# azuxmioy/Render-In-Between

Measured on AMD Instinct MI355X. Metric: rendered frames/sec at 512x512 (generator forward + blend, device-resident), higher is better.
Workload: dtype f32

## Files before the change

### render-in-between_amd/csrc/kernels.hip.h

```cpp
#pragma once
#include "igemm.hip.h"

namespace rib {

struct GemmDmaParams {
  const float* A; const float* B; float* C;
  int M, N, K, lda, ldc;
  size_t sA, sB, sC;
  int modB;
};

typedef uint32_t u32x4 __attribute__((ext_vector_type(4)));
__device__ __forceinline__ void split3_bf16(const float4 p, const float4 q, bf16x8& hi, bf16x8& mid, bf16x8& lo) {
  const float x[8] = {p.x, p.y, p.z, p.w, q.x, q.y, q.z, q.w};
  u32x4 h, m, l;
#pragma unroll
  for (int i = 0; i < 4; ++i) {
    const uint32_t u0 = __float_as_uint(x[2 * i]), u1 = __float_as_uint(x[2 * i + 1]);
    h[i] = __builtin_amdgcn_perm(u1, u0, 0x07060302u);
    const float r0 = x[2 * i] - __uint_as_float(u0 & 0xffff0000u), r1 = x[2 * i + 1] - __uint_as_float(u1 & 0xffff0000u);
    const uint32_t v0 = __float_as_uint(r0), v1 = __float_as_uint(r1);
    m[i] = __builtin_amdgcn_perm(v1, v0, 0x07060302u);
    const float s0 = r0 - __uint_as_float(v0 & 0xffff0000u), s1 = r1 - __uint_as_float(v1 & 0xffff0000u);
    l[i] = __builtin_amdgcn_perm(__float_as_uint(s1), __float_as_uint(s0), 0x07060302u);
  }
  hi = __builtin_bit_cast(bf16x8, h); mid = __builtin_bit_cast(bf16x8, m); lo = __builtin_bit_cast(bf16x8, l);
}

template <int WM, int WN, int NF, int ST = ST_F32, int X3 = 0>
__global__ __launch_bounds__(256) void k_gemm_dma(const GemmDmaParams p) {
  static_assert(WM * WN == 4, "4 waves per workgroup");
  static_assert(X3 == 0 || ST == ST_F32, "split products: fp32 storage");
  constexpr int BM = 32 * WM, BN = 32 * NF * WN, BK = 32;
  constexpr int EPW = ST == ST_F32 ? 1 : 2;
  constexpr int STAGE = (BM + BN) * BK;
  constexpr int NFILL = (BM + BN) / 32;
  __shared__ __attribute__((aligned(16))) float smem[2 * STAGE];
  const int tid = threadIdx.x, lane = tid & 63, li = lane & 31, lh = lane >> 5;
  const int wave = __builtin_amdgcn_readfirstlane(tid >> 6);
  const int wm = wave / WN, wn = wave % WN;
  const int m0 = blockIdx.x * BM, n0 = blockIdx.y * BN;
  const int z = blockIdx.z;
  const float* A = p.A + (size_t)z * p.sA / EPW;
  const float* B = p.B + (size_t)(p.modB ? z % p.modB : 0) * p.sB / EPW;
  f32x16 acc[NF];
  f32x16 acc_s[X3 == 2 ? NF : 1];
#pragma unroll
  for (int nf = 0; nf < NF; ++nf)
#pragma unroll
    for (int r = 0; r < 16; ++r) { acc[nf][r] = 0.f; if constexpr (X3 == 2) acc_s[nf][r] = 0.f; }
  const int nch = p.K / (BK * EPW);
  typedef __attribute__((address_space(3))) void lds_void;
  const uint32_t lds0 = (uint32_t)(size_t)(lds_void*)smem;
  const float* src[NFILL];
#pragma unroll
  for (int j = 0; j < NFILL; ++j) {
    const int trow = wave * 8 + 32 * j + (lane >> 3);
    const bool isA = 32 * j < BM;
    const int row = isA ? trow : trow - BM;
    const int ls = (lane & 7) ^ ((row >> 1) & 7);
    src[j] = isA ? A + (size_t)min(m0 + row, p.M - 1) * (p.lda / EPW) + ls * 4 : B + (size_t)min(n0 + row, p.N - 1) * (p.K / EPW) + ls * 4;
  }
  auto fill = [&](int st, int kc) {
#pragma unroll
    for (int j = 0; j < NFILL; ++j) {
      const uint32_t dst = lds0 + (uint32_t)(st * STAGE + (wave * 8 + 32 * j) * BK) * 4u;
      asm volatile("s_mov_b32 m0, %0\n\ts_nop 0\n\tglobal_load_lds_dwordx4 %1, off" ::"s"(dst), "v"(src[j] + kc) : "memory");
    }
  };
  fill(0, 0);
  for (int c = 0; c < nch; ++c) {
    const int st = c & 1;
    asm volatile("s_waitcnt vmcnt(0)\n\ts_waitcnt lgkmcnt(0)\n\ts_barrier" ::: "memory");
    if (c + 1 < nch) fill(st ^ 1, (c + 1) * BK);
    const float* sA = smem + st * STAGE;
    const float* sB = sA + BM * BK;
    if constexpr (X3 != 0) {
#pragma unroll
      for (int ks = 0; ks < BK / 16; ++ks) {
        const int s0 = ks * 4 + lh, s1 = s0 + 2;
        const int ra = wm * 32 + li;
        bf16x8 ah, am, al;
        split3_bf16(*reinterpret_cast<const float4*>(sA + ra * BK + (s0 ^ ((ra >> 1) & 7)) * 4),
                    *reinterpret_cast<const float4*>(sA + ra * BK + (s1 ^ ((ra >> 1) & 7)) * 4), ah, am, al);
#pragma unroll
        for (int nf = 0; nf < NF; ++nf) {
          const int rb = (wn * NF + nf) * 32 + li;
          bf16x8 bh, bm, bl;
          split3_bf16(*reinterpret_cast<const float4*>(sB + rb * BK + (s0 ^ ((rb >> 1) & 7)) * 4),
                      *reinterpret_cast<const float4*>(sB + rb * BK + (s1 ^ ((rb >> 1) & 7)) * 4), bh, bm, bl);
          f32x16& sm = X3 == 2 ? acc_s[nf] : acc[nf];
          sm = __builtin_amdgcn_mfma_f32_32x32x16_bf16(am, bm, sm, 0, 0, 0);
          sm = __builtin_amdgcn_mfma_f32_32x32x16_bf16(ah, bl, sm, 0, 0, 0);
          sm = __builtin_amdgcn_mfma_f32_32x32x16_bf16(al, bh, sm, 0, 0, 0);
          sm = __builtin_amdgcn_mfma_f32_32x32x16_bf16(ah, bm, sm, 0, 0, 0);
          sm = __builtin_amdgcn_mfma_f32_32x32x16_bf16(am, bh, sm, 0, 0, 0);
          acc[nf] = __builtin_amdgcn_mfma_f32_32x32x16_bf16(ah, bh, acc[nf], 0, 0, 0);
        }
      }
      continue;
    }
#pragma unroll
    for (int kb = 0; kb < BK / 8; ++kb) {
      const int slot = kb * 2 + lh;
      const int ra = wm * 32 + li;
      const float4 a = *reinterpret_cast<const float4*>(sA + ra * BK + (slot ^ ((ra >> 1) & 7)) * 4);
      float4 b[NF];
#pragma unroll
      for (int nf = 0; nf < NF; ++nf) {
        const int rb = (wn * NF + nf) * 32 + li;
        b[nf] = *reinterpret_cast<const float4*>(sB + rb * BK + (slot ^ ((rb >> 1) & 7)) * 4);
      }
#pragma unroll
      for (int nf = 0; nf < NF; ++nf) {
        if constexpr (ST == ST_F32) {
          acc[nf] = __builtin_amdgcn_mfma_f32_32x32x2f32(a.x, b[nf].x, acc[nf], 0, 0, 0);
          acc[nf] = __builtin_amdgcn_mfma_f32_32x32x2f32(a.y, b[nf].y, acc[nf], 0, 0, 0);
          acc[nf] = __builtin_amdgcn_mfma_f32_32x32x2f32(a.z, b[nf].z, acc[nf], 0, 0, 0);
          acc[nf] = __builtin_amdgcn_mfma_f32_32x32x2f32(a.w, b[nf].w, acc[nf], 0, 0, 0);
        } else if constexpr (ST == ST_F16) {
          acc[nf] = __builtin_amdgcn_mfma_f32_32x32x16_f16(*reinterpret_cast<const f16x8*>(&a), *reinterpret_cast<const f16x8*>(&b[nf]), acc[nf], 0, 0, 0);
        } else {
          acc[nf] = __builtin_amdgcn_mfma_f32_32x32x16_bf16(*reinterpret_cast<const bf16x8*>(&a), *reinterpret_cast<const bf16x8*>(&b[nf]), acc[nf], 0, 0, 0);
        }
      }
    }
  }
  float* C = p.C + (size_t)z * p.sC;
#pragma unroll
  for (int nf = 0; nf < NF; ++nf) {
    const int col = n0 + (wn * NF + nf) * 32 + li;
#pragma unroll
    for (int r = 0; r < 16; ++r) {
      const int row = m0 + wm * 32 + (r & 3) + 8 * (r >> 2) + 4 * lh;
      float v = acc[nf][r];
      if constexpr (X3 == 2) v += acc_s[nf][r];
      if (row < p.M && col < p.N) C[(size_t)row * p.ldc + col] = v;
    }
  }
}

struct FinalizeParams {
  const double* part;
  int tiles, Cs, C;
// ... 106 lines not shown
      const int oy = pix / p.Wout, ox = pix % p.Wout;
      const size_t rpix = p.res_ups ? ((size_t)n * (p.Hout >> 1) + (oy >> 1)) * (p.Wout >> 1) + (ox >> 1) : (size_t)n * npix + pix;
#pragma unroll
      for (int e = 0; e < 4; ++e) rres[k][e] = ld_act<ST>(p.res, rpix * p.resC + min(c4 * 4 + e, p.resC - 1));
    }
  }
  float vals[4][4];
#pragma unroll
  for (int k = 0; k < 4; ++k) {
    const int pix = blockIdx.x * ppb + k * slots + slot;
    const float4 a = acc4[k];
    const float v[4] = {a.x + bv.x, a.y + bv.y, a.z + bv.z, a.w + bv.w};
#pragma unroll
    for (int e = 0; e < 4; ++e) {
      float t = v[e];
      if (p.res) t += rres[k][e];
      t = apply_act(t, p.act);
      if constexpr (ST != ST_F32) t = round16<ST>(t);
      vals[k][e] = (pix < npix && c4 * 4 + e < p.Cout) ? t : 0.f;
    }
#pragma unroll
    for (int e = 0; e < 4; ++e) { s1[e] += (double)vals[k][e]; s2[e] += (double)vals[k][e] * (double)vals[k][e]; }
  }
#pragma unroll
  for (int k = 0; k < 4; ++k) {
    const int pix = blockIdx.x * ppb + k * slots + slot;
    if (pix < npix) {
      const size_t opix = (size_t)n * npix + pix;
#pragma unroll
      for (int e = 0; e < 4; ++e)
        if (c4 * 4 + e < p.Cout) st_act<ST>(p.y, opix * p.yC + p.yoff + c4 * 4 + e, vals[k][e]);
    }
  }
  if (p.stat_part) {
#pragma unroll
    for (int e = 0; e < 4; ++e) { red[0][threadIdx.x][e] = s1[e]; red[1][threadIdx.x][e] = s2[e]; }
    __syncthreads();
    for (int c = threadIdx.x; c < p.CoutPad; c += 256) {
      const int g = c / 4, e = c % 4;
      double a1 = 0.0, a2 = 0.0;
      for (int s = 0; s < slots; ++s) { a1 += red[0][s * c4n + g][e]; a2 += red[1][s * c4n + g][e]; }
      double* dst = p.stat_part + (((size_t)n * p.blocks + blockIdx.x) * 2) * p.CoutPad;
      dst[c] = a1;
      dst[p.CoutPad + c] = a2;
    }
  }
}

struct StatSrc {
  const double* part;
  int tiles, Cs;
  float inv_count;
  const float* gamma;
  const float* beta;
};

__device__ __forceinline__ void block_stats_64(const StatSrc& s, int n, int c0, int nch, double* red ,
                                               float* s_sc, float* s_sh) {
  const int j = threadIdx.x & 63, q = threadIdx.x >> 6;
  double a1 = 0.0, a2 = 0.0;
  if (j < nch) stats_from_partials(s.part + (size_t)n * s.tiles * 2 * s.Cs, s.tiles, s.Cs, c0 + j, q, 4, a1, a2);
  red[(q * 64 + j) * 2] = a1; red[(q * 64 + j) * 2 + 1] = a2;
  __syncthreads();
  if (q == 0 && j < nch) {
    double t1 = 0.0, t2 = 0.0;
#pragma unroll
    for (int k = 0; k < 4; ++k) { t1 += red[(k * 64 + j) * 2]; t2 += red[(k * 64 + j) * 2 + 1]; }
    float sc, sh;
    scale_shift_of(t1, t2, s.inv_count, s.gamma ? s.gamma[c0 + j] : 1.f, s.beta ? s.beta[c0 + j] : 0.f, sc, sh);
    s_sc[j] = sc; s_sh[j] = sh;
  }
  __syncthreads();
}

enum { WSRC_PLAIN = 0, WSRC_SPADE = 1, WSRC_JOIN = 2 };
struct WinoInParams {
  const float* x; int H, W, xC, Cin;
  const float* pro_scale; const float* pro_shift; int pro_ld, pro_lrelu;
  StatSrc st;
  float* v; int tilesY, tilesX;
  int nslices, ublocks;
  int x_ups; const float* slab; int slab_ld, col0; const float* sbias;
  const float* x2; const float* xres; float* o; const float* pro2_scale; const float* pro2_shift; StatSrc st2;
};

__device__ __forceinline__ float spade_mod1(float x, float sc, float sh, float g, float bg, float b, float bb) {
  return fmaf(fmaf(x, sc, sh), 1.f + (g + bg), b + bb);
}

template <int MODE> struct WinoConsts { float4 sc, sh, bg, bb, sc2, sh2; bool aff; };
template <int MODE> struct WinoRaw { float4 a, b, c; };

template <int MODE>
__device__ __forceinline__ void wino_in_consts(const WinoInParams& p, int n, int slice, int c4, bool cok, double* red, float* s_sc,
                                               float* s_sh, WinoConsts<MODE>& k) {
  k.sc = make_float4(1.f, 1.f, 1.f, 1.f); k.sh = make_float4(0.f, 0.f, 0.f, 0.f);
  k.aff = false;
  const int l = (threadIdx.x & 15) * 4;
  if (p.st.part) {
    block_stats_64(p.st, n, slice * 64, min(64, p.Cin - slice * 64), red, s_sc, s_sh);
    k.sc = make_float4(s_sc[l], s_sc[l + 1], s_sc[l + 2], s_sc[l + 3]);
    k.sh = make_float4(s_sh[l], s_sh[l + 1], s_sh[l + 2], s_sh[l + 3]);
    k.aff = true;
  } else if (p.pro_scale && cok) {
    k.sc = *reinterpret_cast<const float4*>(p.pro_scale + (size_t)n * p.pro_ld + c4 * 4);
    k.sh = *reinterpret_cast<const float4*>(p.pro_shift + (size_t)n * p.pro_ld + c4 * 4);
    k.aff = true;
  }
  if constexpr (MODE == WSRC_SPADE) {
    const int v = c4 * 4, colg = (v / 32) * 64 + (v % 32);
    k.bg = cok ? *reinterpret_cast<const float4*>(p.sbias + colg) : k.sh;
    k.bb = cok ? *reinterpret_cast<const float4*>(p.sbias + colg + 32) : k.sh;
  }
  if constexpr (MODE == WSRC_JOIN) {
    k.sc2 = make_float4(1.f, 1.f, 1.f, 1.f); k.sh2 = make_float4(0.f, 0.f, 0.f, 0.f);
    if (p.x2) {
      if (p.st2.part) {
        __syncthreads();
        block_stats_64(p.st2, n, slice * 64, min(64, p.Cin - slice * 64), red, s_sc, s_sh);
        k.sc2 = make_float4(s_sc[l], s_sc[l + 1], s_sc[l + 2], s_sc[l + 3]);
        k.sh2 = make_float4(s_sh[l], s_sh[l + 1], s_sh[l + 2], s_sh[l + 3]);
      } else if (cok) {
        k.sc2 = *reinterpret_cast<const float4*>(p.pro2_scale + (size_t)n * p.pro_ld + c4 * 4);
        k.sh2 = *reinterpret_cast<const float4*>(p.pro2_shift + (size_t)n * p.pro_ld + c4 * 4);
      }
    }
  }
}

template <int MODE>
__device__ __forceinline__ void wino_fetch(const WinoInParams& p, int n, int cy, int cx, int c4, WinoRaw<MODE>& r) {
  if constexpr (MODE == WSRC_SPADE) {
    const int Hs = p.x_ups ? p.H >> 1 : p.H, Ws = p.x_ups ? p.W >> 1 : p.W;
    const int sy = p.x_ups ? cy >> 1 : cy, sx = p.x_ups ? cx >> 1 : cx;
    r.a = *reinterpret_cast<const float4*>(p.x + (((size_t)n * Hs + sy) * Ws + sx) * p.xC + c4 * 4);
    const int v = c4 * 4, colg = (v / 32) * 64 + (v % 32);
    const float* sl = p.slab + (((size_t)n * p.H + cy) * p.W + cx) * p.slab_ld + p.col0 + colg;
    r.b = *reinterpret_cast<const float4*>(sl);
    r.c = *reinterpret_cast<const float4*>(sl + 32);
  } else {
    const size_t e = (((size_t)n * p.H + cy) * p.W + cx) * p.xC + c4 * 4;
    r.a = *reinterpret_cast<const float4*>(p.x + e);
    if constexpr (MODE == WSRC_JOIN) r.b = *reinterpret_cast<const float4*>((p.x2 ? p.x2 : p.xres) + e);
  }
}

template <int MODE>
__device__ __forceinline__ float4 wino_value(const WinoInParams& p, const WinoConsts<MODE>& k, const WinoRaw<MODE>& r) {
  float4 w = r.a;
  if constexpr (MODE == WSRC_SPADE) {
    w = make_float4(spade_mod1(r.a.x, k.sc.x, k.sh.x, r.b.x, k.bg.x, r.c.x, k.bb.x), spade_mod1(r.a.y, k.sc.y, k.sh.y, r.b.y, k.bg.y, r.c.y, k.bb.y),
                    spade_mod1(r.a.z, k.sc.z, k.sh.z, r.b.z, k.bg.z, r.c.z, k.bb.z), spade_mod1(r.a.w, k.sc.w, k.sh.w, r.b.w, k.bg.w, r.c.w, k.bb.w));
    if (p.pro_lrelu) w = lrelu4(w);
  } else if constexpr (MODE == WSRC_JOIN) {
    w = make_float4(w.x * k.sc.x + k.sh.x, w.y * k.sc.y + k.sh.y, w.z * k.sc.z + k.sh.z, w.w * k.sc.w + k.sh.w);
    if (p.x2) { w.x += r.b.x * k.sc2.x + k.sh2.x; w.y += r.b.y * k.sc2.y + k.sh2.y; w.z += r.b.z * k.sc2.z + k.sh2.z; w.w += r.b.w * k.sc2.w + k.sh2.w; }
    else { w.x += r.b.x; w.y += r.b.y; w.z += r.b.z; w.w += r.b.w; }
  } else {
    if (k.aff) w = make_float4(w.x * k.sc.x + k.sh.x, w.y * k.sc.y + k.sh.y, w.z * k.sc.z + k.sh.z, w.w * k.sc.w + k.sh.w);
    if (p.pro_lrelu) w = lrelu4(w);
  }
  return w;
}

#define RIB_F4_SUB(a, b) make_float4((a).x - (b).x, (a).y - (b).y, (a).z - (b).z, (a).w - (b).w)
#define RIB_F4_ADD(a, b) make_float4((a).x + (b).x, (a).y + (b).y, (a).z + (b).z, (a).w + (b).w)

template <int MODE>
__global__ __launch_bounds__(256) void k_wino_in(const WinoInParams p) {
  __shared__ double red[4 * 64 * 2];
  __shared__ float s_sc[64], s_sh[64];
  const int c4n = p.Cin / 4;
  const int n = blockIdx.y;
  const int slice = blockIdx.x % p.nslices, ub = blockIdx.x / p.nslices;
  const int c4 = slice * 16 + (threadIdx.x & 15);
  const bool cok = c4 < c4n;
  const int ntiles = p.tilesY * p.tilesX;
  WinoConsts<MODE> kc;
  wino_in_consts<MODE>(p, n, slice, c4, cok, red, s_sc, s_sh, kc);
  if (!cok) return;
  for (int u = ub * 16 + (threadIdx.x >> 4); u < ntiles * 4; u += p.ublocks * 16) {
    const int r = u & 3, tile = u >> 2;
    const int ty = tile / p.tilesX, tx = tile % p.tilesX;
    const int ia = r == 0 ? 0 : (r == 2 ? 2 : 1), ib = r == 0 ? 2 : (r == 1 ? 2 : (r == 2 ? 1 : 3));
    const float sg = r == 1 ? 1.f : -1.f;
    WinoRaw<MODE> d[2][4];
#pragma unroll
    for (int a = 0; a < 2; ++a)
#pragma unroll
      for (int q = 0; q < 4; ++q) {
        const int iy = 2 * ty - 1 + (a ? ib : ia), ix = 2 * tx - 1 + q;
        wino_fetch<MODE>(p, n, min(max(iy, 0), p.H - 1), min(max(ix, 0), p.W - 1), c4, d[a][q]);
      }
    float4 t[4];
#pragma unroll
    for (int q = 0; q < 4; ++q) {
      float4 v[2];
#pragma unroll
      for (int a = 0; a < 2; ++a) {
        const int iy = 2 * ty - 1 + (a ? ib : ia), ix = 2 * tx - 1 + q;
        const bool inb = iy >= 0 && iy < p.H && ix >= 0 && ix < p.W;
        float4 w = wino_value<MODE>(p, kc, d[a][q]);
        if constexpr (MODE == WSRC_JOIN) {
          if (r == 1 && (q == 1 || q == 2) && inb) *reinterpret_cast<float4*>(p.o + (((size_t)n * p.H + iy) * p.W + ix) * p.xC + c4 * 4) = w;
        }
        if (!inb) w = make_float4(0.f, 0.f, 0.f, 0.f);
        v[a] = w;
      }
      t[q] = make_float4(v[0].x + sg * v[1].x, v[0].y + sg * v[1].y, v[0].z + sg * v[1].z, v[0].w + sg * v[1].w);
    }
    const size_t plane = (size_t)ntiles * p.Cin;
    float* vb = p.v + (size_t)n * 16 * plane + (size_t)tile * p.Cin + c4 * 4;
    *reinterpret_cast<float4*>(vb + (size_t)(r * 4 + 0) * plane) = RIB_F4_SUB(t[0], t[2]);
    *reinterpret_cast<float4*>(vb + (size_t)(r * 4 + 1) * plane) = RIB_F4_ADD(t[1], t[2]);
    *reinterpret_cast<float4*>(vb + (size_t)(r * 4 + 2) * plane) = RIB_F4_SUB(t[2], t[1]);
    *reinterpret_cast<float4*>(vb + (size_t)(r * 4 + 3) * plane) = RIB_F4_SUB(t[1], t[3]);
  }
}

struct WinoOutParams {
  const float* m; int tilesY, tilesX, CoutPad;
  const float* bias;
  float* y; int yC, yoff, Cout, Hout, Wout;
  int act;
  const float* res; int resC;
  double* stat_part;
  int nslices, ublocks;
};

__device__ __forceinline__ void wino_out_partials(double (*red)[256][4], const double s1[4], const double s2[4], double* stat_part,
                                                  int n, int ublocks, int ub, int slice, int CoutPad) {
#pragma unroll
  for (int e = 0; e < 4; ++e) { red[0][threadIdx.x][e] = s1[e]; red[1][threadIdx.x][e] = s2[e]; }
  __syncthreads();
  if (threadIdx.x < 64) {
    const int c = slice * 64 + threadIdx.x;
    if (c < CoutPad) {
      const int g = threadIdx.x >> 2, e = threadIdx.x & 3;
      double a1 = 0.0, a2 = 0.0;
#pragma unroll
      for (int s = 0; s < 16; ++s) { a1 += red[0][s * 16 + g][e]; a2 += red[1][s * 16 + g][e]; }
      double* dst = stat_part + (((size_t)n * ublocks + ub) * 2) * CoutPad;
      dst[c] = a1;
      dst[CoutPad + c] = a2;
    }
  }
}

__global__ __launch_bounds__(256) void k_wino_out(const WinoOutParams p) {
  __shared__ __attribute__((aligned(16))) double red[2][256][4];
  const int c4n = p.CoutPad / 4;
  const int slice = blockIdx.x % p.nslices, ub = blockIdx.x / p.nslices;
  const int c4 = slice * 16 + (threadIdx.x & 15);
  const int n = blockIdx.y;
  const int ntiles = p.tilesY * p.tilesX;
  double s1[4] = {0.0, 0.0, 0.0, 0.0}, s2[4] = {0.0, 0.0, 0.0, 0.0};
  if (c4 < c4n) {
    const float4 bv = *reinterpret_cast<const float4*>(p.bias + c4 * 4);
    const size_t plane = (size_t)ntiles * p.CoutPad;
    for (int u = ub * 16 + (threadIdx.x >> 4); u < ntiles * 2; u += p.ublocks * 16) {
      const int r = u & 1, tile = u >> 1;
      const float* mb = p.m + (size_t)n * 16 * plane + (size_t)tile * p.CoutPad + c4 * 4;
      float4 mm[3][4];
#pragma unroll
      for (int a = 0; a < 3; ++a)
#pragma unroll
        for (int q = 0; q < 4; ++q) mm[a][q] = *reinterpret_cast<const float4*>(mb + (size_t)((r + a) * 4 + q) * plane);
      const float sg = r ? -1.f : 1.f;
      float4 uu[4];
#pragma unroll
      for (int q = 0; q < 4; ++q)
        uu[q] = make_float4(mm[0][q].x + sg * (mm[1][q].x + mm[2][q].x), mm[0][q].y + sg * (mm[1][q].y + mm[2][q].y),
                            mm[0][q].z + sg * (mm[1][q].z + mm[2][q].z), mm[0][q].w + sg * (mm[1][q].w + mm[2][q].w));
      float4 yv[2];
      yv[0] = RIB_F4_ADD(RIB_F4_ADD(uu[0], uu[1]), uu[2]);
      yv[1] = RIB_F4_SUB(RIB_F4_SUB(uu[1], uu[2]), uu[3]);
      const int ty = tile / p.tilesX, tx = tile % p.tilesX;
      const int oy = 2 * ty + r;
      float rr[2][4];
#pragma unroll
      for (int q = 0; q < 2; ++q) {
        const int cy = min(oy, p.Hout - 1), cx = min(2 * tx + q, p.Wout - 1);
#pragma unroll
        for (int e = 0; e < 4; ++e)
          rr[q][e] = p.res ? p.res[(((size_t)n * p.Hout + cy) * p.Wout + cx) * p.resC + min(c4 * 4 + e, p.resC - 1)] : 0.f;
      }
#pragma unroll
      for (int q = 0; q < 2; ++q) {
        const int ox = 2 * tx + q;
        const bool inb = oy < p.Hout && ox < p.Wout;
        const float v4[4] = {yv[q].x + bv.x, yv[q].y + bv.y, yv[q].z + bv.z, yv[q].w + bv.w};
#pragma unroll
        for (int e = 0; e < 4; ++e) {
          float t = apply_act(v4[e] + rr[q][e], p.act);
          const bool ok = inb && c4 * 4 + e < p.Cout;
          if (ok) p.y[(((size_t)n * p.Hout + oy) * p.Wout + ox) * p.yC + p.yoff + c4 * 4 + e] = t;
          t = ok ? t : 0.f;
          s1[e] += (double)t; s2[e] += (double)t * (double)t;
        }
      }
    }
  }
  if (p.stat_part) wino_out_partials(red, s1, s2, p.stat_part, n, p.ublocks, ub, slice, p.CoutPad);
}

__device__ __constant__ float kWino4BT[6][6] = {
    {81.f / 64, 0.f, -45.f / 16, 0.f, 1.f, 0.f},        {0.f, -27.f / 16, -9.f / 4, 3.f / 4, 1.f, 0.f},
    {0.f, 27.f / 16, -9.f / 4, -3.f / 4, 1.f, 0.f},     {0.f, -27.f / 32, -9.f / 16, 3.f / 2, 1.f, 0.f},
    {0.f, 27.f / 32, -9.f / 16, -3.f / 2, 1.f, 0.f},    {0.f, 81.f / 64, 0.f, -45.f / 16, 0.f, 1.f}};
__device__ __constant__ float kWino4AT[4][6] = {
    {1.f, 1.f, 1.f, 1.f, 1.f, 0.f},                      {0.f, 3.f / 4, -3.f / 4, 3.f / 2, -3.f / 2, 0.f},
    {0.f, 9.f / 16, 9.f / 16, 9.f / 4, 9.f / 4, 0.f},    {0.f, 27.f / 64, -27.f / 64, 27.f / 8, -27.f / 8, 1.f}};

__device__ __forceinline__ float4 f4_fma(float a, float4 x, float4 acc) {
  return make_float4(fmaf(a, x.x, acc.x), fmaf(a, x.y, acc.y), fmaf(a, x.z, acc.z), fmaf(a, x.w, acc.w));
}
__device__ __forceinline__ float4 f4_scale(float a, float4 x) { return make_float4(a * x.x, a * x.y, a * x.z, a * x.w); }

template <int MODE>
__global__ __launch_bounds__(256) void k_wino4_in(const WinoInParams p) {
  __shared__ double red[4 * 64 * 2];
  __shared__ float s_sc[64], s_sh[64];
  const int c4n = p.Cin / 4;
  const int n = blockIdx.y;
  const int slice = blockIdx.x % p.nslices, ub = blockIdx.x / p.nslices;
  const int c4 = slice * 16 + (threadIdx.x & 15);
  const bool cok = c4 < c4n;
  const int ntiles = p.tilesY * p.tilesX;
  WinoConsts<MODE> kc;
  wino_in_consts<MODE>(p, n, slice, c4, cok, red, s_sc, s_sh, kc);
  if (!cok) return;
  for (int u = ub * 16 + (threadIdx.x >> 4); u < ntiles * 6; u += p.ublocks * 16) {
    const int r = u % 6, tile = u / 6;
    const int ty = tile / p.tilesX, tx = tile % p.tilesX;
    const int a0 = r == 0 ? 0 : 1, da = (r == 0 || r == 5) ? 2 : 1, na = (r == 0 || r == 5) ? 3 : 4;
    float4 t[6];
#pragma unroll
    for (int q = 0; q < 6; ++q) t[q] = make_float4(0.f, 0.f, 0.f, 0.f);
    if constexpr (MODE == WSRC_PLAIN) {
      WinoRaw<MODE> d[4][6];
#pragma unroll
      for (int k = 0; k < 4; ++k)
#pragma unroll
        for (int q = 0; q < 6; ++q) {
          const int iy = 4 * ty - 1 + a0 + min(k, na - 1) * da, ix = 4 * tx - 1 + q;
          wino_fetch<MODE>(p, n, min(max(iy, 0), p.H - 1), min(max(ix, 0), p.W - 1), c4, d[k][q]);
        }
#pragma unroll
      for (int k = 0; k < 4; ++k) {
        const int a = a0 + min(k, na - 1) * da;
        const float coef = k < na ? kWino4BT[r][a] : 0.f;
        const int iy = 4 * ty - 1 + a;
#pragma unroll
        for (int q = 0; q < 6; ++q) {
          const int ix = 4 * tx - 1 + q;
          float4 w = wino_value<MODE>(p, kc, d[k][q]);
          if (!(iy >= 0 && iy < p.H && ix >= 0 && ix < p.W)) w = make_float4(0.f, 0.f, 0.f, 0.f);
          t[q] = f4_fma(coef, w, t[q]);
        }
      }
    } else {
#pragma unroll 1
      for (int k = 0; k < na; ++k) {
        const int a = a0 + k * da;
        const float coef = kWino4BT[r][a];
        const int iy = 4 * ty - 1 + a;
        WinoRaw<MODE> d[6];
#pragma unroll
        for (int q = 0; q < 6; ++q) wino_fetch<MODE>(p, n, min(max(iy, 0), p.H - 1), min(max(4 * tx - 1 + q, 0), p.W - 1), c4, d[q]);
#pragma unroll
        for (int q = 0; q < 6; ++q) {
          const int ix = 4 * tx - 1 + q;
          const bool inb = iy >= 0 && iy < p.H && ix >= 0 && ix < p.W;
          float4 w = wino_value<MODE>(p, kc, d[q]);
          if constexpr (MODE == WSRC_JOIN) {
            if (r == 1 && q >= 1 && q <= 4 && inb) *reinterpret_cast<float4*>(p.o + (((size_t)n * p.H + iy) * p.W + ix) * p.xC + c4 * 4) = w;
          }
          if (!inb) w = make_float4(0.f, 0.f, 0.f, 0.f);
          t[q] = f4_fma(coef, w, t[q]);
        }
      }
    }
    const size_t plane = (size_t)ntiles * p.Cin;
    float* vb = p.v + (size_t)n * 36 * plane + (size_t)tile * p.Cin + c4 * 4;
    const float4 e24 = f4_fma(-45.f / 16, t[2], t[4]);
    const float4 o13 = f4_fma(-45.f / 16, t[3], t[5]);
    const float4 ev1 = f4_fma(-9.f / 4, t[2], t[4]), od1 = f4_fma(-27.f / 16, t[1], f4_scale(3.f / 4, t[3]));
    const float4 ev2 = f4_fma(-9.f / 16, t[2], t[4]), od2 = f4_fma(-27.f / 32, t[1], f4_scale(3.f / 2, t[3]));
    *reinterpret_cast<float4*>(vb + (size_t)(r * 6 + 0) * plane) = f4_fma(81.f / 64, t[0], e24);
    *reinterpret_cast<float4*>(vb + (size_t)(r * 6 + 1) * plane) = RIB_F4_ADD(ev1, od1);
    *reinterpret_cast<float4*>(vb + (size_t)(r * 6 + 2) * plane) = RIB_F4_SUB(ev1, od1);
    *reinterpret_cast<float4*>(vb + (size_t)(r * 6 + 3) * plane) = RIB_F4_ADD(ev2, od2);
    *reinterpret_cast<float4*>(vb + (size_t)(r * 6 + 4) * plane) = RIB_F4_SUB(ev2, od2);
    *reinterpret_cast<float4*>(vb + (size_t)(r * 6 + 5) * plane) = f4_fma(81.f / 64, t[1], o13);
  }
}

__global__ __launch_bounds__(256) void k_wino4_out(const WinoOutParams p) {
  __shared__ __attribute__((aligned(16))) double red[2][256][4];
  const int c4n = p.CoutPad / 4;
  const int slice = blockIdx.x % p.nslices, ub = blockIdx.x / p.nslices;
  const int c4 = slice * 16 + (threadIdx.x & 15);
  const int n = blockIdx.y;
  const int ntiles = p.tilesY * p.tilesX;
  double s1[4] = {0.0, 0.0, 0.0, 0.0}, s2[4] = {0.0, 0.0, 0.0, 0.0};
  if (c4 < c4n) {
    const float4 bv = *reinterpret_cast<const float4*>(p.bias + c4 * 4);
    const size_t plane = (size_t)ntiles * p.CoutPad;
    for (int unit = ub * 16 + (threadIdx.x >> 4); unit < ntiles * 4; unit += p.ublocks * 16) {
      const int tile = unit >> 2, r = unit & 3;
      const float* mb = p.m + (size_t)n * 36 * plane + (size_t)tile * p.CoutPad + c4 * 4;
      float4 u[6];
#pragma unroll
      for (int q = 0; q < 6; ++q) u[q] = make_float4(0.f, 0.f, 0.f, 0.f);
      const int ax = r == 0 ? 0 : 5;
      const float cx_ = (r == 0 || r == 3) ? 1.f : 0.f;
      float4 mm[5][6];
#pragma unroll
      for (int k = 0; k < 5; ++k)
#pragma unroll
        for (int q = 0; q < 6; ++q) mm[k][q] = *reinterpret_cast<const float4*>(mb + (size_t)((k < 4 ? k + 1 : ax) * 6 + q) * plane);
#pragma unroll
      for (int k = 0; k < 5; ++k) {
        const float coef = k < 4 ? kWino4AT[r][k + 1] : cx_;
#pragma unroll
        for (int q = 0; q < 6; ++q) u[q] = f4_fma(coef, mm[k][q], u[q]);
      }
      const float4 s12 = RIB_F4_ADD(u[1], u[2]);
      const float4 d12 = RIB_F4_SUB(u[1], u[2]);
      const float4 s34 = RIB_F4_ADD(u[3], u[4]);
      const float4 d34 = RIB_F4_SUB(u[3], u[4]);
      float4 yv[4];
      yv[0] = make_float4(u[0].x + s12.x + s34.x, u[0].y + s12.y + s34.y, u[0].z + s12.z + s34.z, u[0].w + s12.w + s34.w);
      yv[1] = f4_fma(3.f / 4, d12, f4_scale(3.f / 2, d34));
      yv[2] = f4_fma(9.f / 16, s12, f4_scale(9.f / 4, s34));
      yv[3] = f4_fma(27.f / 64, d12, f4_fma(27.f / 8, d34, u[5]));
      const int ty = tile / p.tilesX, tx = tile % p.tilesX;
      const int oy = 4 * ty + r;
      float rr[4][4];
#pragma unroll
      for (int q = 0; q < 4; ++q) {
        const int cy = min(oy, p.Hout - 1), cx = min(4 * tx + q, p.Wout - 1);
#pragma unroll
        for (int e = 0; e < 4; ++e)
          rr[q][e] = p.res ? p.res[(((size_t)n * p.Hout + cy) * p.Wout + cx) * p.resC + min(c4 * 4 + e, p.resC - 1)] : 0.f;
      }
#pragma unroll
      for (int q = 0; q < 4; ++q) {
        const int ox = 4 * tx + q;
        const bool inb = oy < p.Hout && ox < p.Wout;
        const float v4[4] = {yv[q].x + bv.x, yv[q].y + bv.y, yv[q].z + bv.z, yv[q].w + bv.w};
#pragma unroll
        for (int e = 0; e < 4; ++e) {
          float t = apply_act(v4[e] + rr[q][e], p.act);
          const bool ok = inb && c4 * 4 + e < p.Cout;
          if (ok) p.y[(((size_t)n * p.Hout + oy) * p.Wout + ox) * p.yC + p.yoff + c4 * 4 + e] = t;
          t = ok ? t : 0.f;
          s1[e] += (double)t; s2[e] += (double)t * (double)t;
        }
      }
    }
  }
  if (p.stat_part) wino_out_partials(red, s1, s2, p.stat_part, n, p.ublocks, ub, slice, p.CoutPad);
}
#undef RIB_F4_SUB
#undef RIB_F4_ADD

struct ModulateParams {
  const float* slab; int ksplit, B, slab_ld, col0;
  const float* bias;
  const float* xm; int xmC, xm_ups;
  const float* m_scale; const float* m_shift; int m_ld;
  StatSrc st;
  int C, nsets;
  float* ys0; float* ys1; int act0, act1;
  int Hout, Wout;
  int nslices, pblocks;
};
// ... 728 lines not shown
```

### render-in-between_amd/csrc/rib.hip

```cpp
#include "kernels.hip.h"
#include "raster.hip.h"
#include "quality.hip.h"
#include "resize.hip.h"
#include <hip/hip_ext.h>
#include "../../include/rib.h"

#include <algorithm>
#include <array>
#include <climits>
#include <cmath>
#include <cstdarg>
#include <cstdio>
#include <cstdlib>
#include <cstring>
#include <map>
#include <memory>
#include <string>
#include <variant>
#include <vector>


#include "variants.hip.h"
#define RIB_V(sec, ...) RIB_I_V(RIB_F_EXTERN, __VA_ARGS__)
#define RIB_VK(sec, ...) RIB_I_VK(RIB_F_EXTERN, __VA_ARGS__)
// ... 23 lines not shown
#undef RIB_VBX
#undef RIB_V1D
#undef RIB_VS1D
#undef RIB_VD
#undef RIB_VSD
#undef RIB_VD9

using namespace rib;

namespace { struct ProfPair { hipEvent_t start = nullptr, stop = nullptr; }; thread_local ProfPair g_prof_pair; }
#define RIB_KLAUNCH(KERNEL, grid, block, lds, st, ...)                                                                       \
  do {                                                                                                                       \
    if (g_prof_pair.start) hipExtLaunchKernelGGL(KERNEL, grid, block, lds, st, g_prof_pair.start, g_prof_pair.stop, 0, __VA_ARGS__); \
    else hipLaunchKernelGGL(KERNEL, grid, block, lds, st, __VA_ARGS__);                                                      \
  } while (0)

#if !defined(RIB_BUILD_STAMP) || !defined(RIB_SHARD_STAMP)
#error "compile through csrc/build.py (-DRIB_BUILD_STAMP / -DRIB_SHARD_STAMP: content hashes of the sources, see build.py)"
#endif
extern "C" {
#define RIB_X(s) extern const char rib_stamp_section_##s[];
RIB_FOR_SECTIONS(RIB_X)
#undef RIB_X
}
extern "C" __attribute__((used, visibility("hidden"))) const char kLibStamp[] = "rib-stamp lib " RIB_BUILD_STAMP;

namespace {

thread_local std::string g_create_error;

std::string fmt(const char* f, ...) {
  char buf[1024];
  va_list ap;
  va_start(ap, f);
  vsnprintf(buf, sizeof buf, f, ap);
  va_end(ap);
  return buf;
}

inline int pad8(int c) { return c <= 8 ? 8 : (c <= 16 ? 16 : (c + 31) / 32 * 32); }
inline int pad16(int c) { return c <= 16 ? 16 : (c + 31) / 32 * 32; }
inline uint16_t host_bf16(float f) {
  uint32_t u; memcpy(&u, &f, 4);
  if ((u & 0x7fffffffu) > 0x7f800000u) return (uint16_t)((u >> 16) | 0x40);
  u += 0x7fffu + ((u >> 16) & 1u);
  return (uint16_t)(u >> 16);
}
inline uint16_t host_f16(float f) {
  uint32_t u; memcpy(&u, &f, 4);
  const uint32_t sign = (u >> 16) & 0x8000u;
  const uint32_t a = u & 0x7fffffffu;
  if (a > 0x7f800000u) return (uint16_t)(sign | 0x7e00u);
  if (a >= 0x477ff000u) return (uint16_t)(sign | 0x7c00u);
  if (a < 0x33000001u) return (uint16_t)sign;
  int e = (int)(a >> 23) - 127;
  uint32_t m = (a & 0x7fffffu) | 0x800000u;
  int shift = e < -14 ? 13 + (-14 - e) : 13;
  uint32_t half_m = m >> shift;
  const uint32_t rem = m & ((1u << shift) - 1), halfway = 1u << (shift - 1);
  if (rem > halfway || (rem == halfway && (half_m & 1u))) half_m += 1;
  uint32_t h16;
  if (e < -14) h16 = half_m;
  else h16 = ((uint32_t)(e + 15) << 10) + (half_m - 0x400u);
  return (uint16_t)(sign | h16);
}
inline int pad32(int c) { return (c + 31) / 32 * 32; }
inline int pick_bk(int cp) { return cp % 32 == 0 ? 32 : (cp % 16 == 0 ? 16 : 8); }
inline size_t align256(size_t b) { return (b + 255) / 256 * 256; }

struct ConvDef {
  std::string name;
  int cin = 0, cout = 0, ks = 3, stride = 1;
  bool spectral = true;
  int spade_cond = 0;
  bool in_affine = false;
  bool used = true;
  size_t w_off = 0, b_off = 0, g_off = 0, be_off = 0;
  size_t fb_off = 0;
  bool ups_in = false;
  size_t wp_off = 0;
  int cinp = 0, coutp = 0;
  size_t w16_off = 0, wp16_off = 0;
  bool wino_ok = false; size_t zero_off = 0;
  size_t wl_off = 0; int lowc_ce = 0, lowc_ncol = 0;
};

struct TensorDef {
  std::string name;
  std::vector<int64_t> dims;
  bool used;
  std::vector<float> data;
  bool set = false;
};

struct SpadeGroup {
  std::string key;
  int C = 0, Cp = 0, cond = 0, nsets = 1;
  size_t w_off = 0, b_off = 0;
  size_t w16_off = 0;
  int npad = 0;
  size_t w1_off = 0, b1_off = 0;
  int level = 0, col0 = 0;
};

struct Cfg {
  rib_config c;
  int nf(int i) const { return std::min(c.max_num_filters, c.num_filters << i); }
  int mask_nf(int i) const { return std::min(c.mask_max_filters, c.mask_filters << i); }
  int emb_ch(int i) const { return std::min(c.emb_max_filters, c.emb_filters << i); }
  int cond_ch(int i) const { return std::min(c.max_num_filters, c.emb_filters << std::min(i, c.emb_down)); }
  int num_res_blocks() const { return (int)std::ceil((c.num_layers - c.num_down_img) / 2.0) * 2; }
};

void add_embedder(std::vector<ConvDef>& L, const Cfg& g, const std::string& prefix, int cin, bool used) {
  ConvDef c; c.name = prefix + ".conv_first"; c.cin = cin; c.cout = g.emb_ch(0); c.used = used; L.push_back(c);
  for (int i = 0; i < g.c.emb_down; ++i) {
    ConvDef d; d.name = prefix + ".down_" + std::to_string(i); d.cin = g.emb_ch(i); d.cout = g.emb_ch(i + 1);
    d.stride = 2; d.used = used; L.push_back(d);
  }
}
void add_spade_block(std::vector<ConvDef>& L, const std::string& name, int cin, int cout, int cond) {
  const int hidden = std::min(cin, cout);
  ConvDef a; a.name = name + ".conv_block_0"; a.cin = cin; a.cout = hidden; a.spade_cond = cond; L.push_back(a);
  ConvDef b; b.name = name + ".conv_block_1"; b.cin = hidden; b.cout = cout; b.spade_cond = cond; L.push_back(b);
  if (cin != cout) {
    ConvDef s; s.name = name + ".conv_block_s"; s.cin = cin; s.cout = cout; s.ks = 1; s.spade_cond = cond; L.push_back(s);
  }
}
void add_mask_block(std::vector<ConvDef>& L, const std::string& name, int cin, int cout) {
  const int hidden = std::min(cin, cout);
  ConvDef a; a.name = name + ".conv_block_0"; a.cin = cin; a.cout = hidden; a.in_affine = true; L.push_back(a);
  ConvDef b; b.name = name + ".conv_block_1"; b.cin = hidden; b.cout = cout; b.in_affine = true; L.push_back(b);
  if (cin != cout) {
    ConvDef s; s.name = name + ".conv_block_s"; s.cin = cin; s.cout = cout; s.ks = 1; s.in_affine = true; L.push_back(s);
  }
}

std::vector<ConvDef> build_inventory(const Cfg& g) {
  std::vector<ConvDef> L;
  const rib_config& c = g.c;
  add_embedder(L, g, "ref_embedding", c.image_nc * 2, true);
  add_embedder(L, g, "label_embedding", c.label_nc, false);
  for (int i = c.num_down_img; i >= 0; --i) add_spade_block(L, "up_" + std::to_string(i), g.nf(i + 1), g.nf(i), g.cond_ch(i));
  { ConvDef d; d.name = "conv_img"; d.cin = c.num_filters; d.cout = c.image_nc; d.spectral = false; L.push_back(d); }
  { ConvDef d; d.name = "conv_mask"; d.cin = c.num_filters; d.cout = 1; d.spectral = false; d.used = false; L.push_back(d); }
  { ConvDef d; d.name = "down_first"; d.cin = c.label_nc; d.cout = c.num_filters; d.spectral = false; L.push_back(d); }
  for (int i = 0; i <= c.num_down_img; ++i) add_spade_block(L, "down_" + std::to_string(i), g.nf(i), g.nf(i + 1), g.cond_ch(i));
  const int res_ch = g.nf(c.num_down_img + 1);
  for (int i = 0; i < g.num_res_blocks(); ++i) add_spade_block(L, "res_" + std::to_string(i), res_ch, res_ch, g.cond_ch(c.num_down_img + 1));
  const std::string m = "flow_network_temp";
  const char* branches[2] = {"down_lbl", "down_img"};
  const int bcin[2] = {c.label_nc, c.image_nc * 3};
  for (int b = 0; b < 2; ++b) {
    ConvDef d; d.name = m + "." + branches[b] + ".0"; d.cin = bcin[b]; d.cout = c.mask_filters; d.in_affine = true; L.push_back(d);
    for (int i = 0; i < c.mask_down; ++i) {
      ConvDef e; e.name = m + "." + branches[b] + "." + std::to_string(i + 1); e.cin = g.mask_nf(i); e.cout = g.mask_nf(i + 1);
      e.stride = 2; e.in_affine = true; L.push_back(e);
    }
  }
  const int ch = g.mask_nf(c.mask_down);
  for (int i = 0; i < c.mask_res_blocks; ++i) add_mask_block(L, m + ".res_flow." + std::to_string(i), i == 0 ? ch * 2 : ch, ch);
  for (int j = 0; j < c.mask_down; ++j) {
    const int i = c.mask_down - 1 - j;
    ConvDef d; d.name = m + ".up_flow." + std::to_string(2 * j + 1); d.cin = g.mask_nf(i + 1); d.cout = g.mask_nf(i); d.in_affine = true; d.ups_in = true; L.push_back(d);
  }
  { ConvDef d; d.name = m + ".conv_mask.0"; d.cin = c.mask_filters; d.cout = 1; d.spectral = false; L.push_back(d); }
// ... 136 lines not shown
}

Choice choose_variant_dt(int bf16, int stride, int ks, bool ups, bool spade, int ncols, int B, int Hout, int Wout,
                         int Cin, bool allow_split, int Cin2, bool allow_n16) {
  Choice best;
  best.cycles = 1e300;
  static const int kSplits[] = {1, 2, 3, 4, 6, 8, 12, 16};
  for (int i = 0; i < kNumVariants; ++i) {
    const Variant& v = kVariants[i];
    if (v.dma() || v.DMAK) continue;
    if (v.STRIDE != stride || v.KS != ks || v.UPS != ups || v.SPADE != spade || Cin % v.BK != 0 || Cin2 % v.BK != 0) continue;
    if (v.NF == 0 && !allow_n16) continue;
    if (v.SPADE && v.NF == 1) continue;
    if (v.BF16 != bf16) continue;
    const int BK = v.BK;
    if ((v.KW > 1 || v.TB > 1) && (long)((Hout + v.TH() - 1) / v.TH()) * ((Wout + v.TW() - 1) / v.TW()) * ((ncols + v.BN() - 1) / v.BN()) * B >= 512) continue;
    const int nchunks = Cin / BK;
    const int Ht = ups ? Hout / 2 : Hout, Wt = ups ? Wout / 2 : Wout;
    const long tiles = (long)((Ht + v.TH() - 1) / v.TH()) * ((Wt + v.TW() - 1) / v.TW());
    const long ntiles = v.NF == 0 ? 1 : (ncols + v.BN() - 1) / v.BN();
    const int occ = std::max(1, std::min(v.MF * v.NF * (ups ? 4 : 1) >= 4 ? 4 : 6, 160 * 1024 / v.lds_bytes()));
    for (int S : kSplits) {
      if (S > nchunks || (S > 1 && (!allow_split || v.NF == 0))) break;
      const long wgs = tiles * ntiles * B * S;
      const int chunks = (nchunks + S - 1) / S;
      const int taps = ups ? 16 : ks * ks;
      const double mfma_tap = v.NF == 0 ? (BK / 16) * v.MF * 8 * 32.0
                                        : (v.BF16 != PREC_F32 ? (BK / 16) * v.MF * v.NF * 32.0 : (BK / 8) * v.MF * v.NF * 4 * 64.0);
      const double ovh_wg = (chunks * (std::max(1, taps / v.TB) * 350.0 + (ks == 1 && v.TB == 2 ? 300.0 : 600.0)) + 7000.0) / v.KW + (v.KW - 1) * 1500.0;
      const double mfma_wg = (double)chunks * taps * mfma_tap;
      const double t_lat = std::ceil((double)wgs / (256.0 * occ)) * (mfma_wg + ovh_wg);
      const double t_cu = std::ceil((double)wgs / 256.0) * (mfma_wg + ovh_wg / occ);
      double t = std::max(t_lat, t_cu);
      if (S > 1) t += 6000.0 + (double)(S + 1) * B * Hout * Wout * pad32(ncols) * 4.0 / 1667.0;
      if (t < best.cycles) { best.cycles = t; best.v = &v; best.ksplit = S; }
    }
  }
  return best;
}

const Variant* pick_gemm_dma(int prec, long Z, int M, int N, int K) {
  static const bool off = getenv("RIB_NO_DMA") != nullptr;
  if (off || K % (prec == PREC_F32 ? 32 : 64) != 0) return nullptr;
  const Variant* best = nullptr; long best_area = 0, best_wgs = 0;
  for (int i = 0; i < kNumVariants; ++i) {
    const Variant& v = kVariants[i];
    if (!v.dma() || v.BF16 != prec) continue;
    const long wgs = Z * ((M + v.BM() - 1) / v.BM()) * ((N + v.BN() - 1) / v.BN());
    const long area = (long)v.BM() * v.BN();
    const bool full = wgs >= 512, bfull = best_wgs >= 512;
    if (!best || (full && (!bfull || area > best_area)) || (!full && !bfull && wgs > best_wgs)) { best = &v; best_area = area; best_wgs = wgs; }
  }
  return best;
}

enum OpKind { OP_PACK, OP_IGEMM, OP_FINALIZE, OP_POOL, OP_INADD, OP_SPLITEPI, OP_MODULATE, OP_WINO_IN, OP_WINO_OUT, OP_LOWC, OP_GEMM };

enum PtrSpace { PS_NULL = 0, PS_WS, PS_WEIGHT, PS_USER, PS_WINO };
enum UserSlot { U_LABEL = 0, U_FAKE, U_PREV, U_IMG, U_MASK, U_FUSE, U_COUNT };
struct PRef {
  PtrSpace sp = PS_NULL;
  size_t off = 0;
};


using OpParams = std::variant<PackParams, IgemmParams, FinalizeParams, PoolParams, InAddParams, SplitEpiParams, ModulateParams,
                              WinoInParams, WinoOutParams, LowcParams, GemmDmaParams>;
static_assert(std::is_same<std::variant_alternative_t<OP_IGEMM, OpParams>, IgemmParams>::value &&
              std::is_same<std::variant_alternative_t<OP_GEMM, OpParams>, GemmDmaParams>::value, "OpParams follows OpKind");
struct Op {
  int kclass = 0;
  std::string name;
  std::string for_op;
  bool label_only = false;
  dim3 grid;
  double flops = 0;
  const Variant* var = nullptr;
  int small_co = 0;
  bool head = false;
  bool fuse_blend = false;
  bool wino = false;
  int wino_m = 0;
  int wi_mode = 0;
  int lowc_ce = 0, lowc_ncol = 0, lowc_tw = 32;
  OpParams params;
  struct Binding { PRef ref; unsigned field = 0; };
  static constexpr int kMaxBindings = 24;
  Binding binds[kMaxBindings];
  int nbinds = 0;

  OpKind kind() const { return (OpKind)params.index(); }
  template <class P> const P& as() const { return std::get<P>(params); }
  template <class P, class T> unsigned field_of(T* P::*f) const {
    return (unsigned)(reinterpret_cast<const char*>(&(as<P>().*f)) - reinterpret_cast<const char*>(&params));
  }
  template <class P, class T> unsigned field_of(StatSrc P::*s, T* StatSrc::*f) const {
    return (unsigned)(reinterpret_cast<const char*>(&((as<P>().*s).*f)) - reinterpret_cast<const char*>(&params));
  }
  PRef ref_at(unsigned field) const {
    for (int i = 0; i < nbinds; ++i) if (binds[i].field == field) return binds[i].ref;
    return PRef();
  }
  void bind_at(unsigned field, PRef r) {
    int i = 0;
    while (i < nbinds && binds[i].field != field) ++i;
    if (r.sp == PS_NULL) { if (i < nbinds) binds[i] = binds[--nbinds]; return; }
    if (i == kMaxBindings) abort();
    binds[i] = Binding{r, field};
    if (i == nbinds) ++nbinds;
  }
  template <class P, class T> bool bound(T* P::*f) const { return ref_at(field_of(f)).sp != PS_NULL; }
};
template <class P> struct OpOf : Op {
  OpOf(int kclass_, const std::string& name_) { kclass = kclass_; name = name_; memset(&params.emplace<P>(), 0, sizeof(P)); }
  P& p() { return std::get<P>(params); }
  template <class T> void bind(T* P::*f, PRef r) { bind_at(field_of(f), r); }
  template <class T> void bind(StatSrc P::*s, T* StatSrc::*f, PRef r) { bind_at(field_of(s, f), r); }
  template <class T> PRef ref(T* P::*f) const { return ref_at(field_of(f)); }
};

struct PendingStats {
  Op fin;
  bool pushed = false;
  size_t part_off = 0; int tiles = 0, Cs = 0; float inv_count = 0.f;
  bool affine = false; size_t g_off = 0, be_off = 0;
};

struct Tap { std::string name; size_t off; int Cp, C, H, W; };

struct LazySrc;
struct Act {
  size_t off = 0;
  int Cp = 0, C = 0, H = 0, W = 0;
  bool virt = false; int usrc[3] = {0, 0, 0}, uc[3] = {0, 0, 0};
  std::shared_ptr<LazySrc> lazy;
};
struct PendingStats;
struct Norm {
  size_t sc = 0, sh = 0; int ld = 0;
  bool valid = false;
  std::shared_ptr<PendingStats> pend;
};

struct LazySrc {
  int mode = 0;
  std::string name;
  Act x; Norm nx;
  bool x_ups = false, lrelu = false;
  size_t slab_off = 0; int slab_ld = 0, col0 = 0; size_t sbias_off = 0;
  bool has2 = false; Act x2; Norm n2; Act xres; Act o;
};

struct LabelSlots { size_t x0 = 0, x0_b = 0, nx_sc = 0, nx_sh = 0, nx_b = 0, cat = 0, cat_b = 0, ncat_sc = 0, ncat_sh = 0, ncat_b = 0; };

struct Plan {
  bool labels_only = false;
  LabelSlots ls;
  int B, H, W;
  size_t ws_bytes = 0;
  size_t ws_virtual = 0;
  std::vector<Op> ops;
  std::vector<Tap> taps;
  double flops[RIB_KC_COUNT] = {0};
};

}

struct rib_handle {
  Cfg g;
  int device = 0;
  std::string err;
  std::vector<ConvDef> convs;
  std::map<std::string, int> conv_index;
  std::vector<TensorDef> tensors;
  std::map<std::string, int> tensor_index;
  std::vector<SpadeGroup> spades;
  std::map<std::string, int> spade_index;
  std::map<int, std::vector<int>> level_groups;
  float* d_blob = nullptr;
  size_t d_blob_floats = 0;
  std::vector<float> host_blob;
  size_t blob_floats = 0;
  size_t zero_off = 0;
  uint64_t layout_hash = 0;
  struct WinoSet { int conv = 0, wm = 0; float* d = nullptr; size_t floats = 0; };
  std::vector<WinoSet> wino_sets;
  std::map<std::pair<int, int>, int> wino_index;
  bool weights_ready = false;
  int prec_mode = PREC_F32;
  int prec() const { return prec_mode; }
  int products = 0;
  bool mc16() const { return prec_mode != PREC_F32; }
  int padc(int c) const { return mc16() ? pad16(c) : pad8(c); }
  int esz() const { return mc16() ? 2 : 4; }
  bool warp_lds_ready = false;
  bool keep_taps = false;
  int plan_batch = 0;
  std::map<std::array<int, 5>, std::unique_ptr<Plan>> plans;
  std::map<std::string, std::pair<int, int>> choices;
  struct ChainGraph { std::array<uintptr_t, 12> key; hipGraphExec_t exec; uint64_t used; hipStream_t stream; };
  std::vector<ChainGraph> chain_graphs;
  bool graph_replay = false;
  uint64_t graph_clock = 0, graph_captures = 0, graph_replays = 0;
  struct RasterStage { char* host = nullptr; size_t bytes = 0; hipEvent_t done = nullptr; };
  RasterStage raster_stage[2];
  int raster_next = 0;
  bool profiling = false;
  bool prof_kernels = false;
  std::vector<std::pair<int, hipEvent_t>> prof_events;
  struct KernelEv { int kclass; hipEvent_t start, stop; };
  std::vector<KernelEv> prof_kernel_events;
  int64_t prof_launches[RIB_KC_COUNT] = {0};
  double prof_ms[RIB_KC_COUNT] = {0};
};

namespace {

#define HIP_TRY(h, expr)                                                                   \
  do {                                                                                     \
    hipError_t e_ = (expr);                                                                \
    if (e_ != hipSuccess) {                                                                \
      (h)->err = fmt("%s failed: %s (%s:%d)", #expr, hipGetErrorString(e_), __FILE__, __LINE__); \
      return RIB_ERR_HIP;                                                                  \
    }                                                                                      \
  } while (0)

void destroy_chain_graph(rib_handle::ChainGraph& g) {
  (void)hipDeviceSynchronize();
  (void)hipGraphExecDestroy(g.exec);
}
void drop_chain_graphs(rib_handle* h) {
  if (h->chain_graphs.empty()) return;
  if (h->device >= 0) (void)hipSetDevice(h->device);
  for (auto& g : h->chain_graphs) destroy_chain_graph(g);
  h->chain_graphs.clear();
}

int fail(rib_handle* h, int code, const std::string& msg) {
  h->err = msg;
  return code;
}

const ConvDef& conv_of(const rib_handle* h, const std::string& name) {
  return h->convs[h->conv_index.at(name)];
}

__global__ __launch_bounds__(256) void k_wino_filters(const float* w, float* u, int coutp, int cinp, int wm) {
#pragma clang fp contract(off)
  const double G2[4][3] = {{1, 0, 0}, {0.5, 0.5, 0.5}, {0.5, -0.5, 0.5}, {0, 0, 1}};
  const double G4[6][3] = {{64.0 / 81, 0, 0},
                           {-128.0 / 243, -32.0 / 81, -8.0 / 27}, {-128.0 / 243, 32.0 / 81, -8.0 / 27},
                           {32.0 / 243, 16.0 / 81, 8.0 / 27},     {32.0 / 243, -16.0 / 81, 8.0 / 27},
                           {0, 0, 1}};
  const int T = wm + 2;
  const size_t idx = (size_t)blockIdx.x * 256 + threadIdx.x;
  if (idx >= (size_t)coutp * cinp) return;
  const int o = (int)(idx / cinp), i = (int)(idx % cinp);
  double g[3][3], t[6][3];
  for (int k = 0; k < 9; ++k) g[k / 3][k % 3] = (double)w[((size_t)o * 9 + k) * cinp + i];
  for (int r = 0; r < T; ++r)
    for (int dx = 0; dx < 3; ++dx) {
      const double* Gr = wm == 2 ? G2[r] : G4[r];
      t[r][dx] = Gr[0] * g[0][dx] + Gr[1] * g[1][dx] + Gr[2] * g[2][dx];
    }
  for (int r = 0; r < T; ++r)
    for (int q = 0; q < T; ++q) {
      const double* Gq = wm == 2 ? G2[q] : G4[q];
      u[((size_t)(r * T + q) * coutp + o) * cinp + i] = (float)(t[r][0] * Gq[0] + t[r][1] * Gq[1] + t[r][2] * Gq[2]);
    }
}

int fill_wino_set(rib_handle* h, int si, hipStream_t st) {
  rib_handle::WinoSet& ws = h->wino_sets[si];
  const ConvDef& c = h->convs[ws.conv];
  if (!ws.d || !h->d_blob) return RIB_OK;
  const size_t n = (size_t)c.coutp * c.cinp;
  RIB_KLAUNCH(k_wino_filters, dim3((unsigned)((n + 255) / 256)), dim3(256), 0, st, h->d_blob + c.w_off, ws.d, c.coutp, c.cinp, ws.wm);
  HIP_TRY(h, hipGetLastError());
  return RIB_OK;
}

int ensure_wino_set(rib_handle* h, int ci, int wm) {
  auto it = h->wino_index.find({ci, wm});
  if (it != h->wino_index.end()) return it->second;
  const ConvDef& c = h->convs[ci];
  rib_handle::WinoSet ws; ws.conv = ci; ws.wm = wm; ws.floats = (size_t)(wm + 2) * (wm + 2) * c.coutp * c.cinp;
  if (h->device >= 0) {
    hipError_t e = hipSetDevice(h->device);
    if (e == hipSuccess) e = hipMalloc(reinterpret_cast<void**>(&ws.d), ws.floats * sizeof(float));
    if (e != hipSuccess) { h->err = fmt("Winograd filter set of %s: %s", c.name.c_str(), hipGetErrorString(e)); return -1; }
  }
  const int si = (int)h->wino_sets.size();
  h->wino_sets.push_back(ws);
  h->wino_index[{ci, wm}] = si;
  if (h->device >= 0 && h->weights_ready) {
    if (hipDeviceSynchronize() != hipSuccess) { h->err = "Winograd filter transform: device not idle-able"; return -1; }
    if (fill_wino_set(h, si, nullptr) != RIB_OK) return -1;
    if (hipDeviceSynchronize() != hipSuccess) { h->err = "Winograd filter transform failed"; return -1; }
  }
  return si;
}

int refresh_wino_sets(rib_handle* h, hipStream_t st) {
  for (int si = 0; si < (int)h->wino_sets.size(); ++si) {
    const int rc = fill_wino_set(h, si, st);
    if (rc) return rc;
  }
  return RIB_OK;
}
void free_wino_sets(rib_handle* h) {
  for (auto& ws : h->wino_sets) if (ws.d) (void)hipFree(ws.d);
  h->wino_sets.clear(); h->wino_index.clear();
}

static bool lowc_instantiated(int ce, int ncol) {
  return (ce == 6 && ncol == 64) || (ce == 10 && ncol == 32) || (ce == 22 && ncol == 32) || (ce == 24 && ncol == 16);
}
template <int CE, int NCOL> static void launch_lowc_t(int tw, dim3 grid, hipStream_t st, const LowcParams& p) {
  if (tw == 16) RIB_KLAUNCH((k_conv_lowc<CE, NCOL, ST_F32, 16>), grid, dim3(256), 0, st, p);
  else RIB_KLAUNCH((k_conv_lowc<CE, NCOL, ST_F32, 32>), grid, dim3(256), 0, st, p);
}
static void launch_lowc(int ce, int ncol, int tw, dim3 grid, hipStream_t st, const LowcParams& p) {
  if (ce == 6 && ncol == 64) launch_lowc_t<6, 64>(tw, grid, st, p);
  else if (ce == 10 && ncol == 32) launch_lowc_t<10, 32>(tw, grid, st, p);
  else if (ce == 22 && ncol == 32) launch_lowc_t<22, 32>(tw, grid, st, p);
  else if (ce == 24 && ncol == 16) launch_lowc_t<24, 16>(tw, grid, st, p);
}

enum { BLOB_HEADER_FLOATS = 64, BLOB_MAGIC = 0x57424952 , BLOB_VERSION = 3 };
struct BlobHeader { uint32_t magic, version, prec, reserved; uint64_t floats, layout_hash; };

void assign_weight_layout(rib_handle* h) {
  size_t off = BLOB_HEADER_FLOATS;
  h->spades.clear(); h->spade_index.clear();
  auto take = [&](size_t nfloats) { size_t o = off; off += (nfloats + 63) / 64 * 64; return o; };
  h->zero_off = take(64);
  for (auto& c : h->convs) {
    if (!c.used) continue;
    c.cinp = h->padc(c.cin);
    c.coutp = pad32(c.cout);
    c.w16_off = c.wp16_off = 0; c.fb_off = 0;
    c.w_off = take((size_t)c.coutp * c.ks * c.ks * c.cinp);
    if (c.ups_in) c.wp_off = take((size_t)c.coutp * 16 * c.cinp);
    c.b_off = take(c.coutp);
    if (c.in_affine) { c.g_off = take(c.coutp); c.be_off = take(c.coutp); }
    if (c.spade_cond && c.name.size() > 13 && c.name.compare(c.name.size() - 13, 13, ".conv_block_1") == 0 &&
        h->conv_index.count(c.name.substr(0, c.name.size() - 1) + "s"))
      c.fb_off = take(c.coutp);
  }
  {
    const rib_config& gc = h->g.c;
    const int D = gc.num_down_img;
    std::vector<std::pair<std::string, int>> blocks;
    for (int i = 0; i <= D; ++i) blocks.push_back({"down_" + std::to_string(i), std::min(gc.emb_down, i)});
    for (int i = 0; i < h->g.num_res_blocks(); ++i) blocks.push_back({"res_" + std::to_string(i), std::min(gc.emb_down, D + 1)});
    for (int i = D; i >= 0; --i) blocks.push_back({"up_" + std::to_string(i), std::min(i, gc.emb_down)});
    h->level_groups.clear();
    for (int level = 0; level <= gc.emb_down; ++level) {
      int col = 0;
      for (auto& bl : blocks) {
        if (bl.second != level) continue;
        for (const char* which : {"0", "1"}) {
          auto it = h->conv_index.find(bl.first + ".conv_block_" + which);
          if (it == h->conv_index.end()) continue;
          const ConvDef& c = h->convs[it->second];
          if (!c.used || !c.spade_cond) continue;
          SpadeGroup sg;
          sg.C = c.cin; sg.Cp = h->padc(c.cin); sg.cond = c.spade_cond;
          sg.nsets = (which[0] == '0' && h->conv_index.count(bl.first + ".conv_block_s")) ? 2 : 1;
          sg.key = bl.first + "." + which;
          sg.npad = (sg.nsets * sg.Cp + 31) / 32 * 64;
          sg.level = level; sg.col0 = col; col += sg.npad;
          sg.w_off = take((size_t)sg.npad * h->padc(sg.cond));
          h->level_groups[level].push_back((int)h->spades.size());
          h->spade_index[sg.key] = (int)h->spades.size();
          h->spades.push_back(sg);
        }
      }
    }
    for (auto& sg : h->spades) sg.b_off = take(sg.npad);
  }
  for (auto& c : h->convs) { c.wino_ok = false; c.zero_off = 0; }
  if (h->prec() == PREC_F32 && !getenv("RIB_NO_WINO")) {
    for (auto& c : h->convs) {
      if (!c.used || c.ks != 3 || c.stride != 1 || c.ups_in || c.fb_off != 0 || c.cin < 256 || c.cout < 64 || c.cinp % 32 || 128 % (c.coutp / 4)) continue;
      c.wino_ok = true;
      c.zero_off = take(c.coutp);
    }
  }
  for (auto& sg : h->spades) {
    sg.w1_off = sg.b1_off = 0;
    if (h->prec() == PREC_F32 && sg.nsets * sg.Cp == 16 && !getenv("RIB_NO_SPADE16")) {
      sg.w1_off = take((size_t)32 * h->padc(sg.cond));
      sg.b1_off = take(32);
    }
  }
  for (auto& c : h->convs) {
    c.wl_off = 0; c.lowc_ce = c.lowc_ncol = 0;
    if (!c.used || c.ks != 3 || c.stride != 1 || c.ups_in || c.fb_off != 0 || c.cin > 24 || h->mc16() || getenv("RIB_NO_LOWC")) continue;
    const int ncol = c.cout <= 16 ? 16 : c.coutp;
    const int ce = ncol == 16 ? (c.cin + 3) / 4 * 4 : (c.cin + 1) / 2 * 2;
    if (!lowc_instantiated(ce, ncol)) continue;
    c.lowc_ce = ce; c.lowc_ncol = ncol;
    c.wl_off = take((size_t)9 * ce * ncol);
  }
  if (h->mc16()) {
    const size_t pl = 1;
    for (auto& c : h->convs) {
      if (!c.used) continue;
      c.w16_off = take((pl * c.coutp * c.ks * c.ks * c.cinp + 1) / 2);
      if (c.ups_in) c.wp16_off = take((pl * c.coutp * 16 * c.cinp + 1) / 2);
    }
    for (auto& sg : h->spades) sg.w16_off = take((pl * sg.npad * h->padc(sg.cond) + 1) / 2);
  }
  h->blob_floats = off;
  uint64_t hs = 1469598103934665603ull;
  auto mix = [&](uint64_t v) { for (int i = 0; i < 8; ++i) { hs ^= (v >> (8 * i)) & 0xff; hs *= 1099511628211ull; } };
  for (const auto& c : h->convs)
    for (uint64_t v : {(uint64_t)c.w_off, (uint64_t)c.b_off, (uint64_t)c.g_off, (uint64_t)c.be_off, (uint64_t)c.fb_off, (uint64_t)c.wp_off, (uint64_t)c.w16_off,
                       (uint64_t)c.wp16_off, (uint64_t)c.zero_off, (uint64_t)c.wl_off}) mix(v);
  for (const auto& sg : h->spades)
    for (uint64_t v : {(uint64_t)sg.w_off, (uint64_t)sg.b_off, (uint64_t)sg.w16_off, (uint64_t)sg.w1_off, (uint64_t)sg.b1_off}) mix(v);
  mix(off);
  h->layout_hash = hs;
}
BlobHeader blob_header_of(const rib_handle* h) {
  BlobHeader bh; bh.magic = BLOB_MAGIC; bh.version = BLOB_VERSION; bh.prec = (uint32_t)h->prec(); bh.reserved = 0;
  bh.floats = h->blob_floats; bh.layout_hash = h->layout_hash;
  return bh;
}

void register_tensors(rib_handle* h) {
  auto add = [&](const std::string& n, std::vector<int64_t> d, bool used) {
    TensorDef t; t.name = n; t.dims = d; t.used = used;
    h->tensor_index[n] = (int)h->tensors.size();
    h->tensors.push_back(t);
  };
  for (auto& c : h->convs) {
    if (c.spade_cond) {
      add(c.name + ".layers.norm.mlps.0.0.layers.conv.weight", {2 * c.cin, c.spade_cond, 1, 1}, c.used);
      add(c.name + ".layers.norm.mlps.0.0.layers.conv.bias", {2 * c.cin}, c.used);
    }
    const std::string p = c.name + ".layers.conv";
    if (c.spectral) {
      add(p + ".bias", {c.cout}, c.used);
      add(p + ".weight_orig", {c.cout, c.cin, c.ks, c.ks}, c.used);
      add(p + ".weight_u", {c.cout}, c.used);
      add(p + ".weight_v", {(int64_t)c.cin * c.ks * c.ks}, c.used);
    } else {
      add(p + ".weight", {c.cout, c.cin, c.ks, c.ks}, c.used);
      add(p + ".bias", {c.cout}, c.used);
    }
    if (c.in_affine) {
      add(c.name + ".layers.norm.weight", {c.cout}, c.used);
      add(c.name + ".layers.norm.bias", {c.cout}, c.used);
    }
  }
}

const std::vector<float>* tensor_data(rib_handle* h, const std::string& name) {
  auto it = h->tensor_index.find(name);
  if (it == h->tensor_index.end()) return nullptr;
  TensorDef& t = h->tensors[it->second];
  return t.set ? &t.data : nullptr;
}

static int xcd_chunk_of(int tiles) {
  static const bool off = getenv("RIB_NO_XCD") != nullptr;
  return (!off && tiles >= 64 && tiles % 8 == 0) ? tiles / 8 : 0;
}

struct FusionPolicy {
  bool consumer_stats = !getenv("RIB_NO_CONSUMER_STATS");
  bool head_conv = !getenv("RIB_NO_HEADCONV");
  bool small_conv = !getenv("RIB_NO_SMALLCONV");
  long wino_max_px = getenv("RIB_WINO_MAX_PX") ? atol(getenv("RIB_WINO_MAX_PX")) : 16384;
  int wino_force = getenv("RIB_WINO_M") ? atoi(getenv("RIB_WINO_M")) : 0;
  bool split_k = !getenv("RIB_NO_SPLITK");
  bool n16 = !getenv("RIB_NO_N16");
  int lowc_tw = getenv("RIB_LOWC_TW") ? (atoi(getenv("RIB_LOWC_TW")) == 16 ? 16 : 32) : 0;
  long cond_gemm_max_px = getenv("RIB_COND_GEMM_MAX_PX") ? atol(getenv("RIB_COND_GEMM_MAX_PX")) : 4096;
  bool unfused_spade = !getenv("RIB_NO_UNFUSED_SPADE");
  bool lazy_sources = !getenv("RIB_NO_LAZY");
  bool fuse_shortcut = !getenv("RIB_NO_FUSE_SHORTCUT");
  bool ws_reuse = !getenv("RIB_NO_WS_REUSE");
  static bool pair_mask_encoders() { return !getenv("RIB_NO_PAIR"); }
};

struct Builder {
  rib_handle* h;
  Plan* P;
  int B;
  const FusionPolicy pol;
  size_t ws = 0;
  std::string error;
  bool mark_label = false;
  bool pair_mask = false;
  bool defer_stats = true;
  void materialize(const Norm& n, const std::string& consumer = std::string()) {
    if (n.pend && !n.pend->pushed) { n.pend->pushed = true; n.pend->fin.for_op = consumer; push(n.pend->fin); }
  }
  static bool has_partials(const Norm& n) { return n.pend && !n.pend->pushed; }
  void finalize_or_defer(Op& f, Norm* out, bool now, size_t part_off, int tiles, int Cs, float inv_count, bool affine, size_t g_off, size_t be_off) {
    if (now || !pol.consumer_stats || !defer_stats || mark_label || tiles > STATS_MAX_PARTIALS) { push(f); return; }
    auto ps = std::make_shared<PendingStats>();
    ps->fin = f; ps->part_off = part_off; ps->tiles = tiles; ps->Cs = Cs; ps->inv_count = inv_count;
    ps->affine = affine; ps->g_off = g_off; ps->be_off = be_off;
    out->pend = ps;
  }
  template <class P> bool take_partials(const Norm& n, OpOf<P>& op, StatSrc P::*src) {
    if (!has_partials(n) || n.pend->tiles > STATS_MAX_PARTIALS) return false;
    const PendingStats& ps = *n.pend;
    StatSrc& st = op.p().*src;
    st.tiles = ps.tiles; st.Cs = ps.Cs; st.inv_count = ps.inv_count;
    op.bind(src, &StatSrc::part, WS(ps.part_off));
    if (ps.affine) { op.bind(src, &StatSrc::gamma, WT(ps.g_off)); op.bind(src, &StatSrc::beta, WT(ps.be_off)); }
    return true;
  }
  OpOf<FinalizeParams> finalize_op(const std::string& producer, size_t part_off, int tiles, int Cs, int C, const Norm& out, size_t choff,
                                   int H, int W, const ConvDef* affine, int images) {
    OpOf<FinalizeParams> f(RIB_KC_STATS, producer + ".stats");
    FinalizeParams& q = f.p();
    q.tiles = tiles; q.Cs = Cs; q.C = C; q.ld = out.ld; q.off = (int)choff;
    q.inv_count = 1.0f / ((float)H * (float)W); q.eps = 1e-5f;
    f.bind(&FinalizeParams::part, WS(part_off));
    if (affine) { f.bind(&FinalizeParams::gamma, WT(affine->g_off)); f.bind(&FinalizeParams::beta, WT(affine->be_off)); }
    f.bind(&FinalizeParams::scale, WS(out.sc)); f.bind(&FinalizeParams::shift, WS(out.sh));
    f.grid = dim3((Cs + 15) / 16, images, 1);
    return f;
  }
  struct LevelSlab { size_t off = 0; int ld = 0; };
  std::map<int, LevelSlab> level_slab;
  int tuneB = 0;
  int TB_() const { return tuneB > 0 ? tuneB : B; }
  void push(Op op) {
    op.label_only = mark_label;
    P->ops.push_back(op);
  }

  struct AllocRec { size_t voff, bytes, phys; int first, last; };
  std::vector<AllocRec> allocs;
  size_t alloc(size_t bytes) {
    size_t o = ws; ws += align256(bytes);
    allocs.push_back(AllocRec{o, align256(bytes), o, INT_MAX, -1});
    return o;
  }
  Act act(int C, int H, int W) {
    Act a; a.C = C; a.Cp = h->padc(C); a.H = H; a.W = W;
    a.off = alloc((size_t)B * H * W * a.Cp * h->esz());
    return a;
  }
  Norm norm(int Cp, int images = 0) {
    Norm n; n.ld = Cp; n.valid = true;
    n.sc = alloc((size_t)(images ? images : B) * Cp * sizeof(float));
    n.sh = alloc((size_t)(images ? images : B) * Cp * sizeof(float));
    return n;
  }
  Act act_n(int images, int C, int H, int W) {
    Act a; a.C = C; a.Cp = h->padc(C); a.H = H; a.W = W;
    a.off = alloc((size_t)images * H * W * a.Cp * h->esz());
    return a;
  }
  Act virt(int C, int H, int W, int s0, int c0, int s1 = 0, int c1 = 0, int s2 = 0, int c2 = 0) {
    Act a; a.virt = true; a.C = C; a.Cp = 0; a.H = H; a.W = W;
    a.usrc[0] = s0; a.uc[0] = c0; a.usrc[1] = s1; a.uc[1] = c1; a.usrc[2] = s2; a.uc[2] = c2;
    return a;
  }
  bool lowc_serves(std::initializer_list<const char*> names) {
    for (const char* nm : names) {
      auto it = h->conv_index.find(nm);
      if (it == h->conv_index.end() || !h->convs[it->second].wl_off) return false;
    }
    return true;
  }
  bool head_without_nhwc(const ConvDef& c) {
    return c.cout <= 3 && c.ks == 3 && c.stride == 1 && (c.cinp == 16 || c.cinp == 32) && pol.small_conv && pol.head_conv;
  }
  static PRef WS(size_t off) { PRef r; r.sp = PS_WS; r.off = off; return r; }
  static PRef WT(size_t off) { PRef r; r.sp = PS_WEIGHT; r.off = off; return r; }
  static PRef US(int slot) { PRef r; r.sp = PS_USER; r.off = (size_t)slot; return r; }
  static PRef WINO(int set) { PRef r; r.sp = PS_WINO; r.off = (size_t)set; return r; }
  void tap(const std::string& name, const Act& a) { P->taps.push_back(Tap{name, a.off, a.Cp, a.C, a.H, a.W}); }

  struct ConvArgs {
    const ConvDef* cd = nullptr;
    Act in;
    bool ups = false;
    const Norm* pro = nullptr; size_t pro_choff = 0;
    bool pro_lrelu = false;
    Act out; int yoff = 0;
    int cout_store = -1;
    int act = ACT_NONE;
    const Act* res = nullptr; bool res_ups = false;
    const ConvDef* aux = nullptr; Act aux_in;
    PRef y_nchw;
    PRef y_user;
    bool y_none = false;
    bool want_stats = false;
    Norm* stats_out = nullptr; size_t stats_choff = 0;
    bool affine = false;
    bool stats_now = false;
    const ConvDef* pair = nullptr; bool pair_merge = false; int pair_yoff = 0;
    bool no_split = false;
    std::vector<std::string> choice_names;
  };

  bool runs_wino(const ConvArgs& a, int Hout, int Wout) const {
    const ConvDef& c = *a.cd;
    return h->prec() == PREC_F32 && c.wino_ok && !a.ups && !a.aux && !a.res_ups && !a.pair && !a.in.virt && a.y_nchw.sp == PS_NULL &&
           a.y_user.sp == PS_NULL && (long)Hout * Wout <= pol.wino_max_px && Hout >= 2 && Wout >= 2;
  }
  bool would_wino(const ConvDef& cd, int H, int W) const { ConvArgs t; t.cd = &cd; return runs_wino(t, H, W); }

  bool conv(const ConvArgs& a, const std::string& opname) {
    const ConvDef& c = *a.cd;
    const int Hout = a.ups ? a.in.H * 2 : (c.stride == 2 ? a.in.H / 2 : a.in.H);
    const int Wout = a.ups ? a.in.W * 2 : (c.stride == 2 ? a.in.W / 2 : a.in.W);
    if (a.in.virt) return conv_lowc(a, opname);
    const int nB = a.pair ? 2 * B : B;
    if (a.pair) {
      const ConvDef& d = *a.pair;
      if (d.cinp != c.cinp || d.coutp != c.coutp || d.cout != c.cout || d.ks != c.ks || d.stride != c.stride || d.ups_in || c.ups_in || a.ups || a.res || a.aux ||
          a.y_nchw.sp != PS_NULL || a.y_user.sp != PS_NULL || a.y_none || !a.want_stats || c.in_affine != d.in_affine || d.w_off <= c.w_off || d.b_off <= c.b_off ||
          (c.in_affine && (d.g_off <= c.g_off || d.g_off - c.g_off != d.be_off - c.be_off)) || (h->mc16() && d.w16_off <= c.w16_off)) {
        error = opname + ": the two convolutions of a paired launch must have the same shape"; return false;
      }
    }
    if (a.in.Cp != c.cinp) { error = fmt("%s: input channels %d != expected %d", opname.c_str(), a.in.Cp, c.cinp); return false; }
    if (runs_wino(a, Hout, Wout)) return conv_wino(a, opname, Hout, Wout);
    if (a.in.lazy) { error = opname + ": a lazy input (" + a.in.lazy->name + ") needs the Winograd path"; return false; }
    const bool can_split = (256 % (c.coutp / 4) == 0) && a.y_nchw.sp == PS_NULL && !a.pair && !a.no_split && pol.split_k;
    const bool can_n16 = c.cout <= 16 && !a.res && !h->mc16() && pol.n16;
    Choice ch = choose_variant(h->prec(), c.stride, c.ks, a.ups, false, c.coutp, TB_(), Hout, Wout, c.cinp, can_split, a.aux ? a.aux->cinp : 0, can_n16);
    {
      auto it = h->choices.end();
      for (const std::string& nm : a.choice_names) {
        it = h->choices.find(fmt("%d,%d,%d|%s", TB_(), P->H, P->W, nm.c_str()));
        if (it != h->choices.end()) break;
      }
      if (it == h->choices.end()) it = h->choices.find(fmt("%d,%d,%d|%s", TB_(), P->H, P->W, opname.c_str()));
      if (it != h->choices.end()) {
        const Variant& tv = kVariants[it->second.first];
        const int ts = it->second.second;
        const bool ok = !tv.dma() && !(tv.DMAK && (a.aux || ts != 1)) && !(tv.DMAK && !tv.fn_pro && !tv.fn && (a.pro || a.pro_lrelu)) && tv.BF16 == h->prec() && tv.STRIDE == c.stride && tv.KS == c.ks && tv.UPS == a.ups && !tv.SPADE && c.cinp % tv.BK == 0 &&
                        (!a.aux || a.aux->cinp % tv.BK == 0) && (tv.NF != 0 || (can_n16 && ts == 1)) &&
                        ts >= 1 && ts <= c.cinp / tv.BK && (ts == 1 || can_split);
        if (!ok) { error = fmt("%s: tuned choice (variant %d, ksplit %d) does not fit this layer", opname.c_str(), it->second.first, ts); return false; }
        ch.v = &tv; ch.ksplit = ts;
      }
    }
    const Variant* v = ch.v;
    if (!v) { error = fmt("%s: no kernel variant for Cin=%d stride=%d ks=%d ups=%d", opname.c_str(), c.cinp, c.stride, c.ks, (int)a.ups); return false; }
    const int S = ch.ksplit;
    OpOf<IgemmParams> op(RIB_KC_IGEMM, opname); op.var = v;
    IgemmParams& p = op.p();
    p.Hin = a.in.H; p.Win = a.in.W; p.xC = a.in.Cp; p.Cin = c.cinp;
    p.pro_ld = a.pro ? a.pro->ld : 0; p.pro_lrelu = a.pro_lrelu ? 1 : 0;
    p.CoutPad = c.coutp;
    p.Hout = Hout; p.Wout = Wout;
    p.tilesX = ((a.ups ? a.in.W : Wout) + v->TW() - 1) / v->TW(); p.tilesY = ((a.ups ? a.in.H : Hout) + v->TH() - 1) / v->TH();
    p.xcd_chunk = xcd_chunk_of(p.tilesX * p.tilesY);
    if (a.ups && (!c.ups_in || c.ks != 3 || c.stride != 1)) { error = opname + ": no phase filters for this upsample convolution"; return false; }
    p.act = a.act; p.ksplit = S;
    op.bind(&IgemmParams::x, WS(a.in.off));
    const bool small = c.cout <= 4 && c.ks == 3 && c.stride == 1 && !a.ups && !a.res && !a.aux && !a.want_stats &&
                       c.cinp <= 32 && 256 % (c.cinp / 4) == 0 &&
                       pol.small_conv;
    if (a.pro) {
      materialize(*a.pro, opname);
      op.bind(&IgemmParams::pro_scale, WS(a.pro->sc + a.pro_choff * sizeof(float)));
      op.bind(&IgemmParams::pro_shift, WS(a.pro->sh + a.pro_choff * sizeof(float)));
    }
    const bool w16 = h->mc16() && !small;
    op.bind(&IgemmParams::w, WT(a.ups ? (w16 ? c.wp16_off : c.wp_off) : (w16 ? c.w16_off : c.w_off))); op.bind(&IgemmParams::bias, WT(c.b_off));
    double aux_flops = 0.0;
    if (a.aux) {
      if (c.ks != 3 || c.stride != 1 || a.ups || !c.fb_off || a.aux->ks != 1 || a.aux->coutp != c.coutp || a.aux_in.Cp != a.aux->cinp ||
          a.aux_in.H != Hout || a.aux_in.W != Wout) { error = opname + ": fused shortcut operand does not fit"; return false; }
      op.bind(&IgemmParams::x2, WS(a.aux_in.off)); op.bind(&IgemmParams::w2, WT(h->mc16() ? a.aux->w16_off : a.aux->w_off)); op.bind(&IgemmParams::bias, WT(c.fb_off));
      p.x2C = a.aux_in.Cp; p.Cin2 = a.aux->cinp;
      aux_flops = 2.0 * a.aux->cin * a.aux->cout * (double)Hout * Wout * B;
    }
    if (a.y_user.sp != PS_NULL) {
      op.bind(&IgemmParams::y, a.y_user); p.yC = c.cout; p.yoff = 0; p.Cout = c.cout; p.y_f32 = 1;
    } else if (a.y_none) {
      p.yC = 0; p.yoff = 0; p.Cout = a.cout_store >= 0 ? a.cout_store : c.cout;
    } else {
      op.bind(&IgemmParams::y, WS(a.out.off)); p.yC = a.out.Cp; p.yoff = a.yoff;
      p.Cout = a.cout_store >= 0 ? a.cout_store : h->padc(c.cout);
      if (a.out.H != Hout || a.out.W != Wout) { error = fmt("%s: output size mismatch", opname.c_str()); return false; }
    }
    if (a.pair) {
      const bool w16p = h->mc16();
      p.w_mod = 2;
      p.w_stride = (unsigned)(w16p ? 2 * (a.pair->w16_off - c.w16_off) : a.pair->w_off - c.w_off);
      p.b_stride = (unsigned)(a.pair->b_off - c.b_off);
      p.pair = a.pair_merge ? 1 : 0; p.pair_yoff = a.pair_yoff;
    }
    if (a.res) { op.bind(&IgemmParams::res, WS(a.res->off)); p.resC = a.res->Cp; p.res_ups = a.res_ups ? 1 : 0; }
    op.bind(&IgemmParams::y_nchw, a.y_nchw);
    if (a.y_none && !(small && c.cout <= 3 && (c.cinp == 16 || c.cinp == 32) && pol.head_conv && a.y_nchw.sp != PS_NULL)) {
      error = opname + ": only the head kernel can run without an NHWC destination"; return false;
    }
    if (small) {
      op.small_co = c.cout;
      op.head = c.cout <= 3 && (c.cinp == 16 || c.cinp == 32) && pol.head_conv;
      op.fuse_blend = op.head && c.cout == 1 && a.y_user.sp == PS_USER && a.y_user.off == (size_t)U_MASK;
      p.bl_C = h->g.c.image_nc;
      p.ksplit = 1;
      p.tilesX = (Wout + 15) / 16; p.tilesY = (Hout + 15) / 16; p.xcd_chunk = xcd_chunk_of(p.tilesX * p.tilesY);
      op.grid = dim3(p.tilesX * p.tilesY, 1, B);
      op.flops = 2.0 * c.cin * c.ks * c.ks * c.cout * (double)Hout * Wout * B;
      P->flops[RIB_KC_IGEMM] += op.flops;
      push(op);
      return true;
    }
    int tiles = p.tilesX * p.tilesY;
    size_t part_off = 0;
    op.grid = dim3(tiles, v->NF == 0 ? 1 : (c.coutp + v->BN() - 1) / v->BN(), nB * S);
    op.flops = 2.0 * c.cin * c.ks * c.ks * c.cout * (double)Hout * Wout * nB + aux_flops;
    P->flops[RIB_KC_IGEMM] += op.flops;
    if (a.pair && (S != 1 || v->NF == 0)) { error = opname + ": a paired launch cannot split K or use the 16-column path"; return false; }
    if (S == 1) {
      if (a.want_stats) { part_off = alloc((size_t)nB * tiles * 2 * c.coutp * sizeof(double)); op.bind(&IgemmParams::stat_part, WS(part_off)); }
      push(op);
    } else {
      const size_t slab_off = alloc((size_t)S * B * Hout * Wout * c.coutp * sizeof(float));
      op.bind(&IgemmParams::slab, WS(slab_off));
      OpOf<SplitEpiParams> e(RIB_KC_CONVAUX, opname + ".splitk_sum");
      SplitEpiParams& q = e.p();
      q.ksplit = S; q.B = B; q.CoutPad = c.coutp; q.yC = p.yC; q.yoff = p.yoff; q.Cout = p.Cout;
      q.act = p.act; q.resC = p.resC; q.res_ups = p.res_ups; q.Hout = Hout; q.Wout = Wout;
      const int slots = 256 / (c.coutp / 4), ppb = slots * 4;
      const int blocks = (Hout * Wout + ppb - 1) / ppb;
      q.blocks = blocks;
      e.bind(&SplitEpiParams::slab, WS(slab_off)); e.bind(&SplitEpiParams::bias, op.ref(&IgemmParams::bias));
      e.bind(&SplitEpiParams::y, op.ref(&IgemmParams::y)); e.bind(&SplitEpiParams::res, op.ref(&IgemmParams::res));
      if (a.want_stats) { part_off = alloc((size_t)B * blocks * 2 * c.coutp * sizeof(double)); e.bind(&SplitEpiParams::stat_part, WS(part_off)); }
      e.grid = dim3(blocks, B, 1);
      tiles = blocks;
      op.bind(&IgemmParams::y, PRef()); op.bind(&IgemmParams::res, PRef());
      push(op);
      push(e);
    }
    if (a.want_stats) {
      OpOf<FinalizeParams> f = finalize_op(opname, part_off, tiles, c.coutp, h->padc(c.cout), *a.stats_out, a.stats_choff, Hout, Wout, a.affine ? &c : nullptr, nB);
      if (a.pair) { f.p().g_stride = a.affine ? (int)(a.pair->g_off - c.g_off) : 0; f.p().pair_merge = a.pair_merge ? 1 : 0; f.p().pair_off = a.pair_yoff; }
      finalize_or_defer(f, a.stats_out, a.stats_choff != 0 || a.stats_now || a.pair != nullptr, part_off, tiles, c.coutp, f.p().inv_count, a.affine, c.g_off, c.be_off);
    }
    return true;
  }

  bool conv_lowc(const ConvArgs& a, const std::string& opname) {
    const ConvDef& c = *a.cd;
    const int H = a.in.H, W = a.in.W;
    if (!c.wl_off || c.ks != 3 || c.stride != 1 || a.ups || a.pro || a.res || a.aux || a.y_nchw.sp != PS_NULL || a.y_user.sp != PS_NULL ||
        a.in.uc[0] + a.in.uc[1] + a.in.uc[2] != c.cin) { error = opname + ": not a layer k_conv_lowc can run"; return false; }
    if (a.out.H != H || a.out.W != W) { error = fmt("%s: output size mismatch", opname.c_str()); return false; }
    OpOf<LowcParams> op(RIB_KC_IGEMM, opname); op.lowc_ce = c.lowc_ce; op.lowc_ncol = c.lowc_ncol;
    LowcParams& p = op.p();
    p.c0 = a.in.uc[0]; p.c1 = a.in.uc[1]; p.c2 = a.in.uc[2];
    p.H = H; p.W = W; p.yC = a.out.Cp; p.yoff = a.yoff; p.Cout = a.cout_store >= 0 ? a.cout_store : h->padc(c.cout);
    p.act = a.act; p.CoutPad = c.coutp;
    const int tw = pol.lowc_tw ? pol.lowc_tw : ((c.lowc_ncol == 64 && !a.want_stats) ? 16 : 32);
    op.lowc_tw = tw;
    p.tilesX = (W + tw - 1) / tw; p.tilesY = (H + 7) / 8;
    if (p.Cout > c.lowc_ncol || c.cout > c.lowc_ncol) { error = opname + ": more output columns than the k_conv_lowc instantiation has"; return false; }
    op.bind(&LowcParams::s0, US(a.in.usrc[0])); if (p.c1) op.bind(&LowcParams::s1, US(a.in.usrc[1])); if (p.c2) op.bind(&LowcParams::s2, US(a.in.usrc[2]));
    op.bind(&LowcParams::w, WT(c.wl_off)); op.bind(&LowcParams::bias, WT(c.b_off)); op.bind(&LowcParams::y, WS(a.out.off));
    const int tiles = p.tilesX * p.tilesY;
    size_t part_off = 0;
    if (a.want_stats) { part_off = alloc((size_t)B * tiles * 2 * c.coutp * sizeof(double)); op.bind(&LowcParams::stat_part, WS(part_off)); }
    op.grid = dim3(tiles, B, 1);
    op.flops = 2.0 * c.cin * 9.0 * c.cout * (double)H * W * B;
    P->flops[RIB_KC_IGEMM] += op.flops;
    push(op);
    if (a.want_stats) {
      OpOf<FinalizeParams> f = finalize_op(opname, part_off, tiles, c.coutp, h->padc(c.cout), *a.stats_out, a.stats_choff, H, W, a.affine ? &c : nullptr, B);
      finalize_or_defer(f, a.stats_out, a.stats_choff != 0 || a.stats_now, part_off, tiles, c.coutp, f.p().inv_count, a.affine, c.g_off, c.be_off);
    }
    return true;
  }

  bool conv_wino(const ConvArgs& a, const std::string& opname, int Hout, int Wout) {
    const ConvDef& c = *a.cd;
    const int wino_force = pol.wino_force;
    const int wm = wino_force == 2 || wino_force == 4 ? wino_force : ((long)TB_() * ((Hout + 3) / 4) * ((Wout + 3) / 4) >= 256 ? 4 : 2);
    const int NP = (wm + 2) * (wm + 2);
    const int tilesY = (Hout + wm - 1) / wm, tilesX = (Wout + wm - 1) / wm, ntiles = tilesY * tilesX;
    const std::string gname = opname + (wm == 2 ? ".wino" : ".wino4");
    const size_t v_off = alloc((size_t)B * NP * ntiles * c.cinp * sizeof(float));
    const size_t m_off = alloc((size_t)B * NP * ntiles * c.coutp * sizeof(float));
    {
      OpOf<WinoInParams> op(RIB_KC_CONVAUX, opname + ".wino_in"); op.for_op = gname; op.wino_m = wm;
      WinoInParams& wi = op.p();
      wi.H = a.in.H; wi.W = a.in.W; wi.xC = a.in.Cp; wi.Cin = c.cinp; wi.tilesY = tilesY; wi.tilesX = tilesX;
      wi.pro_lrelu = a.pro_lrelu ? 1 : 0;
      op.bind(&WinoInParams::x, WS(a.in.off)); op.bind(&WinoInParams::v, WS(v_off));
      if (a.in.lazy) {
        const LazySrc& L = *a.in.lazy;
        if (a.pro || a.pro_lrelu) { error = gname + ": a lazy input carries its own prologue"; return false; }
        op.wi_mode = L.mode;
        op.bind(&WinoInParams::x, WS(L.x.off)); wi.xC = L.x.Cp;
        wi.pro_ld = L.nx.ld;
        if (!take_partials(L.nx, op, &WinoInParams::st)) { materialize(L.nx, gname); op.bind(&WinoInParams::pro_scale, WS(L.nx.sc)); op.bind(&WinoInParams::pro_shift, WS(L.nx.sh)); }
        if (L.mode == WSRC_SPADE) {
          wi.x_ups = L.x_ups ? 1 : 0; wi.pro_lrelu = L.lrelu ? 1 : 0;
          op.bind(&WinoInParams::slab, WS(L.slab_off)); wi.slab_ld = L.slab_ld; wi.col0 = L.col0; op.bind(&WinoInParams::sbias, WT(L.sbias_off));
        } else {
          if (L.has2) {
            op.bind(&WinoInParams::x2, WS(L.x2.off));
            if (L.n2.ld != L.nx.ld) { error = gname + ": join operands with different statistics rows"; return false; }
            if (!take_partials(L.n2, op, &WinoInParams::st2)) { materialize(L.n2, gname); op.bind(&WinoInParams::pro2_scale, WS(L.n2.sc)); op.bind(&WinoInParams::pro2_shift, WS(L.n2.sh)); }
          } else op.bind(&WinoInParams::xres, WS(L.xres.off));
          op.bind(&WinoInParams::o, WS(L.o.off));
        }
      } else if (a.pro && !(a.pro_choff == 0 && take_partials(*a.pro, op, &WinoInParams::st))) {
        materialize(*a.pro, gname);
        wi.pro_ld = a.pro->ld;
        op.bind(&WinoInParams::pro_scale, WS(a.pro->sc + a.pro_choff * sizeof(float))); op.bind(&WinoInParams::pro_shift, WS(a.pro->sh + a.pro_choff * sizeof(float)));
      }
      const int nsl = (c.cinp + 63) / 64, units = ntiles * (wm + 2);
      wi.nslices = nsl; wi.ublocks = std::max(1, std::min((units + 15) / 16, (wi.st.tiles > 0 ? 512 : 4096) / nsl));
      op.grid = dim3(wi.ublocks * nsl, B, 1);
      push(op);
    }
    {
      Choice ch;
      ch.v = pick_gemm_dma(h->prec(), (long)TB_() * NP, ntiles, c.coutp, c.cinp);
      if (!ch.v) ch = choose_variant(h->prec(), 1, 1, false, false, c.coutp, TB_() * NP, tilesY, tilesX, c.cinp, false, 0, false);
      auto it = h->choices.find(fmt("%d,%d,%d|%s", TB_(), P->H, P->W, gname.c_str()));
      if (it != h->choices.end()) {
        const Variant& tv = kVariants[it->second.first];
        if (tv.BF16 != h->prec() || tv.KS != 1 || tv.STRIDE != 1 || tv.UPS || tv.SPADE || tv.NF == 0 || c.cinp % tv.BK != 0 || it->second.second != 1) {
          error = fmt("%s: tuned choice (variant %d, ksplit %d) does not fit this layer", gname.c_str(), it->second.first, it->second.second); return false;
        }
        ch.v = &tv; ch.ksplit = 1;
      }
      const Variant* v = ch.v;
      if (!v) { error = gname + ": no 1x1 kernel variant"; return false; }
      const int set = ensure_wino_set(h, (int)(&c - h->convs.data()), wm);
      if (set < 0) { error = gname + ": " + h->err; return false; }
      const double fl = 2.0 * c.cin * 9.0 * c.cout * (double)Hout * Wout * B;
      P->flops[RIB_KC_IGEMM] += fl;
      if (v->dma()) {
        OpOf<GemmDmaParams> op(RIB_KC_IGEMM, gname); op.var = v; op.wino = true; op.wino_m = wm; op.flops = fl;
        GemmDmaParams& g = op.p();
        g.M = ntiles; g.N = c.coutp; g.K = c.cinp; g.lda = c.cinp; g.ldc = c.coutp;
        g.sA = (size_t)ntiles * c.cinp; g.sB = (size_t)c.coutp * c.cinp; g.sC = (size_t)ntiles * c.coutp; g.modB = NP;
        op.bind(&GemmDmaParams::A, WS(v_off)); op.bind(&GemmDmaParams::B, WINO(set)); op.bind(&GemmDmaParams::C, WS(m_off));
        op.grid = dim3((ntiles + v->BM() - 1) / v->BM(), (c.coutp + v->BN() - 1) / v->BN(), B * NP);
        push(op);
      } else {
      OpOf<IgemmParams> op(RIB_KC_IGEMM, gname); op.var = v; op.wino = true; op.wino_m = wm; op.flops = fl;
      IgemmParams& p = op.p();
      p.Hin = tilesY; p.Win = tilesX; p.xC = c.cinp; p.Cin = c.cinp; p.CoutPad = c.coutp; p.Hout = tilesY; p.Wout = tilesX;
      p.tilesX = (tilesX + v->TW() - 1) / v->TW(); p.tilesY = (tilesY + v->TH() - 1) / v->TH(); p.xcd_chunk = xcd_chunk_of(p.tilesX * p.tilesY);
      p.act = ACT_NONE; p.ksplit = 1; p.yC = c.coutp; p.yoff = 0; p.Cout = c.coutp;
      p.w_mod = NP; p.w_stride = (unsigned)((size_t)c.coutp * c.cinp);
      op.bind(&IgemmParams::x, WS(v_off)); op.bind(&IgemmParams::w, WINO(set)); op.bind(&IgemmParams::bias, WT(c.zero_off)); op.bind(&IgemmParams::y, WS(m_off));
      op.grid = dim3(p.tilesX * p.tilesY, (c.coutp + v->BN() - 1) / v->BN(), B * NP);
      push(op);
      }
    }
    {
      OpOf<WinoOutParams> op(RIB_KC_CONVAUX, opname + ".wino_out"); op.for_op = gname; op.wino_m = wm;
      WinoOutParams& wo = op.p();
      const int nsl = (c.coutp + 63) / 64, units = ntiles * wm;
      const int blocks = std::max(1, std::min((units + 15) / 16, (int)STATS_MAX_PARTIALS));
      wo.tilesY = tilesY; wo.tilesX = tilesX; wo.CoutPad = c.coutp; wo.ublocks = blocks; wo.nslices = nsl;
      wo.yC = a.out.Cp; wo.yoff = a.yoff; wo.Cout = a.cout_store >= 0 ? a.cout_store : h->padc(c.cout);
      wo.Hout = Hout; wo.Wout = Wout; wo.act = a.act;
      if (a.out.H != Hout || a.out.W != Wout) { error = fmt("%s: output size mismatch", opname.c_str()); return false; }
      op.bind(&WinoOutParams::m, WS(m_off)); op.bind(&WinoOutParams::bias, WT(c.b_off)); op.bind(&WinoOutParams::y, WS(a.out.off));
      if (a.res) { op.bind(&WinoOutParams::res, WS(a.res->off)); wo.resC = a.res->Cp; }
      size_t part_off = 0;
      if (a.want_stats) { part_off = alloc((size_t)B * blocks * 2 * c.coutp * sizeof(double)); op.bind(&WinoOutParams::stat_part, WS(part_off)); }
      op.grid = dim3(blocks * nsl, B, 1);
      push(op);
      if (a.want_stats) {
        OpOf<FinalizeParams> f = finalize_op(opname, part_off, blocks, c.coutp, h->padc(c.cout), *a.stats_out, a.stats_choff, Hout, Wout, a.affine ? &c : nullptr, B);
        finalize_or_defer(f, a.stats_out, a.stats_choff != 0 || a.stats_now, part_off, blocks, c.coutp, f.p().inv_count, a.affine, c.g_off, c.be_off);
      }
    }
    return true;
  }

  bool cond_level_gemm(int level, const Act& cond) {
    const long max_px = pol.cond_gemm_max_px;
    const auto it = h->level_groups.find(level);
    if (it == h->level_groups.end() || it->second.size() < 2 || (long)TB_() * cond.H * cond.W > max_px) return true;
    int N = 0; double fl = 0.0;
    for (int gi : it->second) {
      const SpadeGroup& sg = h->spades[gi];
      if (sg.col0 != N || h->padc(sg.cond) != cond.Cp) { error = fmt("cond level %d: SPADE group %s does not continue the level's filter matrix", level, sg.key.c_str()); return false; }
      N += sg.npad;
      fl += 2.0 * sg.cond * 2.0 * sg.nsets * sg.C * (double)cond.H * cond.W * B;
    }
    const SpadeGroup& first = h->spades[it->second[0]];
    const std::string name = fmt("cond_%d.gammabeta", level);
    Choice ch;
    ch.v = pick_gemm_dma(h->prec(), TB_(), cond.H * cond.W, N, cond.Cp);
    if (!ch.v) ch = choose_variant(h->prec(), 1, 1, false, false, N, TB_(), cond.H, cond.W, cond.Cp, false);
    {
      auto ct = h->choices.find(fmt("%d,%d,%d|%s", TB_(), P->H, P->W, name.c_str()));
      if (ct != h->choices.end()) {
        const Variant& tv = kVariants[ct->second.first];
        if (tv.BF16 != h->prec() || tv.KS != 1 || tv.STRIDE != 1 || tv.UPS || tv.SPADE || tv.NF == 0 || cond.Cp % tv.BK != 0 || ct->second.second != 1) {
          error = fmt("%s: tuned choice (variant %d, ksplit %d) does not fit this launch", name.c_str(), ct->second.first, ct->second.second); return false;
        }
        ch.v = &tv; ch.ksplit = 1;
      }
    }
    const Variant* v = ch.v;
    if (!v) { error = name + ": no 1x1 kernel variant"; return false; }
    const size_t slab_off = alloc((size_t)B * cond.H * cond.W * N * sizeof(float));
    P->flops[RIB_KC_SPADE] += fl;
    LevelSlab ls; ls.off = slab_off; ls.ld = N;
    level_slab[level] = ls;
    if (v->dma()) {
      OpOf<GemmDmaParams> op(RIB_KC_SPADE, name); op.var = v; op.flops = fl;
      GemmDmaParams& g = op.p();
      g.M = cond.H * cond.W; g.N = N; g.K = cond.Cp; g.lda = cond.Cp; g.ldc = N;
      g.sA = (size_t)g.M * cond.Cp; g.sB = 0; g.sC = (size_t)g.M * N; g.modB = 0;
      op.bind(&GemmDmaParams::A, WS(cond.off)); op.bind(&GemmDmaParams::B, WT(h->mc16() ? first.w16_off : first.w_off)); op.bind(&GemmDmaParams::C, WS(slab_off));
      op.grid = dim3((g.M + v->BM() - 1) / v->BM(), (N + v->BN() - 1) / v->BN(), B);
      push(op);
      return true;
    }
    OpOf<IgemmParams> op(RIB_KC_SPADE, name); op.var = v; op.flops = fl;
    IgemmParams& p = op.p();
    p.Hin = cond.H; p.Win = cond.W; p.xC = cond.Cp; p.Cin = cond.Cp;
    p.CoutPad = N; p.Hout = cond.H; p.Wout = cond.W; p.ksplit = 1;
    p.tilesX = (cond.W + v->TW() - 1) / v->TW(); p.tilesY = (cond.H + v->TH() - 1) / v->TH(); p.xcd_chunk = xcd_chunk_of(p.tilesX * p.tilesY);
    op.bind(&IgemmParams::x, WS(cond.off)); op.bind(&IgemmParams::w, WT(h->mc16() ? first.w16_off : first.w_off));
    op.bind(&IgemmParams::bias, WT(first.b_off)); op.bind(&IgemmParams::slab, WS(slab_off));
    op.grid = dim3(p.tilesX * p.tilesY, (N + v->BN() - 1) / v->BN(), B);
    push(op);
    return true;
  }

  bool spade(const std::string& key, const Act& cond, const Act& x, bool x_ups, const Norm& nx,
             Act* ys0, Act* ys1, bool act0, bool lazy_ok = false) {
    const SpadeGroup& sg = h->spades[h->spade_index.at(key)];
    const int Hout = x_ups ? x.H * 2 : x.H, Wout = x_ups ? x.W * 2 : x.W;
    if (cond.H != Hout || cond.W != Wout) { error = fmt("%s: cond map %dx%d != %dx%d (SPADE resize must be the identity)", key.c_str(), cond.H, cond.W, Hout, Wout); return false; }
    if (cond.Cp != h->padc(sg.cond) || cond.Cp % 32 != 0) { error = fmt("%s: cond channels %d unsupported (need a multiple of 32)", key.c_str(), cond.Cp); return false; }
    if (x.Cp != sg.Cp) { error = fmt("%s: x channels %d != %d", key.c_str(), x.Cp, sg.Cp); return false; }
    const Variant* v = choose_variant(h->prec(), 1, 1, false, true, sg.npad, TB_(), Hout, Wout, cond.Cp, false).v;
    if (sg.w1_off)
      for (int i = 0; i < kNumVariants; ++i) {
        const Variant& t = kVariants[i];
        if (t.SPADE && t.NF == 1 && t.BF16 == h->prec() && t.KW == 1 && t.TB == 1 && cond.Cp % t.BK == 0) { v = &t; break; }
      }
    Choice uf;
    const bool small_map = (long)Hout * Wout * TB_() <= 4096 && pol.unfused_spade;
    if (small_map) uf = choose_variant(h->prec(), 1, 1, false, false, sg.npad, TB_(), Hout, Wout, cond.Cp, true);
    bool unfused = small_map && uf.v != nullptr;
    {
      auto it = h->choices.find(fmt("%d,%d,%d|%s", TB_(), P->H, P->W, (key + ".spade").c_str()));
      if (it != h->choices.end()) {
        const Variant& tv = kVariants[it->second.first];
        const int ts = it->second.second;
        if (tv.dma() || tv.BF16 != h->prec() || tv.KS != 1 || tv.STRIDE != 1 || tv.UPS || cond.Cp % tv.BK != 0 || ts < 1 || ts > cond.Cp / tv.BK || (tv.SPADE && ts != 1) ||
            (tv.SPADE && tv.NF == 1 && !sg.w1_off)) {
          error = key + ": tuned SPADE choice does not fit"; return false;
        }
        if (tv.SPADE) { v = &tv; unfused = false; }
        else { uf.v = &tv; uf.ksplit = ts; unfused = true; }
      }
    }
    const auto lvl = level_slab.find(sg.level);
    const bool from_level = lvl != level_slab.end();
    if (from_level) unfused = true;
    if (!unfused && !v) { error = "no SPADE variant"; return false; }
    const bool no_lazy = !pol.lazy_sources;
    if (from_level && lazy_ok && sg.nsets == 1 && !h->keep_taps && !no_lazy && h->prec() == PREC_F32) {
      auto L = std::make_shared<LazySrc>();
      L->mode = WSRC_SPADE; L->name = key + ".spade.modulate"; L->x = x; L->nx = nx; L->x_ups = x_ups; L->lrelu = act0;
      L->slab_off = lvl->second.off; L->slab_ld = lvl->second.ld; L->col0 = sg.col0; L->sbias_off = sg.b_off;
      Act y; y.C = sg.C; y.Cp = sg.Cp; y.H = Hout; y.W = Wout; y.lazy = L;
      *ys0 = y;
      return true;
    }
    if (unfused) {
      *ys0 = act(sg.C, Hout, Wout);
      if (sg.nsets == 2) *ys1 = act(sg.C, Hout, Wout);
      int S = 1, slab_ld = 0, col0 = 0;
      size_t slab_off = 0;
      if (from_level) {
        slab_off = lvl->second.off; slab_ld = lvl->second.ld; col0 = sg.col0;
      } else {
        const Variant* cv = uf.v; S = uf.ksplit;
        slab_off = alloc((size_t)S * B * Hout * Wout * sg.npad * sizeof(float)); slab_ld = sg.npad;
        OpOf<IgemmParams> op(RIB_KC_SPADE, key + ".spade"); op.var = cv;
        IgemmParams& p = op.p();
        p.Hin = cond.H; p.Win = cond.W; p.xC = cond.Cp; p.Cin = cond.Cp;
        p.CoutPad = sg.npad; p.Hout = Hout; p.Wout = Wout; p.ksplit = S;
        p.tilesX = (Wout + cv->TW() - 1) / cv->TW(); p.tilesY = (Hout + cv->TH() - 1) / cv->TH(); p.xcd_chunk = xcd_chunk_of(p.tilesX * p.tilesY);
        op.bind(&IgemmParams::x, WS(cond.off)); op.bind(&IgemmParams::w, WT(h->mc16() ? sg.w16_off : sg.w_off));
        op.bind(&IgemmParams::bias, WT(sg.b_off)); op.bind(&IgemmParams::slab, WS(slab_off));
        op.grid = dim3(p.tilesX * p.tilesY, (sg.npad + cv->BN() - 1) / cv->BN(), B * S);
        op.flops = 2.0 * sg.cond * 2.0 * sg.nsets * sg.C * (double)Hout * Wout * B;
        P->flops[RIB_KC_SPADE] += op.flops;
        push(op);
      }
      OpOf<ModulateParams> mo(RIB_KC_ELTWISE, key + ".spade.modulate");
      ModulateParams& mp = mo.p();
      mp.ksplit = S; mp.B = B; mp.slab_ld = slab_ld; mp.col0 = col0; mp.xmC = x.Cp; mp.xm_ups = x_ups ? 1 : 0;
      mp.m_ld = nx.ld; mp.C = sg.Cp; mp.nsets = sg.nsets; mp.act0 = act0 ? ACT_LRELU : ACT_NONE; mp.act1 = ACT_NONE;
      mp.Hout = Hout; mp.Wout = Wout;
      mo.bind(&ModulateParams::slab, WS(slab_off)); mo.bind(&ModulateParams::bias, WT(sg.b_off)); mo.bind(&ModulateParams::xm, WS(x.off));
      if (!(sg.Cp % 64 == 0 && nx.pend && !nx.pend->affine && sg.Cp <= nx.pend->Cs && take_partials(nx, mo, &ModulateParams::st))) {
        materialize(nx, key + ".spade");
        mo.bind(&ModulateParams::m_scale, WS(nx.sc)); mo.bind(&ModulateParams::m_shift, WS(nx.sh));
      }
      mo.bind(&ModulateParams::ys0, WS(ys0->off)); if (sg.nsets == 2) mo.bind(&ModulateParams::ys1, WS(ys1->off));
      const int nsl = (sg.nsets * sg.Cp + 63) / 64;
      mp.nslices = nsl; mp.pblocks = std::max(1, std::min((Hout * Wout + 15) / 16, (mp.st.tiles > 0 ? 384 : 2048) / nsl));
      mo.grid = dim3(mp.pblocks * nsl, B, 1);
      push(mo);
      return true;
    }
    *ys0 = act(sg.C, Hout, Wout);
    if (sg.nsets == 2) *ys1 = act(sg.C, Hout, Wout);
    OpOf<IgemmParams> op(RIB_KC_SPADE, key + ".spade"); op.var = v;
    IgemmParams& p = op.p();
    p.Hin = cond.H; p.Win = cond.W; p.xC = cond.Cp; p.Cin = cond.Cp;
    const bool one_frag = v->NF == 1;
    const int ncols = one_frag ? 32 : sg.npad;
    p.CoutPad = ncols; p.Hout = Hout; p.Wout = Wout;
    p.tilesX = (Wout + v->TW() - 1) / v->TW(); p.tilesY = (Hout + v->TH() - 1) / v->TH(); p.xcd_chunk = xcd_chunk_of(p.tilesX * p.tilesY);
    p.ksplit = 1;
    p.xmC = x.Cp; p.xm_ups = x_ups ? 1 : 0; p.m_ld = nx.ld; p.C = sg.Cp; p.nsets = sg.nsets;
    p.act0 = act0 ? ACT_LRELU : ACT_NONE; p.act1 = ACT_NONE;
    op.bind(&IgemmParams::x, WS(cond.off)); op.bind(&IgemmParams::w, WT(h->mc16() ? sg.w16_off : sg.w_off)); op.bind(&IgemmParams::bias, WT(sg.b_off));
    if (one_frag) { op.bind(&IgemmParams::w, WT(sg.w1_off)); op.bind(&IgemmParams::bias, WT(sg.b1_off)); }
    op.bind(&IgemmParams::xm, WS(x.off));
    if (has_partials(nx) && !nx.pend->affine && sg.Cp <= nx.pend->Cs) {
      const PendingStats& ps = *nx.pend;
      op.bind(&IgemmParams::m_part, WS(ps.part_off)); p.m_tiles = ps.tiles; p.m_Cs = ps.Cs; p.m_inv = ps.inv_count;
    } else {
      materialize(nx, key + ".spade");
      op.bind(&IgemmParams::m_scale, WS(nx.sc)); op.bind(&IgemmParams::m_shift, WS(nx.sh));
    }
    op.bind(&IgemmParams::ys0, WS(ys0->off)); if (sg.nsets == 2) op.bind(&IgemmParams::ys1, WS(ys1->off));
    op.grid = dim3(p.tilesX * p.tilesY, (ncols + v->BN() - 1) / v->BN(), B);
    op.flops = 2.0 * sg.cond * 2.0 * sg.nsets * sg.C * (double)Hout * Wout * B;
    P->flops[RIB_KC_SPADE] += op.flops;
    push(op);
    return true;
  }

  bool spade_block(const std::string& name, const Act& x, bool x_ups, const Norm& nx, const Act& cond,
                   Act* out, Norm* nout) {
    const ConvDef& c0 = conv_of(h, name + ".conv_block_0");
    const ConvDef& c1 = conv_of(h, name + ".conv_block_1");
    const bool learned = h->conv_index.count(name + ".conv_block_s") > 0;
    const int Hout = x_ups ? x.H * 2 : x.H, Wout = x_ups ? x.W * 2 : x.W;
    Act ys0, ys1;
    Act hbuf = act(c0.cout, Hout, Wout);
    Norm nh = norm(hbuf.Cp);
    { ConvArgs a; a.cd = &c0; a.out = hbuf; a.want_stats = true; a.stats_out = &nh;
      if (!spade(name + ".0", cond, x, x_ups, nx, &ys0, &ys1, true, runs_wino(a, Hout, Wout))) return false;
      if (!ys0.lazy) tap(name + ".ys0", ys0);
      a.in = ys0;
      if (!conv(a, name + ".conv_block_0")) return false; }
    tap(name + ".h", hbuf);
    Act y1, dummy;
    {
      ConvArgs t; t.cd = &c1; t.res = &x; t.res_ups = !learned && x_ups;
      const bool lazy1 = !learned && runs_wino(t, Hout, Wout);
      if (!spade(name + ".1", cond, hbuf, false, nh, &y1, &dummy, true, lazy1)) return false;
    }
    if (!y1.lazy) tap(name + ".y1", y1);
    const bool fuse_s = learned && pol.fuse_shortcut;
    Act outs;
    if (learned && !fuse_s) {
      const ConvDef& cs = conv_of(h, name + ".conv_block_s");
      outs = act(cs.cout, Hout, Wout);
      ConvArgs a; a.cd = &cs; a.in = ys1; a.out = outs;
      if (!conv(a, name + ".conv_block_s")) return false;
    }
    *out = act(c1.cout, Hout, Wout);
    { ConvArgs a; a.cd = &c1; a.in = y1; a.out = *out;
      if (fuse_s) { a.aux = &conv_of(h, name + ".conv_block_s"); a.aux_in = ys1; }
      else a.res = learned ? &outs : &x;
      a.res_ups = !learned && x_ups;
      if (nout) { *nout = norm(out->Cp); a.want_stats = true; a.stats_out = nout; }
      if (!conv(a, name + ".conv_block_1")) return false; }
    tap(name, *out);
    return true;
  }

  bool mask_branch(int b, const Act& input, const Act& CAT, const Norm& ncat, int chm) {
    const rib_config& c = h->g.c;
    const std::string m = "flow_network_temp";
    const char* branches[2] = {"down_lbl", "down_img"};
    Act cur = input; Norm ncur; bool have = false;
    for (int i = 0; i <= c.mask_down; ++i) {
      const ConvDef& cd = conv_of(h, m + "." + branches[b] + "." + std::to_string(i));
      const bool lastl = (i == c.mask_down);
      Act o = lastl ? CAT : act(cd.cout, i == 0 ? cur.H : cur.H / 2, i == 0 ? cur.W : cur.W / 2);
      Norm no = lastl ? ncat : norm(h->padc(cd.cout));
      ConvArgs a; a.cd = &cd; a.in = cur; a.out = o;
      if (have) { a.pro = &ncur; a.pro_lrelu = true; }
      if (i >= 1) {
        a.no_split = true;
        a.choice_names = {m + ".down_pair." + std::to_string(i), m + ".down_img." + std::to_string(i)};
      }
      if (lastl) { a.yoff = b * chm; a.stats_choff = (size_t)b * chm; a.stats_now = true; }
      a.want_stats = true; a.stats_out = &no; a.affine = true;
      if (!conv(a, cd.name)) return false;
      if (!lastl) tap(std::string("mask.") + (b == 0 ? "lbl_" : "img_") + std::to_string(i) + ".raw", o);
      cur = o; ncur = no; have = true;
    }
    return true;
  }

  bool mask_branches_paired(const Act& L, const Act& I9, const Act& CAT, const Norm& ncat, int chm) {
    const rib_config& c = h->g.c;
    const std::string m = "flow_network_temp";
    const Act* inputs[2] = {&L, &I9};
    const char* branches[2] = {"down_lbl", "down_img"};
    Act cur; Norm ncur;
    {
      const ConvDef& c0 = conv_of(h, m + ".down_lbl.0");
      cur = act_n(2, c0.cout, L.H, L.W); ncur = norm(h->padc(c0.cout), 2);
      const size_t img_bytes = (size_t)L.H * L.W * cur.Cp * h->esz();
      for (int b = 0; b < 2; ++b) {
        const ConvDef& cd = conv_of(h, m + "." + branches[b] + ".0");
        Act o = cur; o.off += b * img_bytes;
        Norm no = ncur; no.sc += (size_t)b * ncur.ld * sizeof(float); no.sh += (size_t)b * ncur.ld * sizeof(float);
        ConvArgs a; a.cd = &cd; a.in = *inputs[b]; a.out = o; a.want_stats = true; a.stats_out = &no; a.affine = true; a.stats_now = true;
        if (!conv(a, cd.name)) return false;
        tap(std::string("mask.") + (b == 0 ? "lbl_0" : "img_0") + ".raw", o);
      }
    }
    for (int i = 1; i <= c.mask_down; ++i) {
      const ConvDef& cl = conv_of(h, m + ".down_lbl." + std::to_string(i));
      const ConvDef& ci = conv_of(h, m + ".down_img." + std::to_string(i));
      const bool lastl = (i == c.mask_down);
      Act o = lastl ? CAT : act_n(2, cl.cout, cur.H / 2, cur.W / 2);
      Norm no = lastl ? ncat : norm(h->padc(cl.cout), 2);
      ConvArgs a; a.cd = &cl; a.pair = &ci; a.in = cur; a.out = o; a.pro = &ncur; a.pro_lrelu = true;
      if (lastl) { a.pair_merge = true; a.pair_yoff = chm; }
      a.want_stats = true; a.stats_out = &no; a.affine = true; a.no_split = true;
      a.choice_names = {m + ".down_pair." + std::to_string(i), m + ".down_img." + std::to_string(i)};
      if (!conv(a, m + ".down_pair." + std::to_string(i))) return false;
      if (!lastl) {
        const size_t img_bytes = (size_t)o.H * o.W * o.Cp * h->esz();
        Act ol = o, oi = o; oi.off += img_bytes;
        tap("mask.lbl_" + std::to_string(i) + ".raw", ol);
        tap("mask.img_" + std::to_string(i) + ".raw", oi);
      }
      cur = o; ncur = no;
    }
    return true;
  }
// ... 370 lines not shown
    }
  }
};

#define RIB_LAUNCH_ST(prec, KERNEL, grid, block, lds, st, ...)                                                        \
  do {                                                                                                                \
    if ((prec) == PREC_BF16) RIB_KLAUNCH((KERNEL<ST_BF16>), grid, block, lds, st, __VA_ARGS__);                \
    else if ((prec) == PREC_F16) RIB_KLAUNCH((KERNEL<ST_F16>), grid, block, lds, st, __VA_ARGS__);             \
    else RIB_KLAUNCH((KERNEL<ST_F32>), grid, block, lds, st, __VA_ARGS__);                                     \
  } while (0)

template <int CO, int CIN> void launch_head_t(int bf16, dim3 grid, hipStream_t st, const IgemmParams& p) {
  if (bf16 == PREC_BF16) RIB_KLAUNCH((k_conv_head<CO, CIN, ST_BF16>), grid, dim3(256), 0, st, p);
  else if (bf16 == PREC_F16) RIB_KLAUNCH((k_conv_head<CO, CIN, ST_F16>), grid, dim3(256), 0, st, p);
  else RIB_KLAUNCH((k_conv_head<CO, CIN, ST_F32>), grid, dim3(256), 0, st, p);
}
template <int CO> void launch_small_t(int bf16, dim3 grid, size_t lds, hipStream_t st, const IgemmParams& p) {
  if (bf16 == PREC_BF16) RIB_KLAUNCH((k_conv_small<CO, ST_BF16>), grid, dim3(256), lds, st, p);
  else if (bf16 == PREC_F16) RIB_KLAUNCH((k_conv_small<CO, ST_F16>), grid, dim3(256), lds, st, p);
  else RIB_KLAUNCH((k_conv_small<CO, ST_F32>), grid, dim3(256), lds, st, p);
}
void launch_head(int co, int cin, int bf16, dim3 grid, hipStream_t st, const IgemmParams& p) {
  if (cin == 16) { if (co == 1) launch_head_t<1, 16>(bf16, grid, st, p); else if (co == 2) launch_head_t<2, 16>(bf16, grid, st, p); else launch_head_t<3, 16>(bf16, grid, st, p); }
  else { if (co == 1) launch_head_t<1, 32>(bf16, grid, st, p); else if (co == 2) launch_head_t<2, 32>(bf16, grid, st, p); else launch_head_t<3, 32>(bf16, grid, st, p); }
}

int run_plan(rib_handle* h, Plan* P, const Resolver& R, hipStream_t st, bool skip_label_ops = false) {
  const int bf16 = h->prec();
  for (Op& op : P->ops) {
    if (skip_label_ops && op.label_only) continue;
    g_prof_pair = ProfPair();
    if (h->profiling && h->prof_kernels) {
      ProfPair pp;
      HIP_TRY(h, hipEventCreate(&pp.start));
      HIP_TRY(h, hipEventCreate(&pp.stop));
      h->prof_kernel_events.push_back({op.kclass, pp.start, pp.stop});
      g_prof_pair = pp;
    } else if (h->profiling) {
      hipEvent_t e0 = nullptr;
      HIP_TRY(h, hipEventCreate(&e0));
      HIP_TRY(h, hipEventRecord(e0, st));
      h->prof_events.push_back({op.kclass, e0});
    }
    OpParams params = op.params;
    for (int i = 0; i < op.nbinds; ++i) {
      void* ptr = R.get(op.binds[i].ref);
      memcpy(reinterpret_cast<char*>(&params) + op.binds[i].field, &ptr, sizeof ptr);
    }
    switch (op.kind()) {
      case OP_IGEMM: {
        IgemmParams& p = std::get<IgemmParams>(params);
        p.zeros = R.blob + h->zero_off;
        if (op.small_co > 0 && op.head) {
          if (op.fuse_blend && R.user[U_FUSE]) {
            p.bl_img = reinterpret_cast<const float*>(R.user[U_IMG]); p.bl_dain = reinterpret_cast<const float*>(R.user[U_FAKE]);
            p.bl_fuse = reinterpret_cast<float*>(const_cast<void*>(R.user[U_FUSE]));
          }
          launch_head(op.small_co, p.Cin, bf16, op.grid, st, p);
        } else if (op.small_co > 0) {
          const size_t lds = ((size_t)18 * 18 * (p.Cin + 4) + (size_t)op.small_co * 9 * p.Cin) * sizeof(float);
          switch (op.small_co) {
            case 1: launch_small_t<1>(bf16, op.grid, lds, st, p); break;
            case 2: launch_small_t<2>(bf16, op.grid, lds, st, p); break;
            case 3: launch_small_t<3>(bf16, op.grid, lds, st, p); break;
            default: launch_small_t<4>(bf16, op.grid, lds, st, p); break;
          }
        } else
        RIB_KLAUNCH(pick_igemm_fn(op.var, p), op.grid, dim3(256 * op.var->KW), 0, st, p);
      } break;
      case OP_GEMM:
        RIB_KLAUNCH(h->products == RIB_PRODUCTS_BF16X3 && op.var->gfn_x3 ? op.var->gfn_x3 : op.var->gfn, op.grid, dim3(256), 0, st, std::get<GemmDmaParams>(params));
        break;
      case OP_FINALIZE: {
        const FinalizeParams& p = std::get<FinalizeParams>(params);
        if (p.tiles > 512) RIB_KLAUNCH(k_stats_finalize<4>, dim3((p.Cs + 3) / 4, op.grid.y, op.grid.z), dim3(1024), 0, st, p);
        else RIB_KLAUNCH(k_stats_finalize<16>, op.grid, dim3(1024), 0, st, p);
      } break;
      case OP_MODULATE: RIB_LAUNCH_ST(bf16, k_spade_modulate, op.grid, dim3(256), 0, st, std::get<ModulateParams>(params)); break;
      case OP_SPLITEPI: RIB_LAUNCH_ST(bf16, k_splitk_epilogue, op.grid, dim3(256), 0, st, std::get<SplitEpiParams>(params)); break;
      case OP_POOL: RIB_LAUNCH_ST(bf16, k_avgpool, op.grid, dim3(256), 0, st, std::get<PoolParams>(params)); break;
      case OP_INADD: RIB_LAUNCH_ST(bf16, k_in_add, op.grid, dim3(256), 0, st, std::get<InAddParams>(params)); break;
      case OP_WINO_IN: {
        const WinoInParams& p = std::get<WinoInParams>(params);
        if (op.wino_m == 4) {
          if (op.wi_mode == WSRC_SPADE) RIB_KLAUNCH(k_wino4_in<WSRC_SPADE>, op.grid, dim3(256), 0, st, p);
          else if (op.wi_mode == WSRC_JOIN) RIB_KLAUNCH(k_wino4_in<WSRC_JOIN>, op.grid, dim3(256), 0, st, p);
          else RIB_KLAUNCH(k_wino4_in<WSRC_PLAIN>, op.grid, dim3(256), 0, st, p);
        } else {
          if (op.wi_mode == WSRC_SPADE) RIB_KLAUNCH(k_wino_in<WSRC_SPADE>, op.grid, dim3(256), 0, st, p);
          else if (op.wi_mode == WSRC_JOIN) RIB_KLAUNCH(k_wino_in<WSRC_JOIN>, op.grid, dim3(256), 0, st, p);
          else RIB_KLAUNCH(k_wino_in<WSRC_PLAIN>, op.grid, dim3(256), 0, st, p);
        }
      } break;
      case OP_WINO_OUT:
        if (op.wino_m == 4) RIB_KLAUNCH(k_wino4_out, op.grid, dim3(256), 0, st, std::get<WinoOutParams>(params));
        else RIB_KLAUNCH(k_wino_out, op.grid, dim3(256), 0, st, std::get<WinoOutParams>(params));
        break;
      case OP_LOWC: launch_lowc(op.lowc_ce, op.lowc_ncol, op.lowc_tw, op.grid, st, std::get<LowcParams>(params)); break;
      case OP_PACK: RIB_LAUNCH_ST(bf16, k_pack, op.grid, dim3(256), 0, st, std::get<PackParams>(params)); break;
    }
  }
  g_prof_pair = ProfPair();
  if (h->profiling && !h->prof_kernels) {
    hipEvent_t e1 = nullptr;
    HIP_TRY(h, hipEventCreate(&e1));
    HIP_TRY(h, hipEventRecord(e1, st));
    h->prof_events.push_back({-1, e1});
  }
  HIP_TRY(h, hipGetLastError());
  return RIB_OK;
}

int check_ready(rib_handle* h) {
  if (!h) return RIB_ERR_INVALID;
  if (!h->weights_ready) return fail(h, RIB_ERR_STATE, "weights not loaded: call rib_finalize_weights() or rib_import_weights() first");
  return RIB_OK;
}

}

extern "C" {

int rib_create(const rib_config* cfg, int device, rib_handle** out) {
  if (!cfg || !out) { g_create_error = "rib_create: null argument"; return RIB_ERR_INVALID; }
  *out = nullptr;
  const rib_config& c = *cfg;
  auto bad = [&](const std::string& m) { g_create_error = "rib_create: " + m; return RIB_ERR_UNSUPPORTED; };
  if (c.label_nc < 1 || c.image_nc < 1 || c.num_filters < 1 || c.num_down_img < 1 || c.mask_down < 1 ||
      c.emb_filters < 1 || c.mask_filters < 1 || c.mask_res_blocks < 1 || c.num_layers < c.num_down_img)
    return bad("invalid hyper-parameters");
  if (c.emb_down != c.num_down_img) return bad("embed.num_downsamples must equal num_downsamples_img (HSM.yaml: 4/4)");
  std::unique_ptr<rib_handle> h(new rib_handle());
  h->g.c = c; h->device = device;
  h->graph_replay = getenv("RIB_GRAPH") != nullptr && atoi(getenv("RIB_GRAPH")) != 0;
  for (int i = 0; i <= c.emb_down; ++i) {
    if (h->g.cond_ch(i) != h->g.emb_ch(i)) return bad("embed/generator max_num_filters disagree on the cond map width");
    if (h->g.emb_ch(i) % 32 != 0) return bad(fmt("embed width %d at level %d is not a multiple of 32", h->g.emb_ch(i), i));
  }
  for (int i = 1; i <= c.mask_down; ++i)
    if (h->g.mask_nf(i - 1) % 32 != 0) return bad("mask.num_filters must be a multiple of 32 (stride-2 kernels use 32-channel chunks)");
  for (int i = 0; i <= c.num_down_img + 1; ++i) {
    const int ch = h->g.nf(i);
    if (ch % 4 != 0 || 256 % (ch / 4 > 0 ? ch / 4 : 1) != 0 || ch > 1024) return bad(fmt("generator width %d unsupported (power-of-two multiples of 4 up to 1024)", ch));
  }
  h->convs = build_inventory(h->g);
  for (size_t i = 0; i < h->convs.size(); ++i) h->conv_index[h->convs[i].name] = (int)i;
  register_tensors(h.get());
  assign_weight_layout(h.get());
  if (device >= 0) {
    hipError_t e = hipSetDevice(device);
    if (e == hipSuccess) e = hipMalloc(reinterpret_cast<void**>(&h->d_blob), h->blob_floats * sizeof(float));
    h->d_blob_floats = h->blob_floats;
    if (e != hipSuccess) { g_create_error = fmt("rib_create: device %d: %s", device, hipGetErrorString(e)); return RIB_ERR_HIP; }
  }
  *out = h.release();
  return RIB_OK;
}

void rib_destroy(rib_handle* h) {
  if (!h) return;
  drop_chain_graphs(h);
  for (auto& rs : h->raster_stage) { if (rs.host) (void)hipHostFree(rs.host); if (rs.done) (void)hipEventDestroy(rs.done); }
  if (h->d_blob) (void)hipFree(h->d_blob);
  free_wino_sets(h);
  for (auto& pe : h->prof_events) (void)hipEventDestroy(pe.second);
  for (auto& ke : h->prof_kernel_events) { (void)hipEventDestroy(ke.start); (void)hipEventDestroy(ke.stop); }
  delete h;
// ... 622 lines not shown
  if (!h) return RIB_ERR_INVALID;
  Plan* P = get_plan(h, B, H, W);
  return P ? (int)P->taps.size() : RIB_ERR_INVALID;
}

int rib_tap_info(rib_handle* h, int B, int H, int W, int idx, const char** name, int* C, int* th, int* tw) {
  if (!h) return RIB_ERR_INVALID;
  Plan* P = get_plan(h, B, H, W);
  if (!P || idx < 0 || idx >= (int)P->taps.size()) return RIB_ERR_INVALID;
  const Tap& t = P->taps[idx];
  if (name) *name = t.name.c_str();
  if (C) *C = t.C;
  if (th) *th = t.H;
  if (tw) *tw = t.W;
  return RIB_OK;
}

int rib_read_tap(rib_handle* h, int B, int H, int W, int idx, const void* workspace, float* dst, void* hip_stream) {
  if (!h || !workspace || !dst) return RIB_ERR_INVALID;
  if (!h->keep_taps) return fail(h, RIB_ERR_STATE, "rib_read_tap: call rib_set_debug_taps(h, 1) before the forward (intermediate buffers are reused otherwise)");
  Plan* P = get_plan(h, B, H, W);
  if (!P || idx < 0 || idx >= (int)P->taps.size()) return RIB_ERR_INVALID;
  const Tap& t = P->taps[idx];
  hipStream_t st = reinterpret_cast<hipStream_t>(hip_stream);
  const float* src = reinterpret_cast<const float*>(reinterpret_cast<const char*>(workspace) + t.off);
  RIB_LAUNCH_ST(h->prec(), k_unpack, dim3((t.H * t.W + 255) / 256, B), dim3(256), 0, st, src, t.Cp, t.C, t.H * t.W, 0, t.H, t.W, dst);
  HIP_TRY(h, hipGetLastError());
  HIP_TRY(h, hipStreamSynchronize(st));
  return RIB_OK;
}

int rib_debug_conv_weight(rib_handle* h, const char* conv_name, float* w_oihw, float* bias) {
  if (!h || !conv_name || !w_oihw || !bias) return RIB_ERR_INVALID;
  if (h->host_blob.empty()) return fail(h, RIB_ERR_STATE, "rib_debug_conv_weight needs a finalized host-only handle (device < 0)");
  auto it = h->conv_index.find(conv_name);
  if (it == h->conv_index.end() || !h->convs[it->second].used) return fail(h, RIB_ERR_INVALID, fmt("unknown conv '%s'", conv_name));
  const ConvDef& c = h->convs[it->second];
  const int taps = c.ks * c.ks;
  for (int o = 0; o < c.cout; ++o) {
    for (int i = 0; i < c.cin; ++i)
      for (int t = 0; t < taps; ++t)
        w_oihw[((size_t)o * c.cin + i) * taps + t] = h->host_blob[c.w_off + ((size_t)o * taps + t) * c.cinp + i];
    bias[o] = h->host_blob[c.b_off + o];
  }
  return RIB_OK;
}

int rib_debug_spade_weight(rib_handle* h, const char* conv_name, float* w_2c_by_cond, float* bias_2c) {
  if (!h || !conv_name || !w_2c_by_cond || !bias_2c) return RIB_ERR_INVALID;
  if (h->host_blob.empty()) return fail(h, RIB_ERR_STATE, "rib_debug_spade_weight needs a finalized host-only handle (device < 0)");
  const std::string cn = conv_name;
  const size_t pos = cn.rfind(".conv_block_");
  if (pos == std::string::npos) return fail(h, RIB_ERR_INVALID, "not a SPADE conv block");
  const std::string blk = cn.substr(0, pos), which = cn.substr(cn.size() - 1);
  const std::string key = blk + "." + (which == "s" ? std::string("0") : which);
  auto it = h->spade_index.find(key);
  if (it == h->spade_index.end()) return fail(h, RIB_ERR_INVALID, fmt("no SPADE group '%s'", key.c_str()));
  const SpadeGroup& sg = h->spades[it->second];
  const int set = which == "s" ? 1 : 0;
  const int condp = h->padc(sg.cond);
  for (int ch = 0; ch < sg.C; ++ch) {
    const int v = set * sg.Cp + ch;
    const int colg = (v / 32) * 64 + (v % 32), colb = colg + 32;
    for (int k = 0; k < sg.cond; ++k) {
      w_2c_by_cond[(size_t)ch * sg.cond + k] = h->host_blob[sg.w_off + (size_t)colg * condp + k];
      w_2c_by_cond[(size_t)(sg.C + ch) * sg.cond + k] = h->host_blob[sg.w_off + (size_t)colb * condp + k];
    }
    bias_2c[ch] = h->host_blob[sg.b_off + colg];
    bias_2c[sg.C + ch] = h->host_blob[sg.b_off + colb];
  }
  return RIB_OK;
}

static int launch_info_head(const Op& op, char* buf, size_t buflen) {
  if (op.kind() == OP_IGEMM && op.small_co > 0)
    snprintf(buf, buflen, "%s|%d|%u,%u,%u|%s 16x16 tile, %d output channels%s|%.0f", op.name.c_str(), op.kclass, op.grid.x, op.grid.y, op.grid.z,
             op.head ? "head (taps as MFMA columns)" : "direct (vector ALUs)", op.small_co, op.fuse_blend ? " + fused blend" : "", op.flops);
  else if (op.kind() == OP_IGEMM)
    snprintf(buf, buflen, "%s|%d|%u,%u,%u|tile %dx%d BN %d BK %d s%d k%d ups%d ksplit%d kw%d tb%d%s v%d|%.0f", op.name.c_str(), op.kclass, op.grid.x, op.grid.y, op.grid.z,
             op.var->TH(), op.var->TW(), op.var->BN(), op.var->BK, op.var->STRIDE, op.var->KS, (int)op.var->UPS, op.as<IgemmParams>().ksplit, op.var->KW, op.var->DMAK ? 100 + (op.var->TB == 9 ? 9 : 0) : op.var->TB,
             op.wino ? (op.wino_m == 4 ? " wino4" : " wino") : "", (int)(op.var - kVariants), op.flops);
  else if (op.kind() == OP_GEMM)
    snprintf(buf, buflen, "%s|%d|%u,%u,%u|gemm (LDS-DMA staged operands) tile %dx%d BK 32, %d x [%d x %d x %d]%s|%.0f", op.name.c_str(), op.kclass, op.grid.x, op.grid.y, op.grid.z,
             op.var->BM(), op.var->BN(), (int)op.grid.z, op.as<GemmDmaParams>().M, op.as<GemmDmaParams>().N, op.as<GemmDmaParams>().K, op.wino ? (op.wino_m == 4 ? " wino4" : " wino") : "", op.flops);
  else if (op.kind() == OP_LOWC)
    snprintf(buf, buflen, "%s|%d|%u,%u,%u|lowc (caller's NCHW tensors, K = 9 x %d real channels) 8x%d tile, %d columns|%.0f", op.name.c_str(), op.kclass,
             op.grid.x, op.grid.y, op.grid.z, op.lowc_ce, op.lowc_tw, op.lowc_ncol, op.flops);
  else
    snprintf(buf, buflen, "%s|%d|%u,%u,%u||0", op.name.c_str(), op.kclass, op.grid.x, op.grid.y, op.grid.z);
  return RIB_OK;
}

static double op_algorithmic_bytes(const rib_handle* h, const Plan* P, const Op& op) {
  const double e = h->esz(), Bn = P->B;
  switch (op.kind()) {
    case OP_IGEMM: {
      const IgemmParams& p = op.as<IgemmParams>();
      const double samples = p.pair ? 2.0 * Bn : Bn;
      const int taps = op.var ? op.var->KS * op.var->KS : 9;
      double b = samples * p.Hin * p.Win * (double)p.Cin * e
                 + (double)p.CoutPad * taps * p.Cin * e * (p.pair ? 2.0 : 1.0)
                 + p.CoutPad * 4.0;
      if (op.var && op.var->SPADE) {
        b += Bn * p.Hout * p.Wout * (double)p.C * e / (p.xm_ups ? 4.0 : 1.0);
        b += Bn * p.Hout * p.Wout * (double)p.C * e * p.nsets;
      } else if (op.bound(&IgemmParams::slab)) {
        b += (double)p.ksplit * samples * p.Hout * p.Wout * p.CoutPad * 4.0;
      } else {
        b += samples * p.Hout * p.Wout * (double)p.Cout * (op.small_co > 0 || p.y_f32 ? 4.0 : e);
        if (op.bound(&IgemmParams::res)) b += samples * p.Hout * p.Wout * (double)p.Cout * e / (p.res_ups ? 4.0 : 1.0);
        if (op.bound(&IgemmParams::x2)) b += samples * p.Hout * p.Wout * (double)p.Cin2 * e + (double)p.CoutPad * p.Cin2 * e;
        if (op.fuse_blend) b += Bn * p.Hout * p.Wout * 3.0 * 4.0 * 3.0;
      }
      return b;
    }
    case OP_GEMM: {
      const GemmDmaParams& g = op.as<GemmDmaParams>();
      const double Z = op.grid.z;
      return Z * g.M * (double)g.K * e + (g.modB ? (double)g.modB : 1.0) * g.N * (double)g.K * e + Z * g.M * (double)g.N * 4.0;
    }
    case OP_LOWC: {
      const LowcParams& l = op.as<LowcParams>();
      return Bn * l.H * l.W * (double)(l.c0 + l.c1 + l.c2) * 4.0 + Bn * l.H * l.W * (double)l.Cout * e + 9.0 * (l.c0 + l.c1 + l.c2) * l.Cout * 4.0;
    }
    case OP_POOL: { const PoolParams& q = op.as<PoolParams>(); return Bn * q.H * q.W * (double)q.C * e * 1.25; }
    case OP_INADD: { const InAddParams& q = op.as<InAddParams>(); return Bn * q.HW * (double)q.C * e * 3.0; }
    case OP_SPLITEPI: {
      const SplitEpiParams& q = op.as<SplitEpiParams>();
      return (double)q.ksplit * q.B * q.Hout * q.Wout * q.CoutPad * 4.0 + (double)q.B * q.Hout * q.Wout * q.Cout * e * (op.bound(&SplitEpiParams::res) ? 2.0 : 1.0);
    }
    case OP_MODULATE: {
      const ModulateParams& m = op.as<ModulateParams>();
      const double px = (double)m.B * m.Hout * m.Wout;
      return px * 2.0 * m.C * m.nsets * 4.0 * m.ksplit + px * m.C * e / (m.xm_ups ? 4.0 : 1.0) + px * m.C * e * m.nsets;
    }
    case OP_WINO_IN: {
      const WinoInParams& w = op.as<WinoInParams>();
      const int T = op.wino_m + 2;
      double b = Bn * w.H * w.W * (double)w.Cin * e / (w.x_ups ? 4.0 : 1.0) + Bn * w.tilesY * w.tilesX * (double)T * T * w.Cin * e;
      if (op.wi_mode != 0 && op.bound(&WinoInParams::slab)) b += Bn * w.H * w.W * 2.0 * w.Cin * 4.0;
      if (op.bound(&WinoInParams::x2) || op.bound(&WinoInParams::xres)) b += Bn * w.H * w.W * (double)w.Cin * e * 2.0;
      return b;
    }
    case OP_WINO_OUT: {
      const WinoOutParams& w = op.as<WinoOutParams>();
      const int T = op.wino_m + 2;
      return Bn * w.tilesY * w.tilesX * (double)T * T * w.CoutPad * 4.0 + Bn * w.Hout * w.Wout * (double)w.Cout * e * (op.bound(&WinoOutParams::res) ? 2.0 : 1.0);
    }
    case OP_FINALIZE: { const FinalizeParams& q = op.as<FinalizeParams>(); return Bn * q.tiles * 2.0 * q.Cs * 8.0; }
    default: return 0.0;
  }
}

int rib_debug_launch_info(rib_handle* h, int B, int H, int W, int idx, char* buf, size_t buflen) {
  if (!h || !buf) return RIB_ERR_INVALID;
  Plan* P = get_plan(h, B, H, W);
  if (!P || idx < 0 || idx >= (int)P->ops.size()) return RIB_ERR_INVALID;
  const Op& op = P->ops[idx];
  const int rc = launch_info_head(op, buf, buflen);
  const size_t n = strlen(buf);
  if (n + 24 < buflen) snprintf(buf + n, buflen - n, "|%.0f", op_algorithmic_bytes(h, P, op));
  return rc;
}

const char* rib_build_info(void) {
  static const std::string info = [] {
#define RIB_X(s) rib_stamp_section_##s,
    const char* sh[RIB_NSECTIONS] = {RIB_FOR_SECTIONS(RIB_X)};
#undef RIB_X
    std::string s = std::string("librib stamp=") + (kLibStamp + sizeof("rib-stamp lib ") - 1) + " shards=";
    bool ok = true;
    for (int i = 0; i < RIB_NSECTIONS; ++i) {
      const char* hash = strrchr(sh[i], ' ');
      hash = hash ? hash + 1 : "?";
      ok = ok && strcmp(hash, RIB_SHARD_STAMP) == 0;
      s += std::string(i ? "," : "") + hash;
    }
    s += fmt(" consistent=%d variants=%d compiler=%s", ok ? 1 : 0, kNumVariants, __VERSION__);
    return s;
  }();
  return info.c_str();
}

int rib_num_variants(void) { return kNumVariants; }

int rib_variant_info(int idx, int geom[12]) {
  if (idx < 0 || idx >= kNumVariants || !geom) return RIB_ERR_INVALID;
  const Variant& v = kVariants[idx];
  const int g[12] = {v.FRW, v.WM, v.WN, v.MF, v.NF, v.BK, v.STRIDE, v.KS, v.UPS ? 1 : 0, v.SPADE ? 1 : 0, v.KW, v.DMAK ? 100 + (v.TB == 9 ? 9 : 0) : v.TB};
  for (int i = 0; i < 12; ++i) geom[i] = g[i];
  return v.BF16;
}

int rib_set_choice(rib_handle* h, int B, int H, int W, const char* op_name, int variant_idx, int ksplit) {
  if (!h || !op_name) return RIB_ERR_INVALID;
  const std::string key = fmt("%d,%d,%d|%s", B, H, W, op_name);
  if (variant_idx < 0) h->choices.erase(key);
  else {
    if (variant_idx >= kNumVariants || ksplit < 1) return fail(h, RIB_ERR_INVALID, "rib_set_choice: bad variant / ksplit");
    h->choices[key] = {variant_idx, ksplit};
  }
  drop_chain_graphs(h);
  for (auto it = h->plans.begin(); it != h->plans.end();) {
    const std::array<int, 5>& k = it->first;
    const bool same_hw = k[3] == H && k[4] == W;
    const bool follows = same_hw && (k[1] > 0 ? k[1] : k[2]) == B;
    if (follows) it = h->plans.erase(it); else ++it;
  }
  return RIB_OK;
}

int rib_time_op(rib_handle* h, int B, int H, int W, const char* op_name, const float* label, const float* img_fake,
                const float* img_prev, float* img, float* mask, void* workspace, size_t workspace_bytes, int iters,
                void* hip_stream, double* usec) {
  int rc = check_ready(h);
  if (rc) return rc;
  if (!op_name || !workspace || !usec || iters < 1) return RIB_ERR_INVALID;
  Plan* P = get_plan(h, B, H, W);
  if (!P) return RIB_ERR_INVALID;
  if (workspace_bytes < P->ws_bytes) return fail(h, RIB_ERR_WORKSPACE, "rib_time_op: workspace too small");
  Plan sub; sub.B = B; sub.H = H; sub.W = W;
  const std::string nm = op_name;
  for (const Op& op : P->ops)
// ... 86 lines not shown
```

Baseline: 391.3.

## Fuse 1x1 learned shortcut into Winograd conv via extended K and masked positions

Folds the 1x1 learned-shortcut convolution into the Winograd-domain GEMM of conv_block_1. The shortcut weights are transformed into the Winograd positions where they are nonzero, and the input transform writes the shortcut input into extra K columns. The GEMM extends K only for those positions through a per-position mask. This removes a separate shortcut conv pass and lets the second SPADE set stay lazy. In exchange it adds a wider V buffer, more template instantiations and a more complex planner path.

```diff
diff --git a/render-in-between_amd/csrc/kernels.hip.h b/render-in-between_amd/csrc/kernels.hip.h
--- a/render-in-between_amd/csrc/kernels.hip.h
+++ b/render-in-between_amd/csrc/kernels.hip.h
@@ -8,6 +8,7 @@
   int M, N, K, lda, ldc;
   size_t sA, sB, sC;
   int modB;
+  int K2; unsigned long long kmask;
 };
 
 typedef uint32_t u32x4 __attribute__((ext_vector_type(4)));
@@ -49,7 +50,8 @@
   for (int nf = 0; nf < NF; ++nf)
 #pragma unroll
     for (int r = 0; r < 16; ++r) { acc[nf][r] = 0.f; if constexpr (X3 == 2) acc_s[nf][r] = 0.f; }
-  const int nch = p.K / (BK * EPW);
+  const int ldb = (p.K + p.K2) / EPW;
+  const int nch = (p.K + (p.K2 && ((p.kmask >> (z % p.modB)) & 1ull) ? p.K2 : 0)) / (BK * EPW);
   typedef __attribute__((address_space(3))) void lds_void;
   const uint32_t lds0 = (uint32_t)(size_t)(lds_void*)smem;
   const float* src[NFILL];
@@ -59,7 +61,7 @@
     const bool isA = 32 * j < BM;
     const int row = isA ? trow : trow - BM;
     const int ls = (lane & 7) ^ ((row >> 1) & 7);
-    src[j] = isA ? A + (size_t)min(m0 + row, p.M - 1) * (p.lda / EPW) + ls * 4 : B + (size_t)min(n0 + row, p.N - 1) * (p.K / EPW) + ls * 4;
+    src[j] = isA ? A + (size_t)min(m0 + row, p.M - 1) * (p.lda / EPW) + ls * 4 : B + (size_t)min(n0 + row, p.N - 1) * ldb + ls * 4;
   }
   auto fill = [&](int st, int kc) {
 #pragma unroll
@@ -332,7 +334,18 @@
   int nslices, ublocks;
   int x_ups; const float* slab; int slab_ld, col0; const float* sbias;
   const float* x2; const float* xres; float* o; const float* pro2_scale; const float* pro2_shift; StatSrc st2;
+  int ldv;
+  int nslices2, Cin2, xC2, x2_ups, lrelu2, pro2_ld;
+  const float* slab2; int slab2_ld, col0_2; const float* sbias2;
 };
+__device__ __forceinline__ WinoInParams wino_second(const WinoInParams& p) {
+  WinoInParams q = p;
+  q.x = p.x2; q.xC = p.xC2; q.Cin = p.Cin2; q.x_ups = p.x2_ups; q.pro_lrelu = p.lrelu2;
+  q.pro_scale = p.pro2_scale; q.pro_shift = p.pro2_shift; q.pro_ld = p.pro2_ld; q.st = p.st2;
+  q.slab = p.slab2; q.slab_ld = p.slab2_ld; q.col0 = p.col0_2; q.sbias = p.sbias2;
+  q.x2 = nullptr; q.v = p.v + p.Cin;
+  return q;
+}
 
 __device__ __forceinline__ float spade_mod1(float x, float sc, float sh, float g, float bg, float b, float bb) {
   return fmaf(fmaf(x, sc, sh), 1.f + (g + bg), b + bb);
@@ -416,21 +429,19 @@
 #define RIB_F4_SUB(a, b) make_float4((a).x - (b).x, (a).y - (b).y, (a).z - (b).z, (a).w - (b).w)
 #define RIB_F4_ADD(a, b) make_float4((a).x + (b).x, (a).y + (b).y, (a).z + (b).z, (a).w + (b).w)
 
-template <int MODE>
-__global__ __launch_bounds__(256) void k_wino_in(const WinoInParams p) {
-  __shared__ double red[4 * 64 * 2];
-  __shared__ float s_sc[64], s_sh[64];
+template <int MODE, bool SC>
+__device__ __forceinline__ void wino_in_slice(const WinoInParams& p, int slice, int ub, double* red, float* s_sc, float* s_sh) {
   const int c4n = p.Cin / 4;
   const int n = blockIdx.y;
-  const int slice = blockIdx.x % p.nslices, ub = blockIdx.x / p.nslices;
   const int c4 = slice * 16 + (threadIdx.x & 15);
   const bool cok = c4 < c4n;
   const int ntiles = p.tilesY * p.tilesX;
+  constexpr int NR = SC ? 2 : 4, Q0 = SC ? 1 : 0, Q1 = SC ? 3 : 4;
   WinoConsts<MODE> kc;
   wino_in_consts<MODE>(p, n, slice, c4, cok, red, s_sc, s_sh, kc);
   if (!cok) return;
-  for (int u = ub * 16 + (threadIdx.x >> 4); u < ntiles * 4; u += p.ublocks * 16) {
-    const int r = u & 3, tile = u >> 2;
+  for (int u = ub * 16 + (threadIdx.x >> 4); u < ntiles * NR; u += p.ublocks * 16) {
+    const int r = SC ? 1 + (u & 1) : u & 3, tile = SC ? u >> 1 : u >> 2;
     const int ty = tile / p.tilesX, tx = tile % p.tilesX;
     const int ia = r == 0 ? 0 : (r == 2 ? 2 : 1), ib = r == 0 ? 2 : (r == 1 ? 2 : (r == 2 ? 1 : 3));
     const float sg = r == 1 ? 1.f : -1.f;
@@ -438,13 +449,13 @@
 #pragma unroll
     for (int a = 0; a < 2; ++a)
 #pragma unroll
-      for (int q = 0; q < 4; ++q) {
+      for (int q = Q0; q < Q1; ++q) {
         const int iy = 2 * ty - 1 + (a ? ib : ia), ix = 2 * tx - 1 + q;
         wino_fetch<MODE>(p, n, min(max(iy, 0), p.H - 1), min(max(ix, 0), p.W - 1), c4, d[a][q]);
       }
     float4 t[4];
 #pragma unroll
-    for (int q = 0; q < 4; ++q) {
+    for (int q = Q0; q < Q1; ++q) {
       float4 v[2];
 #pragma unroll
       for (int a = 0; a < 2; ++a) {
@@ -459,13 +470,25 @@
       }
       t[q] = make_float4(v[0].x + sg * v[1].x, v[0].y + sg * v[1].y, v[0].z + sg * v[1].z, v[0].w + sg * v[1].w);
     }
-    const size_t plane = (size_t)ntiles * p.Cin;
-    float* vb = p.v + (size_t)n * 16 * plane + (size_t)tile * p.Cin + c4 * 4;
-    *reinterpret_cast<float4*>(vb + (size_t)(r * 4 + 0) * plane) = RIB_F4_SUB(t[0], t[2]);
+    const size_t plane = (size_t)ntiles * p.ldv;
+    float* vb = p.v + (size_t)n * 16 * plane + (size_t)tile * p.ldv + c4 * 4;
+    if constexpr (!SC) *reinterpret_cast<float4*>(vb + (size_t)(r * 4 + 0) * plane) = RIB_F4_SUB(t[0], t[2]);
     *reinterpret_cast<float4*>(vb + (size_t)(r * 4 + 1) * plane) = RIB_F4_ADD(t[1], t[2]);
     *reinterpret_cast<float4*>(vb + (size_t)(r * 4 + 2) * plane) = RIB_F4_SUB(t[2], t[1]);
-    *reinterpret_cast<float4*>(vb + (size_t)(r * 4 + 3) * plane) = RIB_F4_SUB(t[1], t[3]);
-  }
+    if constexpr (!SC) *reinterpret_cast<float4*>(vb + (size_t)(r * 4 + 3) * plane) = RIB_F4_SUB(t[1], t[3]);
+  }
+}
+
+template <int MODE, int MODE2 = -1>
+__global__ __launch_bounds__(256) void k_wino_in(const WinoInParams p) {
+  __shared__ double red[4 * 64 * 2];
+  __shared__ float s_sc[64], s_sh[64];
+  const int slice = blockIdx.x % p.nslices, ub = blockIdx.x / p.nslices;
+  if constexpr (MODE2 >= 0) {
+    const int n1 = p.nslices - p.nslices2;
+    if (slice >= n1) { wino_in_slice<MODE2, true>(wino_second(p), slice - n1, ub, red, s_sc, s_sh); return; }
+  }
+  wino_in_slice<MODE, false>(p, slice, ub, red, s_sc, s_sh);
 }
 
 struct WinoOutParams {
@@ -567,21 +590,19 @@
 }
 __device__ __forceinline__ float4 f4_scale(float a, float4 x) { return make_float4(a * x.x, a * x.y, a * x.z, a * x.w); }
 
-template <int MODE>
-__global__ __launch_bounds__(256) void k_wino4_in(const WinoInParams p) {
-  __shared__ double red[4 * 64 * 2];
-  __shared__ float s_sc[64], s_sh[64];
+template <int MODE, bool SC>
+__device__ __forceinline__ void wino4_in_slice(const WinoInParams& p, int slice, int ub, double* red, float* s_sc, float* s_sh) {
   const int c4n = p.Cin / 4;
   const int n = blockIdx.y;
-  const int slice = blockIdx.x % p.nslices, ub = blockIdx.x / p.nslices;
   const int c4 = slice * 16 + (threadIdx.x & 15);
   const bool cok = c4 < c4n;
   const int ntiles = p.tilesY * p.tilesX;
+  constexpr int NR = SC ? 4 : 6, Q0 = SC ? 1 : 0, Q1 = SC ? 5 : 6;
   WinoConsts<MODE> kc;
   wino_in_consts<MODE>(p, n, slice, c4, cok, red, s_sc, s_sh, kc);
   if (!cok) return;
-  for (int u = ub * 16 + (threadIdx.x >> 4); u < ntiles * 6; u += p.ublocks * 16) {
-    const int r = u % 6, tile = u / 6;
+  for (int u = ub * 16 + (threadIdx.x >> 4); u < ntiles * NR; u += p.ublocks * 16) {
+    const int r = SC ? 1 + u % 4 : u % 6, tile = u / NR;
     const int ty = tile / p.tilesX, tx = tile % p.tilesX;
     const int a0 = r == 0 ? 0 : 1, da = (r == 0 || r == 5) ? 2 : 1, na = (r == 0 || r == 5) ? 3 : 4;
     float4 t[6];
@@ -592,7 +613,7 @@
 #pragma unroll
       for (int k = 0; k < 4; ++k)
 #pragma unroll
-        for (int q = 0; q < 6; ++q) {
+        for (int q = Q0; q < Q1; ++q) {
           const int iy = 4 * ty - 1 + a0 + min(k, na - 1) * da, ix = 4 * tx - 1 + q;
           wino_fetch<MODE>(p, n, min(max(iy, 0), p.H - 1), min(max(ix, 0), p.W - 1), c4, d[k][q]);
         }
@@ -602,7 +623,7 @@
         const float coef = k < na ? kWino4BT[r][a] : 0.f;
         const int iy = 4 * ty - 1 + a;
 #pragma unroll
-        for (int q = 0; q < 6; ++q) {
+        for (int q = Q0; q < Q1; ++q) {
           const int ix = 4 * tx - 1 + q;
           float4 w = wino_value<MODE>(p, kc, d[k][q]);
           if (!(iy >= 0 && iy < p.H && ix >= 0 && ix < p.W)) w = make_float4(0.f, 0.f, 0.f, 0.f);
@@ -617,9 +638,9 @@
         const int iy = 4 * ty - 1 + a;
         WinoRaw<MODE> d[6];
 #pragma unroll
-        for (int q = 0; q < 6; ++q) wino_fetch<MODE>(p, n, min(max(iy, 0), p.H - 1), min(max(4 * tx - 1 + q, 0), p.W - 1), c4, d[q]);
-#pragma unroll
-        for (int q = 0; q < 6; ++q) {
+        for (int q = Q0; q < Q1; ++q) wino_fetch<MODE>(p, n, min(max(iy, 0), p.H - 1), min(max(4 * tx - 1 + q, 0), p.W - 1), c4, d[q]);
+#pragma unroll
+        for (int q = Q0; q < Q1; ++q) {
           const int ix = 4 * tx - 1 + q;
           const bool inb = iy >= 0 && iy < p.H && ix >= 0 && ix < p.W;
           float4 w = wino_value<MODE>(p, kc, d[q]);
@@ -631,19 +652,33 @@
         }
       }
     }
-    const size_t plane = (size_t)ntiles * p.Cin;
-    float* vb = p.v + (size_t)n * 36 * plane + (size_t)tile * p.Cin + c4 * 4;
-    const float4 e24 = f4_fma(-45.f / 16, t[2], t[4]);
-    const float4 o13 = f4_fma(-45.f / 16, t[3], t[5]);
+    const size_t plane = (size_t)ntiles * p.ldv;
+    float* vb = p.v + (size_t)n * 36 * plane + (size_t)tile * p.ldv + c4 * 4;
     const float4 ev1 = f4_fma(-9.f / 4, t[2], t[4]), od1 = f4_fma(-27.f / 16, t[1], f4_scale(3.f / 4, t[3]));
     const float4 ev2 = f4_fma(-9.f / 16, t[2], t[4]), od2 = f4_fma(-27.f / 32, t[1], f4_scale(3.f / 2, t[3]));
-    *reinterpret_cast<float4*>(vb + (size_t)(r * 6 + 0) * plane) = f4_fma(81.f / 64, t[0], e24);
+    if constexpr (!SC) {
+      const float4 e24 = f4_fma(-45.f / 16, t[2], t[4]);
+      const float4 o13 = f4_fma(-45.f / 16, t[3], t[5]);
+      *reinterpret_cast<float4*>(vb + (size_t)(r * 6 + 0) * plane) = f4_fma(81.f / 64, t[0], e24);
+      *reinterpret_cast<float4*>(vb + (size_t)(r * 6 + 5) * plane) = f4_fma(81.f / 64, t[1], o13);
+    }
     *reinterpret_cast<float4*>(vb + (size_t)(r * 6 + 1) * plane) = RIB_F4_ADD(ev1, od1);
     *reinterpret_cast<float4*>(vb + (size_t)(r * 6 + 2) * plane) = RIB_F4_SUB(ev1, od1);
     *reinterpret_cast<float4*>(vb + (size_t)(r * 6 + 3) * plane) = RIB_F4_ADD(ev2, od2);
     *reinterpret_cast<float4*>(vb + (size_t)(r * 6 + 4) * plane) = RIB_F4_SUB(ev2, od2);
-    *reinterpret_cast<float4*>(vb + (size_t)(r * 6 + 5) * plane) = f4_fma(81.f / 64, t[1], o13);
-  }
+  }
+}
+
+template <int MODE, int MODE2 = -1>
+__global__ __launch_bounds__(256) void k_wino4_in(const WinoInParams p) {
+  __shared__ double red[4 * 64 * 2];
+  __shared__ float s_sc[64], s_sh[64];
+  const int slice = blockIdx.x % p.nslices, ub = blockIdx.x / p.nslices;
+  if constexpr (MODE2 >= 0) {
+    const int n1 = p.nslices - p.nslices2;
+    if (slice >= n1) { wino4_in_slice<MODE2, true>(wino_second(p), slice - n1, ub, red, s_sc, s_sh); return; }
+  }
+  wino4_in_slice<MODE, false>(p, slice, ub, red, s_sc, s_sh);
 }
 
 __global__ __launch_bounds__(256) void k_wino4_out(const WinoOutParams p) {
diff --git a/render-in-between_amd/csrc/rib.hip b/render-in-between_amd/csrc/rib.hip
--- a/render-in-between_amd/csrc/rib.hip
+++ b/render-in-between_amd/csrc/rib.hip
@@ -129,6 +129,7 @@
   int cinp = 0, coutp = 0;
   size_t w16_off = 0, wp16_off = 0;
   bool wino_ok = false; size_t zero_off = 0;
+  bool wino_s_ok = false;
   size_t wl_off = 0; int lowc_ce = 0, lowc_ncol = 0;
 };
 
@@ -431,6 +432,7 @@
   bool wino = false;
   int wino_m = 0;
   int wi_mode = 0;
+  int wi_mode2 = -1;
   int lowc_ce = 0, lowc_ncol = 0, lowc_tw = 32;
   OpParams params;
   struct Binding { PRef ref; unsigned field = 0; };
@@ -532,9 +534,9 @@
   size_t blob_floats = 0;
   size_t zero_off = 0;
   uint64_t layout_hash = 0;
-  struct WinoSet { int conv = 0, wm = 0; float* d = nullptr; size_t floats = 0; };
+  struct WinoSet { int conv = 0, wm = 0; float* d = nullptr; size_t floats = 0; int aux = -1; };
   std::vector<WinoSet> wino_sets;
-  std::map<std::pair<int, int>, int> wino_index;
+  std::map<std::array<int, 3>, int> wino_index;
   bool weights_ready = false;
   int prec_mode = PREC_F32;
   int prec() const { return prec_mode; }
@@ -594,7 +596,7 @@
   return h->convs[h->conv_index.at(name)];
 }
 
-__global__ __launch_bounds__(256) void k_wino_filters(const float* w, float* u, int coutp, int cinp, int wm) {
+__global__ __launch_bounds__(256) void k_wino_filters(const float* w, float* u, int coutp, int cinp, int wm, int ldu) {
 #pragma clang fp contract(off)
   const double G2[4][3] = {{1, 0, 0}, {0.5, 0.5, 0.5}, {0.5, -0.5, 0.5}, {0, 0, 1}};
   const double G4[6][3] = {{64.0 / 81, 0, 0},
@@ -615,7 +617,22 @@
   for (int r = 0; r < T; ++r)
     for (int q = 0; q < T; ++q) {
       const double* Gq = wm == 2 ? G2[q] : G4[q];
-      u[((size_t)(r * T + q) * coutp + o) * cinp + i] = (float)(t[r][0] * Gq[0] + t[r][1] * Gq[1] + t[r][2] * Gq[2]);
+      u[((size_t)(r * T + q) * coutp + o) * ldu + i] = (float)(t[r][0] * Gq[0] + t[r][1] * Gq[1] + t[r][2] * Gq[2]);
+    }
+}
+__global__ __launch_bounds__(256) void k_wino_filters_1x1(const float* w, float* u, int coutp, int cin2, int wm, int ldu, int col0) {
+#pragma clang fp contract(off)
+  const double G2c[4] = {0, 0.5, -0.5, 0};
+  const double G4c[6] = {0, -32.0 / 81, 32.0 / 81, 16.0 / 81, -16.0 / 81, 0};
+  const int T = wm + 2;
+  const size_t idx = (size_t)blockIdx.x * 256 + threadIdx.x;
+  if (idx >= (size_t)coutp * cin2) return;
+  const int o = (int)(idx / cin2), i = (int)(idx % cin2);
+  const double g = (double)w[(size_t)o * cin2 + i];
+  for (int r = 0; r < T; ++r)
+    for (int q = 0; q < T; ++q) {
+      const double gr = wm == 2 ? G2c[r] : G4c[r], gq = wm == 2 ? G2c[q] : G4c[q];
+      u[((size_t)(r * T + q) * coutp + o) * ldu + col0 + i] = (float)((gr * g) * gq);
     }
 }
 
@@ -624,16 +641,23 @@
   const ConvDef& c = h->convs[ws.conv];
   if (!ws.d || !h->d_blob) return RIB_OK;
   const size_t n = (size_t)c.coutp * c.cinp;
-  RIB_KLAUNCH(k_wino_filters, dim3((unsigned)((n + 255) / 256)), dim3(256), 0, st, h->d_blob + c.w_off, ws.d, c.coutp, c.cinp, ws.wm);
+  const int k2 = ws.aux >= 0 ? h->convs[ws.aux].cinp : 0;
+  RIB_KLAUNCH(k_wino_filters, dim3((unsigned)((n + 255) / 256)), dim3(256), 0, st, h->d_blob + c.w_off, ws.d, c.coutp, c.cinp, ws.wm, c.cinp + k2);
   HIP_TRY(h, hipGetLastError());
-  return RIB_OK;
-}
-
-int ensure_wino_set(rib_handle* h, int ci, int wm) {
-  auto it = h->wino_index.find({ci, wm});
+  if (k2) {
+    const size_t n2 = (size_t)c.coutp * k2;
+    RIB_KLAUNCH(k_wino_filters_1x1, dim3((unsigned)((n2 + 255) / 256)), dim3(256), 0, st, h->d_blob + h->convs[ws.aux].w_off, ws.d, c.coutp, k2, ws.wm, c.cinp + k2, c.cinp);
+    HIP_TRY(h, hipGetLastError());
+  }
+  return RIB_OK;
+}
+
+int ensure_wino_set(rib_handle* h, int ci, int wm, int aux = -1) {
+  auto it = h->wino_index.find({ci, wm, aux});
   if (it != h->wino_index.end()) return it->second;
   const ConvDef& c = h->convs[ci];
-  rib_handle::WinoSet ws; ws.conv = ci; ws.wm = wm; ws.floats = (size_t)(wm + 2) * (wm + 2) * c.coutp * c.cinp;
+  rib_handle::WinoSet ws; ws.conv = ci; ws.wm = wm; ws.aux = aux;
+  ws.floats = (size_t)(wm + 2) * (wm + 2) * c.coutp * (c.cinp + (aux >= 0 ? h->convs[aux].cinp : 0));
   if (h->device >= 0) {
     hipError_t e = hipSetDevice(h->device);
     if (e == hipSuccess) e = hipMalloc(reinterpret_cast<void**>(&ws.d), ws.floats * sizeof(float));
@@ -641,7 +665,7 @@
   }
   const int si = (int)h->wino_sets.size();
   h->wino_sets.push_back(ws);
-  h->wino_index[{ci, wm}] = si;
+  h->wino_index[{ci, wm, aux}] = si;
   if (h->device >= 0 && h->weights_ready) {
     if (hipDeviceSynchronize() != hipSuccess) { h->err = "Winograd filter transform: device not idle-able"; return -1; }
     if (fill_wino_set(h, si, nullptr) != RIB_OK) return -1;
@@ -729,9 +753,10 @@
     }
     for (auto& sg : h->spades) sg.b_off = take(sg.npad);
   }
-  for (auto& c : h->convs) { c.wino_ok = false; c.zero_off = 0; }
+  for (auto& c : h->convs) { c.wino_ok = false; c.wino_s_ok = false; c.zero_off = 0; }
   if (h->prec() == PREC_F32 && !getenv("RIB_NO_WINO")) {
     for (auto& c : h->convs) {
+      if (c.used && c.ks == 3 && c.stride == 1 && !c.ups_in && c.fb_off != 0 && c.cout >= 64 && c.cinp % 32 == 0 && 128 % (c.coutp / 4) == 0) c.wino_s_ok = true;
       if (!c.used || c.ks != 3 || c.stride != 1 || c.ups_in || c.fb_off != 0 || c.cin < 256 || c.cout < 64 || c.cinp % 32 || 128 % (c.coutp / 4)) continue;
       c.wino_ok = true;
       c.zero_off = take(c.coutp);
@@ -832,6 +857,8 @@
   bool unfused_spade = !getenv("RIB_NO_UNFUSED_SPADE");
   bool lazy_sources = !getenv("RIB_NO_LAZY");
   bool fuse_shortcut = !getenv("RIB_NO_FUSE_SHORTCUT");
+  bool wino_shortcut = !getenv("RIB_NO_WINO_SHORTCUT");
+  int wino_shortcut_m = getenv("RIB_WINO_SHORTCUT_M") ? atoi(getenv("RIB_WINO_SHORTCUT_M")) : 0;
   bool ws_reuse = !getenv("RIB_NO_WS_REUSE");
   static bool pair_mask_encoders() { return !getenv("RIB_NO_PAIR"); }
 };
@@ -954,10 +981,21 @@
     std::vector<std::string> choice_names;
   };
 
-  bool runs_wino(const ConvArgs& a, int Hout, int Wout) const {
+  bool runs_wino(const ConvArgs& a, int Hout, int Wout, const std::string& opname = std::string()) const {
     const ConvDef& c = *a.cd;
-    return h->prec() == PREC_F32 && c.wino_ok && !a.ups && !a.aux && !a.res_ups && !a.pair && !a.in.virt && a.y_nchw.sp == PS_NULL &&
-           a.y_user.sp == PS_NULL && (long)Hout * Wout <= pol.wino_max_px && Hout >= 2 && Wout >= 2;
+    return h->prec() == PREC_F32 && (a.aux ? c.wino_s_ok : c.wino_ok) && !a.ups && !a.res_ups && !a.pair && !a.in.virt && a.y_nchw.sp == PS_NULL &&
+           a.y_user.sp == PS_NULL && (long)Hout * Wout <= pol.wino_max_px && Hout >= 2 && Wout >= 2 &&
+           (!a.aux || (!a.res && shortcut_wino_m(c, *a.aux, opname, Hout, Wout) != 0));
+  }
+  int default_wino_m(int Hout, int Wout) const { return (long)TB_() * ((Hout + 3) / 4) * ((Wout + 3) / 4) >= 256 ? 4 : 2; }
+  int shortcut_wino_m(const ConvDef& c, const ConvDef& s, const std::string& opname, int Hout, int Wout) const {
+    if (!pol.wino_shortcut || !pol.fuse_shortcut || opname.empty() || !c.fb_off || s.ks != 1 || s.coutp != c.coutp || s.cinp % 32 != 0 || c.cinp % 32 != 0) return 0;
+    if (!pick_gemm_dma(h->prec(), 16, 64, c.coutp, c.cinp)) return 0;
+    if (pol.wino_shortcut_m == 2 || pol.wino_shortcut_m == 4) return pol.wino_shortcut_m;
+    const int d = default_wino_m(Hout, Wout);
+    for (int m : {d, 6 - d})
+      if (h->choices.count(fmt("%d,%d,%d|%s%s", TB_(), P->H, P->W, opname.c_str(), m == 2 ? ".wino" : ".wino4"))) return m;
+    return 0;
   }
   bool would_wino(const ConvDef& cd, int H, int W) const { ConvArgs t; t.cd = &cd; return runs_wino(t, H, W); }
 
@@ -976,8 +1014,9 @@
       }
     }
     if (a.in.Cp != c.cinp) { error = fmt("%s: input channels %d != expected %d", opname.c_str(), a.in.Cp, c.cinp); return false; }
-    if (runs_wino(a, Hout, Wout)) return conv_wino(a, opname, Hout, Wout);
+    if (runs_wino(a, Hout, Wout, opname)) return conv_wino(a, opname, Hout, Wout);
     if (a.in.lazy) { error = opname + ": a lazy input (" + a.in.lazy->name + ") needs the Winograd path"; return false; }
+    if (a.aux && a.aux_in.lazy) { error = opname + ": a lazy shortcut input (" + a.aux_in.lazy->name + ") needs the Winograd path"; return false; }
     const bool can_split = (256 % (c.coutp / 4) == 0) && a.y_nchw.sp == PS_NULL && !a.pair && !a.no_split && pol.split_k;
     const bool can_n16 = c.cout <= 16 && !a.res && !h->mc16() && pol.n16;
     Choice ch = choose_variant(h->prec(), c.stride, c.ks, a.ups, false, c.coutp, TB_(), Hout, Wout, c.cinp, can_split, a.aux ? a.aux->cinp : 0, can_n16);
@@ -1134,17 +1173,23 @@
   bool conv_wino(const ConvArgs& a, const std::string& opname, int Hout, int Wout) {
     const ConvDef& c = *a.cd;
     const int wino_force = pol.wino_force;
-    const int wm = wino_force == 2 || wino_force == 4 ? wino_force : ((long)TB_() * ((Hout + 3) / 4) * ((Wout + 3) / 4) >= 256 ? 4 : 2);
+    const int wm = a.aux ? shortcut_wino_m(c, *a.aux, opname, Hout, Wout) : (wino_force == 2 || wino_force == 4 ? wino_force : default_wino_m(Hout, Wout));
     const int NP = (wm + 2) * (wm + 2);
     const int tilesY = (Hout + wm - 1) / wm, tilesX = (Wout + wm - 1) / wm, ntiles = tilesY * tilesX;
     const std::string gname = opname + (wm == 2 ? ".wino" : ".wino4");
-    const size_t v_off = alloc((size_t)B * NP * ntiles * c.cinp * sizeof(float));
+    const int K2 = a.aux ? a.aux->cinp : 0, ldv = c.cinp + K2;
+    unsigned long long kmask = 0;
+    if (a.aux) {
+      if (a.aux_in.Cp != K2 || a.aux_in.H != Hout || a.aux_in.W != Wout || a.in.H != Hout || a.in.W != Wout) { error = opname + ": fused shortcut operand does not fit"; return false; }
+      for (int r = 1; r <= wm; ++r) for (int q = 1; q <= wm; ++q) kmask |= 1ull << (r * (wm + 2) + q);
+    }
+    const size_t v_off = alloc((size_t)B * NP * ntiles * ldv * sizeof(float));
     const size_t m_off = alloc((size_t)B * NP * ntiles * c.coutp * sizeof(float));
     {
       OpOf<WinoInParams> op(RIB_KC_CONVAUX, opname + ".wino_in"); op.for_op = gname; op.wino_m = wm;
       WinoInParams& wi = op.p();
       wi.H = a.in.H; wi.W = a.in.W; wi.xC = a.in.Cp; wi.Cin = c.cinp; wi.tilesY = tilesY; wi.tilesX = tilesX;
-      wi.pro_lrelu = a.pro_lrelu ? 1 : 0;
+      wi.pro_lrelu = a.pro_lrelu ? 1 : 0; wi.ldv = ldv;
       op.bind(&WinoInParams::x, WS(a.in.off)); op.bind(&WinoInParams::v, WS(v_off));
       if (a.in.lazy) {
         const LazySrc& L = *a.in.lazy;
@@ -1169,7 +1214,20 @@
         wi.pro_ld = a.pro->ld;
         op.bind(&WinoInParams::pro_scale, WS(a.pro->sc + a.pro_choff * sizeof(float))); op.bind(&WinoInParams::pro_shift, WS(a.pro->sh + a.pro_choff * sizeof(float)));
       }
-      const int nsl = (c.cinp + 63) / 64, units = ntiles * (wm + 2);
+      if (a.aux) {
+        if (op.wi_mode == WSRC_JOIN) { error = gname + ": a join cannot carry a second source"; return false; }
+        wi.nslices2 = (K2 + 63) / 64; wi.Cin2 = K2; wi.xC2 = a.aux_in.Cp;
+        op.wi_mode2 = WSRC_PLAIN;
+        if (a.aux_in.lazy) {
+          const LazySrc& L = *a.aux_in.lazy;
+          if (L.mode != WSRC_SPADE) { error = gname + ": lazy shortcut input of an unknown kind"; return false; }
+          op.wi_mode2 = WSRC_SPADE;
+          op.bind(&WinoInParams::x2, WS(L.x.off)); wi.xC2 = L.x.Cp; wi.pro2_ld = L.nx.ld; wi.x2_ups = L.x_ups ? 1 : 0; wi.lrelu2 = L.lrelu ? 1 : 0;
+          if (!take_partials(L.nx, op, &WinoInParams::st2)) { materialize(L.nx, gname); op.bind(&WinoInParams::pro2_scale, WS(L.nx.sc)); op.bind(&WinoInParams::pro2_shift, WS(L.nx.sh)); }
+          op.bind(&WinoInParams::slab2, WS(L.slab_off)); wi.slab2_ld = L.slab_ld; wi.col0_2 = L.col0; op.bind(&WinoInParams::sbias2, WT(L.sbias_off));
+        } else op.bind(&WinoInParams::x2, WS(a.aux_in.off));
+      }
+      const int nsl = (c.cinp + 63) / 64 + wi.nslices2, units = ntiles * (wm + 2);
       wi.nslices = nsl; wi.ublocks = std::max(1, std::min((units + 15) / 16, (wi.st.tiles > 0 ? 512 : 4096) / nsl));
       op.grid = dim3(wi.ublocks * nsl, B, 1);
       push(op);
@@ -1181,22 +1239,24 @@
       auto it = h->choices.find(fmt("%d,%d,%d|%s", TB_(), P->H, P->W, gname.c_str()));
       if (it != h->choices.end()) {
         const Variant& tv = kVariants[it->second.first];
-        if (tv.BF16 != h->prec() || tv.KS != 1 || tv.STRIDE != 1 || tv.UPS || tv.SPADE || tv.NF == 0 || c.cinp % tv.BK != 0 || it->second.second != 1) {
+        if (tv.BF16 != h->prec() || tv.KS != 1 || tv.STRIDE != 1 || tv.UPS || tv.SPADE || tv.NF == 0 || c.cinp % tv.BK != 0 || it->second.second != 1 || (a.aux && !tv.dma())) {
           error = fmt("%s: tuned choice (variant %d, ksplit %d) does not fit this layer", gname.c_str(), it->second.first, it->second.second); return false;
         }
         ch.v = &tv; ch.ksplit = 1;
       }
       const Variant* v = ch.v;
       if (!v) { error = gname + ": no 1x1 kernel variant"; return false; }
-      const int set = ensure_wino_set(h, (int)(&c - h->convs.data()), wm);
+      if (a.aux && !v->dma()) { error = gname + ": the fused shortcut needs a k_gemm_dma tile"; return false; }
+      const int set = ensure_wino_set(h, (int)(&c - h->convs.data()), wm, a.aux ? (int)(a.aux - h->convs.data()) : -1);
       if (set < 0) { error = gname + ": " + h->err; return false; }
-      const double fl = 2.0 * c.cin * 9.0 * c.cout * (double)Hout * Wout * B;
+      const double fl = 2.0 * c.cin * 9.0 * c.cout * (double)Hout * Wout * B + (a.aux ? 2.0 * a.aux->cin * a.aux->cout * (double)Hout * Wout * B : 0.0);
       P->flops[RIB_KC_IGEMM] += fl;
       if (v->dma()) {
         OpOf<GemmDmaParams> op(RIB_KC_IGEMM, gname); op.var = v; op.wino = true; op.wino_m = wm; op.flops = fl;
         GemmDmaParams& g = op.p();
-        g.M = ntiles; g.N = c.coutp; g.K = c.cinp; g.lda = c.cinp; g.ldc = c.coutp;
-        g.sA = (size_t)ntiles * c.cinp; g.sB = (size_t)c.coutp * c.cinp; g.sC = (size_t)ntiles * c.coutp; g.modB = NP;
+        g.M = ntiles; g.N = c.coutp; g.K = c.cinp; g.lda = ldv; g.ldc = c.coutp;
+        g.sA = (size_t)ntiles * ldv; g.sB = (size_t)c.coutp * ldv; g.sC = (size_t)ntiles * c.coutp; g.modB = NP;
+        g.K2 = K2; g.kmask = kmask;
         op.bind(&GemmDmaParams::A, WS(v_off)); op.bind(&GemmDmaParams::B, WINO(set)); op.bind(&GemmDmaParams::C, WS(m_off));
         op.grid = dim3((ntiles + v->BM() - 1) / v->BM(), (c.coutp + v->BN() - 1) / v->BN(), B * NP);
         push(op);
@@ -1221,7 +1281,7 @@
       wo.yC = a.out.Cp; wo.yoff = a.yoff; wo.Cout = a.cout_store >= 0 ? a.cout_store : h->padc(c.cout);
       wo.Hout = Hout; wo.Wout = Wout; wo.act = a.act;
       if (a.out.H != Hout || a.out.W != Wout) { error = fmt("%s: output size mismatch", opname.c_str()); return false; }
-      op.bind(&WinoOutParams::m, WS(m_off)); op.bind(&WinoOutParams::bias, WT(c.b_off)); op.bind(&WinoOutParams::y, WS(a.out.off));
+      op.bind(&WinoOutParams::m, WS(m_off)); op.bind(&WinoOutParams::bias, WT(a.aux ? c.fb_off : c.b_off)); op.bind(&WinoOutParams::y, WS(a.out.off));
       if (a.res) { op.bind(&WinoOutParams::res, WS(a.res->off)); wo.resC = a.res->Cp; }
       size_t part_off = 0;
       if (a.want_stats) { part_off = alloc((size_t)B * blocks * 2 * c.coutp * sizeof(double)); op.bind(&WinoOutParams::stat_part, WS(part_off)); }
@@ -1290,7 +1350,7 @@
   }
 
   bool spade(const std::string& key, const Act& cond, const Act& x, bool x_ups, const Norm& nx,
-             Act* ys0, Act* ys1, bool act0, bool lazy_ok = false) {
+             Act* ys0, Act* ys1, bool act0, bool lazy_ok = false, bool lazy1_ok = false) {
     const SpadeGroup& sg = h->spades[h->spade_index.at(key)];
     const int Hout = x_ups ? x.H * 2 : x.H, Wout = x_ups ? x.W * 2 : x.W;
     if (cond.H != Hout || cond.W != Wout) { error = fmt("%s: cond map %dx%d != %dx%d (SPADE resize must be the identity)", key.c_str(), cond.H, cond.W, Hout, Wout); return false; }
@@ -1324,17 +1384,23 @@
     if (from_level) unfused = true;
     if (!unfused && !v) { error = "no SPADE variant"; return false; }
     const bool no_lazy = !pol.lazy_sources;
-    if (from_level && lazy_ok && sg.nsets == 1 && !h->keep_taps && !no_lazy && h->prec() == PREC_F32) {
+    const bool can_lazy = from_level && !h->keep_taps && !no_lazy && h->prec() == PREC_F32;
+    const bool lz1 = can_lazy && lazy1_ok && sg.nsets == 2 && sg.Cp % 32 == 0;
+    const bool lz0 = can_lazy && lazy_ok && (sg.nsets == 1 || lz1);
+    const int set1_col = sg.Cp / 32 * 64;
+    for (int set = 0; set < 2; ++set) {
+      if (!(set ? lz1 : lz0)) continue;
       auto L = std::make_shared<LazySrc>();
-      L->mode = WSRC_SPADE; L->name = key + ".spade.modulate"; L->x = x; L->nx = nx; L->x_ups = x_ups; L->lrelu = act0;
-      L->slab_off = lvl->second.off; L->slab_ld = lvl->second.ld; L->col0 = sg.col0; L->sbias_off = sg.b_off;
+      L->mode = WSRC_SPADE; L->name = key + ".spade.modulate"; L->x = x; L->nx = nx; L->x_ups = x_ups; L->lrelu = set ? false : act0;
+      L->slab_off = lvl->second.off; L->slab_ld = lvl->second.ld; L->col0 = sg.col0 + set * set1_col; L->sbias_off = sg.b_off + set * set1_col;
       Act y; y.C = sg.C; y.Cp = sg.Cp; y.H = Hout; y.W = Wout; y.lazy = L;
-      *ys0 = y;
-      return true;
-    }
+      *(set ? ys1 : ys0) = y;
+    }
+    if (lz0 && (lz1 || sg.nsets == 1)) return true;
+    const int mnsets = lz1 ? 1 : sg.nsets;
     if (unfused) {
       *ys0 = act(sg.C, Hout, Wout);
-      if (sg.nsets == 2) *ys1 = act(sg.C, Hout, Wout);
+      if (sg.nsets == 2 && !lz1) *ys1 = act(sg.C, Hout, Wout);
       int S = 1, slab_ld = 0, col0 = 0;
       size_t slab_off = 0;
       if (from_level) {
@@ -1357,15 +1423,15 @@
       OpOf<ModulateParams> mo(RIB_KC_ELTWISE, key + ".spade.modulate");
       ModulateParams& mp = mo.p();
       mp.ksplit = S; mp.B = B; mp.slab_ld = slab_ld; mp.col0 = col0; mp.xmC = x.Cp; mp.xm_ups = x_ups ? 1 : 0;
-      mp.m_ld = nx.ld; mp.C = sg.Cp; mp.nsets = sg.nsets; mp.act0 = act0 ? ACT_LRELU : ACT_NONE; mp.act1 = ACT_NONE;
+      mp.m_ld = nx.ld; mp.C = sg.Cp; mp.nsets = mnsets; mp.act0 = act0 ? ACT_LRELU : ACT_NONE; mp.act1 = ACT_NONE;
       mp.Hout = Hout; mp.Wout = Wout;
       mo.bind(&ModulateParams::slab, WS(slab_off)); mo.bind(&ModulateParams::bias, WT(sg.b_off)); mo.bind(&ModulateParams::xm, WS(x.off));
       if (!(sg.Cp % 64 == 0 && nx.pend && !nx.pend->affine && sg.Cp <= nx.pend->Cs && take_partials(nx, mo, &ModulateParams::st))) {
         materialize(nx, key + ".spade");
         mo.bind(&ModulateParams::m_scale, WS(nx.sc)); mo.bind(&ModulateParams::m_shift, WS(nx.sh));
       }
-      mo.bind(&ModulateParams::ys0, WS(ys0->off)); if (sg.nsets == 2) mo.bind(&ModulateParams::ys1, WS(ys1->off));
-      const int nsl = (sg.nsets * sg.Cp + 63) / 64;
+      mo.bind(&ModulateParams::ys0, WS(ys0->off)); if (mnsets == 2) mo.bind(&ModulateParams::ys1, WS(ys1->off));
+      const int nsl = (mnsets * sg.Cp + 63) / 64;
       mp.nslices = nsl; mp.pblocks = std::max(1, std::min((Hout * Wout + 15) / 16, (mp.st.tiles > 0 ? 384 : 2048) / nsl));
       mo.grid = dim3(mp.pblocks * nsl, B, 1);
       push(mo);
@@ -1410,20 +1476,20 @@
     Act ys0, ys1;
     Act hbuf = act(c0.cout, Hout, Wout);
     Norm nh = norm(hbuf.Cp);
+    const bool fuse_s = learned && pol.fuse_shortcut;
+    bool wino1;
+    { ConvArgs t; t.cd = &c1;
+      if (fuse_s) t.aux = &conv_of(h, name + ".conv_block_s"); else { t.res = &x; t.res_ups = !learned && x_ups; }
+      wino1 = runs_wino(t, Hout, Wout, name + ".conv_block_1"); }
     { ConvArgs a; a.cd = &c0; a.out = hbuf; a.want_stats = true; a.stats_out = &nh;
-      if (!spade(name + ".0", cond, x, x_ups, nx, &ys0, &ys1, true, runs_wino(a, Hout, Wout))) return false;
+      if (!spade(name + ".0", cond, x, x_ups, nx, &ys0, &ys1, true, runs_wino(a, Hout, Wout), fuse_s && wino1)) return false;
       if (!ys0.lazy) tap(name + ".ys0", ys0);
       a.in = ys0;
       if (!conv(a, name + ".conv_block_0")) return false; }
     tap(name + ".h", hbuf);
     Act y1, dummy;
-    {
-      ConvArgs t; t.cd = &c1; t.res = &x; t.res_ups = !learned && x_ups;
-      const bool lazy1 = !learned && runs_wino(t, Hout, Wout);
-      if (!spade(name + ".1", cond, hbuf, false, nh, &y1, &dummy, true, lazy1)) return false;
-    }
+    if (!spade(name + ".1", cond, hbuf, false, nh, &y1, &dummy, true, (!learned || fuse_s) && wino1)) return false;
     if (!y1.lazy) tap(name + ".y1", y1);
-    const bool fuse_s = learned && pol.fuse_shortcut;
     Act outs;
     if (learned && !fuse_s) {
       const ConvDef& cs = conv_of(h, name + ".conv_block_s");
@@ -1960,7 +2026,16 @@
       case OP_INADD: RIB_LAUNCH_ST(bf16, k_in_add, op.grid, dim3(256), 0, st, std::get<InAddParams>(params)); break;
       case OP_WINO_IN: {
         const WinoInParams& p = std::get<WinoInParams>(params);
-        if (op.wino_m == 4) {
+        if (op.wi_mode2 >= 0) {
+          const bool s1 = op.wi_mode == WSRC_SPADE, s2 = op.wi_mode2 == WSRC_SPADE;
+#define RIB_WINO_IN2(K)                                                                                     \
+          if (s1 && s2) RIB_KLAUNCH((K<WSRC_SPADE, WSRC_SPADE>), op.grid, dim3(256), 0, st, p);             \
+          else if (s1) RIB_KLAUNCH((K<WSRC_SPADE, WSRC_PLAIN>), op.grid, dim3(256), 0, st, p);              \
+          else if (s2) RIB_KLAUNCH((K<WSRC_PLAIN, WSRC_SPADE>), op.grid, dim3(256), 0, st, p);              \
+          else RIB_KLAUNCH((K<WSRC_PLAIN, WSRC_PLAIN>), op.grid, dim3(256), 0, st, p)
+          if (op.wino_m == 4) { RIB_WINO_IN2(k_wino4_in); } else { RIB_WINO_IN2(k_wino_in); }
+#undef RIB_WINO_IN2
+        } else if (op.wino_m == 4) {
           if (op.wi_mode == WSRC_SPADE) RIB_KLAUNCH(k_wino4_in<WSRC_SPADE>, op.grid, dim3(256), 0, st, p);
           else if (op.wi_mode == WSRC_JOIN) RIB_KLAUNCH(k_wino4_in<WSRC_JOIN>, op.grid, dim3(256), 0, st, p);
           else RIB_KLAUNCH(k_wino4_in<WSRC_PLAIN>, op.grid, dim3(256), 0, st, p);
@@ -2749,7 +2824,7 @@
              op.wino ? (op.wino_m == 4 ? " wino4" : " wino") : "", (int)(op.var - kVariants), op.flops);
   else if (op.kind() == OP_GEMM)
     snprintf(buf, buflen, "%s|%d|%u,%u,%u|gemm (LDS-DMA staged operands) tile %dx%d BK 32, %d x [%d x %d x %d]%s|%.0f", op.name.c_str(), op.kclass, op.grid.x, op.grid.y, op.grid.z,
-             op.var->BM(), op.var->BN(), (int)op.grid.z, op.as<GemmDmaParams>().M, op.as<GemmDmaParams>().N, op.as<GemmDmaParams>().K, op.wino ? (op.wino_m == 4 ? " wino4" : " wino") : "", op.flops);
+             op.var->BM(), op.var->BN(), (int)op.grid.z, op.as<GemmDmaParams>().M, op.as<GemmDmaParams>().N, op.as<GemmDmaParams>().K, (std::string(op.wino ? (op.wino_m == 4 ? " wino4" : " wino") : "") + (op.as<GemmDmaParams>().K2 ? fmt(" + K %d of the 1x1 shortcut at %d positions", op.as<GemmDmaParams>().K2, __builtin_popcountll(op.as<GemmDmaParams>().kmask)) : std::string())).c_str(), op.flops);
   else if (op.kind() == OP_LOWC)
     snprintf(buf, buflen, "%s|%d|%u,%u,%u|lowc (caller's NCHW tensors, K = 9 x %d real channels) 8x%d tile, %d columns|%.0f", op.name.c_str(), op.kclass,
              op.grid.x, op.grid.y, op.grid.z, op.lowc_ce, op.lowc_tw, op.lowc_ncol, op.flops);
@@ -2784,7 +2859,9 @@
     case OP_GEMM: {
       const GemmDmaParams& g = op.as<GemmDmaParams>();
       const double Z = op.grid.z;
-      return Z * g.M * (double)g.K * e + (g.modB ? (double)g.modB : 1.0) * g.N * (double)g.K * e + Z * g.M * (double)g.N * 4.0;
+      const double z2 = g.K2 ? Bn * __builtin_popcountll(g.kmask) : 0.0, nb2 = g.K2 ? (double)__builtin_popcountll(g.kmask) : 0.0;
+      return Z * g.M * (double)g.K * e + (g.modB ? (double)g.modB : 1.0) * g.N * (double)g.K * e + Z * g.M * (double)g.N * 4.0 +
+             z2 * g.M * (double)g.K2 * e + nb2 * g.N * (double)g.K2 * e;
     }
     case OP_LOWC: {
       const LowcParams& l = op.as<LowcParams>();
@@ -2806,6 +2883,10 @@
       const int T = op.wino_m + 2;
       double b = Bn * w.H * w.W * (double)w.Cin * e / (w.x_ups ? 4.0 : 1.0) + Bn * w.tilesY * w.tilesX * (double)T * T * w.Cin * e;
       if (op.wi_mode != 0 && op.bound(&WinoInParams::slab)) b += Bn * w.H * w.W * 2.0 * w.Cin * 4.0;
+      if (op.wi_mode2 >= 0) {
+        b += Bn * w.H * w.W * (double)w.Cin2 * e / (w.x2_ups ? 4.0 : 1.0) + Bn * w.tilesY * w.tilesX * (double)op.wino_m * op.wino_m * w.Cin2 * e;
+        if (op.bound(&WinoInParams::slab2)) b += Bn * w.H * w.W * 2.0 * w.Cin2 * 4.0;
+      } else
       if (op.bound(&WinoInParams::x2) || op.bound(&WinoInParams::xres)) b += Bn * w.H * w.W * (double)w.Cin * e * 2.0;
       return b;
     }
```

New measurement: 395.5, median of 6. 1.01x the previous value.
